# sony/aki

Hardware: AMD Instinct MI355X
Metric: image+text tokens/sec forward, AKI-4B, 336px img + 512 txt (higher is better)
Workload: dtype bf16

## Files before the change

aki_amd/_lib.py:

```python
from __future__ import annotations

import ctypes as C
import os
from typing import Optional

_HERE = os.path.dirname(os.path.abspath(__file__))
LIB_PATH = os.environ.get("AKI_MI355X_LIB") or os.path.join(_HERE, "lib", "libaki_mi355x.so")
LAB_LIB_PATH = os.path.join(_HERE, "lib", "libaki_mi355x_lab.so")

AKI_DT_BF16, AKI_DT_F32, AKI_DT_FP8_E4M3, AKI_DT_W8A16, AKI_DT_W4A16 = 0, 1, 2, 3, 4
AKI_ACT_NONE, AKI_ACT_GELU_ERF, AKI_ACT_GELU_TANH, AKI_ACT_SWIGLU = 0, 1, 2, 3
AKI_DEAD_ROWS_ZERO, AKI_DEAD_ROWS_UNIFORM = 0, 1
AKI_MAX_RECTS = 8
AKI_PLAN_STRIDE = 12
AKI_ABI_VERSION = 17
AKI_LOGITS_PROCESS_MAX_V = 131072
AKI_BEAM_MAX_K, AKI_BEAM_MAX_EOS, AKI_KV_BEAM_REORDER_CHUNK = 16, 8, 16


class AkiError(RuntimeError):
    pass


class MmaRect(C.Structure):
    _fields_ = [("row_lo", C.c_int32), ("row_hi", C.c_int32), ("col_lo", C.c_int32), ("col_hi", C.c_int32)]


class MmaAttnCoreArgs(C.Structure):
    _fields_ = [("q", C.c_void_p), ("k", C.c_void_p), ("v", C.c_void_p), ("o", C.c_void_p), ("lse", C.c_void_p),
                ("rects", C.c_void_p), ("col_valid_bits", C.c_void_p), ("seq_lens", C.c_void_p),
                ("max_rects", C.c_int32), ("B", C.c_int32), ("H", C.c_int32), ("L", C.c_int32), ("Dh", C.c_int32),
                ("scale", C.c_float), ("dtype", C.c_int32), ("dead_rows", C.c_int32), ("kv_capacity", C.c_int32)]


class MmaAttnArgs(C.Structure):
    _fields_ = [("x", C.c_void_p), ("w_qkv", C.c_void_p), ("cos", C.c_void_p), ("sin", C.c_void_p),
                ("position_ids", C.c_void_p), ("o", C.c_void_p), ("lse", C.c_void_p), ("rects", C.c_void_p),
                ("col_valid_bits", C.c_void_p), ("seq_lens", C.c_void_p), ("max_rects", C.c_int32),
                ("B", C.c_int32), ("H", C.c_int32), ("L", C.c_int32), ("Dh", C.c_int32), ("d_model", C.c_int32),
                ("ldx", C.c_int32), ("ldw", C.c_int32), ("pos_rows", C.c_int32), ("scale", C.c_float),
                ("dtype", C.c_int32), ("dead_rows", C.c_int32), ("kv_capacity", C.c_int32),
                ("x_scale", C.c_void_p), ("w_scale", C.c_void_p), ("row_scale", C.c_void_p)]


class AttnArgs(C.Structure):
    _fields_ = [("q", C.c_void_p), ("k", C.c_void_p), ("v", C.c_void_p), ("o", C.c_void_p),
                ("q_stride_b", C.c_int64), ("q_stride_h", C.c_int64), ("q_stride_t", C.c_int64),
                ("k_stride_b", C.c_int64), ("k_stride_h", C.c_int64), ("k_stride_t", C.c_int64),
                ("v_stride_b", C.c_int64), ("v_stride_h", C.c_int64), ("v_stride_t", C.c_int64),
                ("B", C.c_int32), ("H", C.c_int32), ("Lq", C.c_int32), ("Lk", C.c_int32), ("Dh", C.c_int32),
                ("scale", C.c_float), ("dtype", C.c_int32), ("lse", C.c_void_p)]


class AttnBwdArgs(C.Structure):
    _fields_ = [("q", C.c_void_p), ("k", C.c_void_p), ("v", C.c_void_p), ("o", C.c_void_p), ("d_o", C.c_void_p), ("lse", C.c_void_p),
                ("dq", C.c_void_p), ("dk", C.c_void_p), ("dv", C.c_void_p), ("rects", C.c_void_p), ("max_rects", C.c_int32),
                ("col_valid_bits", C.c_void_p), ("seq_lens", C.c_void_p), ("masked", C.c_int32),
                ("B", C.c_int32), ("H", C.c_int32), ("Lq", C.c_int32), ("Lk", C.c_int32), ("Dh", C.c_int32),
                ("scale", C.c_float), ("dtype", C.c_int32)]


class LinearArgs(C.Structure):
    _fields_ = [("x", C.c_void_p), ("w", C.c_void_p), ("bias", C.c_void_p), ("residual", C.c_void_p), ("y", C.c_void_p),
                ("M", C.c_int32), ("N", C.c_int32), ("K", C.c_int32), ("ldx", C.c_int32), ("ldw", C.c_int32),
                ("ldy", C.c_int32), ("ldr", C.c_int32), ("res_row_mod", C.c_int32), ("act", C.c_int32),
                ("dtype", C.c_int32), ("x_scale", C.c_void_p), ("w_scale", C.c_void_p),
                ("w2", C.c_void_p), ("w2_row0", C.c_int32), ("w2_rows", C.c_int32),
                ("row_scale", C.c_void_p), ("row_shift", C.c_void_p), ("col_shift", C.c_void_p), ("stats_rstd", C.c_void_p),
                ("stats_mean", C.c_void_p), ("stats_eps", C.c_float), ("stats_workspace", C.c_void_p),
                ("stats_workspace_bytes", C.c_size_t), ("splitk_workspace", C.c_void_p), ("splitk_workspace_bytes", C.c_size_t),
                ("preact_out", C.c_void_p), ("ld_preact", C.c_int64)]


class DecoderLayer(C.Structure):
    _fields_ = [("w_qkv", C.c_void_p), ("w_o", C.c_void_p), ("w_gate_up", C.c_void_p), ("w_down", C.c_void_p), ("k_cache", C.c_void_p),
                ("v_cache", C.c_void_p)]


class DecoderStackArgs(C.Structure):
    _fields_ = [("layers", C.POINTER(DecoderLayer)), ("n_layers", C.c_int32), ("h_in", C.c_void_p), ("h_out", C.c_void_p), ("rstd_out", C.c_void_p),
                ("cos", C.c_void_p), ("sin", C.c_void_p), ("position_ids", C.c_void_p), ("pos_rows", C.c_int32), ("rects", C.c_void_p),
                ("col_valid_bits", C.c_void_p), ("seq_lens", C.c_void_p), ("max_rects", C.c_int32), ("B", C.c_int32), ("H", C.c_int32),
                ("L", C.c_int32), ("Dh", C.c_int32), ("d", C.c_int32), ("F", C.c_int32), ("kv_capacity", C.c_int32), ("scale", C.c_float),
                ("rms_eps", C.c_float), ("dead_rows", C.c_int32), ("workspace", C.c_void_p), ("workspace_bytes", C.c_size_t),
                ("stats_workspace", C.c_void_p), ("stats_workspace_bytes", C.c_size_t), ("splitk_workspace", C.c_void_p),
                ("splitk_workspace_bytes", C.c_size_t)]


class SiglipLayer(C.Structure):
    _fields_ = [("w_qkv", C.c_void_p), ("b_qkv", C.c_void_p), ("c_qkv", C.c_void_p), ("w_out", C.c_void_p), ("b_out", C.c_void_p),
                ("w_fc1", C.c_void_p), ("b_fc1", C.c_void_p), ("c_fc1", C.c_void_p), ("w_fc2", C.c_void_p), ("b_fc2", C.c_void_p)]


class SiglipStackArgs(C.Structure):
    _fields_ = [("layers", C.POINTER(SiglipLayer)), ("n_layers", C.c_int32), ("h_in", C.c_void_p), ("h_out", C.c_void_p), ("fc1_out", C.c_void_p),
                ("N", C.c_int32), ("L", C.c_int32), ("E", C.c_int32), ("heads", C.c_int32), ("I", C.c_int32), ("Ip", C.c_int32),
                ("act", C.c_int32), ("ln_eps", C.c_float), ("scale", C.c_float), ("workspace", C.c_void_p), ("workspace_bytes", C.c_size_t),
                ("stats_workspace", C.c_void_p), ("stats_workspace_bytes", C.c_size_t), ("splitk_workspace", C.c_void_p),
                ("splitk_workspace_bytes", C.c_size_t)]


class PerceiverLayer(C.Structure):
    _fields_ = [("norm_media_w", C.c_void_p), ("norm_media_b", C.c_void_p), ("norm_latents_w", C.c_void_p), ("norm_latents_b", C.c_void_p),
                ("w_q", C.c_void_p), ("w_kv", C.c_void_p), ("w_out", C.c_void_p), ("ff_ln_w", C.c_void_p), ("ff_ln_b", C.c_void_p),
                ("ff_w1", C.c_void_p), ("ff_w2", C.c_void_p)]


class PerceiverStackArgs(C.Structure):
    _fields_ = [("layers", C.POINTER(PerceiverLayer)), ("n_layers", C.c_int32), ("x", C.c_void_p), ("latents", C.c_void_p), ("norm_w", C.c_void_p),
                ("norm_b", C.c_void_p), ("proj_w", C.c_void_p), ("proj_b", C.c_void_p), ("out", C.c_void_p), ("n1", C.c_int32), ("n2", C.c_int32),
                ("D", C.c_int32), ("heads", C.c_int32), ("dim_head", C.c_int32), ("d_ff", C.c_int32), ("D_out", C.c_int32), ("scale", C.c_float),
                ("eps", C.c_float), ("workspace", C.c_void_p), ("workspace_bytes", C.c_size_t)]


class SpliceArgs(C.Structure):
    _fields_ = [("lang_x", C.c_void_p), ("attention_mask", C.c_void_p), ("labels", C.c_void_p),
                ("embed_weight", C.c_void_p), ("embed_additional", C.c_void_p), ("vision_tokens", C.c_void_p),
                ("plan", C.c_void_p), ("inputs_embeds", C.c_void_p), ("labels_out", C.c_void_p),
                ("mask_1d_out", C.c_void_p), ("rects", C.c_void_p), ("col_valid_bits", C.c_void_p),
                ("seq_lens", C.c_void_p), ("max_original_id", C.c_int64), ("media_token_id", C.c_int64),
                ("pad_token_id", C.c_int64), ("B", C.c_int32), ("T", C.c_int32), ("T_img", C.c_int32),
                ("Nv", C.c_int32), ("d", C.c_int32), ("L_out", C.c_int32), ("max_rects", C.c_int32),
                ("padding_side", C.c_int32), ("dtype", C.c_int32)]


class DecodeChainLayer(C.Structure):
    _fields_ = [("w_qkv", C.c_void_p), ("w_o", C.c_void_p), ("w_gate_up", C.c_void_p), ("w_down", C.c_void_p), ("norm1", C.c_void_p),
                ("norm2", C.c_void_p), ("k_cache", C.c_void_p), ("v_cache", C.c_void_p), ("s_qkv", C.c_void_p), ("s_o", C.c_void_p),
                ("s_gate_up", C.c_void_p), ("s_down", C.c_void_p)]


class DecodeChainArgs(C.Structure):
    _fields_ = [("layers", C.c_void_p), ("h_in", C.c_void_p), ("h_out", C.c_void_p), ("cos", C.c_void_p), ("sin", C.c_void_p),
                ("cache_len", C.c_void_p), ("col_valid_bits", C.c_void_p), ("workspace", C.c_void_p), ("workspace_bytes", C.c_size_t),
                ("n_layers", C.c_int32), ("nwords", C.c_int32), ("d", C.c_int32), ("H", C.c_int32), ("Dh", C.c_int32), ("F", C.c_int32),
                ("capacity", C.c_int32), ("max_keys", C.c_int32), ("scale", C.c_float), ("rms_eps", C.c_float), ("dtype", C.c_int32),
                ("batch", C.c_int32)]


SIGNATURES = {
    "aki_strerror": (C.c_char_p, [C.c_int]),
    "aki_abi_version": (C.c_int, []),
    "aki_mma_attn_core_workspace_bytes": (C.c_size_t, [C.c_int32] * 5),
    "aki_mma_attn_core_fwd": (C.c_int, [C.POINTER(MmaAttnCoreArgs), C.c_void_p, C.c_size_t, C.c_void_p]),
    "aki_mma_attn_workspace_bytes": (C.c_size_t, [C.c_int32] * 5),
    "aki_mma_attn_fwd": (C.c_int, [C.POINTER(MmaAttnArgs), C.c_void_p, C.c_size_t, C.c_void_p]),
    "aki_qkv_rope_fwd": (C.c_int, [C.POINTER(MmaAttnArgs), C.c_void_p, C.c_void_p, C.c_void_p, C.c_void_p, C.c_size_t, C.c_void_p]),
    "aki_attn_fwd": (C.c_int, [C.POINTER(AttnArgs), C.c_void_p, C.c_size_t, C.c_void_p]),
    "aki_linear_fwd": (C.c_int, [C.POINTER(LinearArgs), C.c_void_p]),
    "aki_linear_stats_workspace_bytes": (C.c_size_t, [C.c_int32, C.c_int32]),
    "aki_linear_splitk_workspace_bytes": (C.c_size_t, [C.c_int32, C.c_int32, C.c_int32]),
    "aki_linear_stats_counter_bytes": (C.c_size_t, [C.c_int32]),
    "aki_row_stats": (C.c_int, [C.c_void_p, C.c_int32, C.c_int32, C.c_int32, C.c_float, C.c_void_p, C.c_void_p, C.c_int32, C.c_void_p]),
    "aki_rmsnorm_fwd": (C.c_int, [C.c_void_p, C.c_void_p, C.c_void_p, C.c_int32, C.c_int32, C.c_int32, C.c_int32,
                                  C.c_float, C.c_int32, C.c_void_p]),
    "aki_layernorm_fwd": (C.c_int, [C.c_void_p, C.c_void_p, C.c_void_p, C.c_void_p, C.c_int32, C.c_int32, C.c_int32,
                                    C.c_int32, C.c_float, C.c_int32, C.c_void_p]),
    "aki_patch_embed_workspace_bytes": (C.c_size_t, [C.c_int32] * 4),
    "aki_patch_embed_fwd": (C.c_int, [C.c_void_p] * 5 + [C.c_int32] * 6 + [C.c_void_p, C.c_size_t, C.c_void_p]),
    "aki_connector_mlp_workspace_bytes": (C.c_size_t, [C.c_int32] * 4),
    "aki_connector_mlp_fwd": (C.c_int, [C.c_void_p] * 6 + [C.c_int32] * 3 + [C.c_float, C.c_int32, C.c_void_p, C.c_size_t,
                                                                            C.c_void_p]),
    "aki_connector_proj_fwd": (C.c_int, [C.c_void_p] * 6 + [C.c_int32] * 3 + [C.c_float, C.c_int32, C.c_void_p, C.c_size_t,
                                                                             C.c_void_p]),
    "aki_rope_append_fwd": (C.c_int, [C.c_void_p] * 8 + [C.c_int32] * 5 + [C.c_void_p]),
    "aki_decode_attn_workspace_bytes": (C.c_size_t, [C.c_int32] * 4),
    "aki_decode_attn_fwd": (C.c_int, [C.c_void_p] * 6 + [C.c_int32] * 6 + [C.c_float, C.c_int32, C.c_void_p, C.c_size_t, C.c_void_p]),
    "aki_decode_attn_fused_fwd": (C.c_int, [C.c_void_p] * 8 + [C.c_int32] * 6 + [C.c_float, C.c_int32, C.c_void_p, C.c_size_t,
                                            C.c_void_p]),
    "aki_decode_linear_fwd": (C.c_int, [C.POINTER(LinearArgs), C.c_void_p, C.c_float, C.c_void_p]),
    "aki_kv_cache_quant_fp8": (C.c_int, [C.c_void_p, C.c_int32, C.c_void_p, C.c_void_p] + [C.c_int32] * 5 + [C.c_void_p]),
    "aki_decode_attn_fused_fp8kv_fwd": (C.c_int, [C.c_void_p] * 10 + [C.c_int32] * 6 + [C.c_float, C.c_int32, C.c_void_p, C.c_size_t,
                                                                                  C.c_void_p]),
    "aki_chunk_attn_workspace_bytes": (C.c_size_t, [C.c_int32] * 4),
    "aki_chunk_attn_fwd": (C.c_int, [C.c_void_p] * 9 + [C.c_int32] * 7 + [C.c_float, C.c_int32, C.c_void_p, C.c_size_t, C.c_void_p]),
    "aki_decode_attn_group_workspace_bytes": (C.c_size_t, [C.c_int32] * 6),
    "aki_decode_attn_group_fwd": (C.c_int, [C.c_void_p] * 11 + [C.c_int32] * 9 + [C.c_float, C.c_int32, C.c_void_p, C.c_size_t, C.c_void_p]),
    "aki_decode_chain_workspace_bytes": (C.c_size_t, [C.c_int32] * 5),
    "aki_decode_chain_error_offset": (C.c_size_t, [C.c_int32] * 2),
    "aki_decode_chain_batch_workspace_bytes": (C.c_size_t, [C.c_int32] * 6),
    "aki_decode_chain_batch_error_offset": (C.c_size_t, [C.c_int32] * 3),
    "aki_decode_chain_fwd": (C.c_int, [C.POINTER(DecodeChainArgs), C.c_void_p]),
    "aki_attn_bwd_workspace_bytes": (C.c_size_t, [C.c_int32] * 3),
    "aki_attn_bwd": (C.c_int, [C.POINTER(AttnBwdArgs), C.c_void_p, C.c_size_t, C.c_void_p]),
    "aki_transpose": (C.c_int, [C.c_void_p, C.c_void_p] + [C.c_int32] * 6 + [C.c_void_p]),
    "aki_gemm_tn": (C.c_int, [C.c_void_p, C.c_void_p, C.c_void_p] + [C.c_int32] * 3 + [C.c_int64] * 3 + [C.c_int32, C.c_void_p]),
    "aki_norm_bwd_workspace_bytes": (C.c_size_t, [C.c_int32]),
    "aki_norm_bwd": (C.c_int, [C.c_int32] + [C.c_void_p] * 7 + [C.c_int32] * 6 + [C.c_float, C.c_int32, C.c_int32, C.c_void_p, C.c_size_t,
                                                                                  C.c_void_p]),
    "aki_colsum_workspace_bytes": (C.c_size_t, [C.c_int32]),
    "aki_colsum": (C.c_int, [C.c_void_p, C.c_void_p] + [C.c_int32] * 5 + [C.c_void_p, C.c_size_t, C.c_void_p]),
    "aki_swiglu_fwd": (C.c_int, [C.c_void_p, C.c_void_p] + [C.c_int32] * 5 + [C.c_void_p]),
    "aki_swiglu_bwd": (C.c_int, [C.c_void_p] * 3 + [C.c_int32] * 6 + [C.c_void_p]),
    "aki_gelu_fwd": (C.c_int, [C.c_void_p, C.c_void_p, C.c_size_t, C.c_int32, C.c_void_p]),
    "aki_gelu_bwd": (C.c_int, [C.c_void_p] * 3 + [C.c_size_t, C.c_int32, C.c_void_p]),
    "aki_rope_bwd_merge": (C.c_int, [C.c_void_p] * 7 + [C.c_int32] * 5 + [C.c_void_p]),
    "aki_ce_loss_fwd_bwd": (C.c_int, [C.c_void_p] * 5 + [C.c_int32] * 5 + [C.c_float, C.c_int32, C.c_void_p]),
    "aki_ce_rows_fwd_bwd": (C.c_int, [C.c_void_p] * 5 + [C.c_int32] * 4 + [C.c_float, C.c_int32, C.c_void_p]),
    "aki_grad_sqnorm_workspace_bytes": (C.c_size_t, []),
    "aki_grad_sqnorm": (C.c_int, [C.c_void_p, C.c_size_t, C.c_void_p, C.c_int32, C.c_int32, C.c_void_p, C.c_size_t, C.c_void_p]),
    "aki_adamw_step": (C.c_int, [C.c_void_p] * 5 + [C.c_size_t, C.c_void_p] + [C.c_float] * 7 + [C.c_int32, C.c_void_p]),
    "aki_adamw_step_t": (C.c_int, [C.c_void_p] * 6 + [C.c_int32] * 3 + [C.c_void_p] + [C.c_float] * 7 + [C.c_int32, C.c_int32, C.c_void_p]),
# ... 179 lines not shown
```

aki_amd/csrc/aki_device.h:

```cpp
#pragma once
#include <hip/hip_runtime.h>
#include <stdint.h>

#include "aki_mi355x.h"

namespace aki {

typedef __attribute__((ext_vector_type(8))) __bf16 bf16x8;
typedef __attribute__((ext_vector_type(4))) __bf16 bf16x4;
typedef __attribute__((ext_vector_type(2))) __bf16 bf16x2;
typedef __attribute__((ext_vector_type(4))) short s16x4;
typedef __attribute__((ext_vector_type(16))) float f32x16;
typedef __attribute__((ext_vector_type(4))) float f32x4;
typedef __attribute__((ext_vector_type(4))) unsigned u32x4;
typedef __attribute__((ext_vector_type(2))) unsigned u32x2;

typedef uint16_t bf16_t;

#ifndef AKI_DEC_ITEMS
#define AKI_DEC_ITEMS 2048
#endif
#define AKI_GLOBAL_PTR(p) ((const __attribute__((address_space(1))) void*)(p))
#define AKI_LDS_PTR(p) ((__attribute__((address_space(3))) void*)(p))

// ... 21 lines not shown
}

__device__ __forceinline__ float fast_sigmoid(float x) {
  return __builtin_amdgcn_rcpf(1.0f + __builtin_amdgcn_exp2f(-1.44269504088896340736f * x));
}
__device__ __forceinline__ float silu_fast(float x) { return x * fast_sigmoid(x); }
__device__ __forceinline__ float gelu_tanh_fast(float x) {
  const float u = 0.79788456080286535588f * (x + 0.044715f * x * x * x);
  return x * fast_sigmoid(2.0f * u);
}
__device__ __forceinline__ float gelu_erf_fast(float x) {
  const float z = fabsf(x) * 0.70710678118654752440f;
  const float t = __builtin_amdgcn_rcpf(1.0f + 0.3275911f * z);
  const float poly = t * (0.254829592f + t * (-0.284496736f + t * (1.421413741f + t * (-1.453152027f + t * 1.061405429f))));
  const float erfz = 1.0f - poly * __builtin_amdgcn_exp2f(-1.44269504088896340736f * z * z);
  return 0.5f * x * (1.0f + copysignf(erfz, x));
}

__device__ __forceinline__ void halves_pair(float x, float& lo, float& hi) {
  float a = x, b = x;
  asm volatile("s_nop 1\n\tv_permlane32_swap_b32 %0, %1" : "+v"(a), "+v"(b));
  lo = a;
  hi = b;
}
__device__ __forceinline__ void mfma_results_settle(f32x16& a, f32x16& b) {
  asm volatile("s_nop 15\n\ts_nop 3" : "+v"(a), "+v"(b));
}

__device__ __forceinline__ float halves_max(float x) {
  float lo, hi;
  halves_pair(x, lo, hi);
  return fmaxf(lo, hi);
}
__device__ __forceinline__ float halves_sum(float x) {
  float lo, hi;
  halves_pair(x, lo, hi);
  return lo + hi;
}

__device__ __forceinline__ int xcd_remap(int bid, int nwg) {
  const int q = nwg >> 3, r = nwg & 7, xcd = bid & 7;
  const int base = (xcd < r) ? xcd * (q + 1) : r * (q + 1) + (xcd - r) * q;
  return base + (bid >> 3);
}

__device__ __forceinline__ void lds_reads_landed() { asm volatile("s_waitcnt lgkmcnt(0)" ::: "memory"); }
template <int N>
__device__ __forceinline__ void lds_fold_ready(float (&v)[N]) {
  lds_reads_landed();
#pragma unroll
  for (int i = 0; i < N; ++i) asm volatile("" : "+v"(v[i]));
}

__device__ __forceinline__ float wave_sum(float v) {
#pragma unroll
  for (int o = 32; o > 0; o >>= 1) v += __shfl_xor(v, o);
  return v;
}
__device__ __forceinline__ float wave_max(float v) {
#pragma unroll
  for (int o = 32; o > 0; o >>= 1) v = fmaxf(v, __shfl_xor(v, o));
  return v;
}
template <int NT>
__device__ __forceinline__ void block_sum2(float& a, float& b, float* red) {
  a = wave_sum(a);
  b = wave_sum(b);
  const int w = threadIdx.x >> 6, lane = threadIdx.x & 63;
  if (lane == 0) { red[w] = a; red[w + NT / 64] = b; }
  __syncthreads();
  float sa = 0.f, sb = 0.f;
#pragma unroll
  for (int i = 0; i < NT / 64; ++i) { sa += red[i]; sb += red[i + NT / 64]; }
  a = sa; b = sb;
  __syncthreads();
}

}

#define AKI_CHECK_ARG(cond) \
  do {                      \
    if (!(cond)) return AKI_ERR_INVALID_ARG; \
  } while (0)
#define AKI_CHECK_ALIGN16(p) \
  do {                       \
    if (((uintptr_t)(p)) & 15) return AKI_ERR_ALIGNMENT; \
  } while (0)
#define AKI_CLEAR_ERR() ((void)hipGetLastError())
#define AKI_LAUNCH_CHECK() \
  do {                     \
    if (hipGetLastError() != hipSuccess) return AKI_ERR_LAUNCH; \
  } while (0)

static inline size_t aki_elt_size(int dtype) { return dtype == AKI_DT_BF16 ? 2 : 4; }
static inline size_t aki_align_up(size_t x, size_t a) { return (x + a - 1) / a * a; }
```

aki_amd/csrc/api.hip:

```cpp
#include "aki_device.h"

namespace aki {
int linear_bf16(const aki_linear_args* a, hipStream_t stream);
size_t linear_stats_ws_bytes(int M, int n_out);
size_t linear_stats_cnt_bytes(int M);
int row_stats_launch(const void* x, int rows, int cols, int ldx, float eps, float* rstd, float* mean, hipStream_t s);
int linear_f32(const aki_linear_args* a, hipStream_t stream);
int qkv_rope_bf16(const aki_mma_attn_args* a, void* q, void* k, void* v, hipStream_t stream);
int qkv_rope_fp8(const aki_mma_attn_args* a, void* q, void* k, void* v, hipStream_t stream);
int linear_fp8(const aki_linear_args* a, hipStream_t stream);
int quant_rows_fp8_launch(const void* x, const void* rms_w, float eps, void* q, float* scale, int rows, int cols, int ldx, int ldq,
                          hipStream_t s);
int qkv_rope_f32(const aki_mma_attn_args* a, void* q, void* k, void* v, float* tmp, hipStream_t stream);
int attn_core_bf16(const aki_mma_attn_core_args* a, void* ws, size_t ws_bytes, hipStream_t stream);
int attn_core_f32(const aki_mma_attn_core_args* a, void* ws, size_t ws_bytes, hipStream_t stream, int causal);
int attn_nc_bf16(const aki_attn_args* a, hipStream_t stream);
int gemv_bf16(const aki_linear_args* a, const void* rms_w, float eps, hipStream_t stream);
int skinny_gemm_bf16(const aki_linear_args* a, const void* rms_w, float eps, hipStream_t stream);
int skinny_gemm_w8(const aki_linear_args* a, const void* rms_w, float eps, hipStream_t stream);
int quant_mxfp4_launch(const void* w, int N, int K, int ldw, uint8_t* wq, uint8_t* ws, hipStream_t s);
int gemv_w4(const aki_linear_args* a, const uint8_t* ws, const void* rms_w, float eps, hipStream_t stream);
int skinny_gemm_w4(const aki_linear_args* a, const uint8_t* ws, const void* rms_w, float eps, hipStream_t stream);
size_t decode_attn_ws_bytes(int B, int H, int Dh, int cap);
int decode_attn_split_launch(const void* q_or_qkv, const float* cos, const float* sin, const int* len, void* kc, void* vc, void* o,
                             const uint64_t* vbits, int nwords, int B, int H, int cap, int max_keys, float scale, bool fused,
                             void* ws, size_t ws_bytes, hipStream_t s);
int rope_append_launch(const void* qkv, const float* cos, const float* sin, const int* pos, const int* cache_len, void* q_out,
                       void* k_cache, void* v_cache, int B, int H, int Dh, int cap, int dtype, hipStream_t s);
int kv_cache_quant_fp8_launch(const void* src, int src_cap, void* dst, float* scale, int dst_cap, int slabs, int rows, hipStream_t s);
int decode_attn_split_fp8kv_launch(const void* qkv, const float* cos, const float* sin, const int* len, void* kc, void* vc, float* ks, float* vs,
                                   void* o, const uint64_t* vbits, int nwords, int B, int H, int cap, int max_keys, float scale, void* ws,
                                   size_t ws_bytes, hipStream_t s);
size_t decode_attn_group_ws_bytes(int B0, int N, int H, int pcap, int scap);
int decode_attn_group_launch(const void* qkv, const float* cos, const float* sin, const int* len, const int* plen, const void* kp,
                             const void* vp, void* ks, void* vs, void* o, const uint64_t* vbits, int nwords, int B0, int N, int H, int pcap,
                             int scap, int max_pkeys, int max_skeys, float scale, void* ws, size_t ws_bytes, hipStream_t s);
size_t chunk_attn_ws_bytes(int B, int H, int T);
int chunk_attn_launch(const void* qkv, const float* cos, const float* sin, const int* cache_len, const int* n_new, void* k_cache, void* v_cache,
                      void* o, const uint64_t* vbits, int nwords, int B, int H, int T, int max_new, int cap, float scale, void* ws,
                      size_t ws_bytes, hipStream_t s);
size_t decode_chain_ws_bytes(int n_layers, int d, int H, int F, int cap);
size_t decode_chain_err_offset(int n_layers, int H);
size_t decode_chain_b_ws_bytes(int n_layers, int d, int H, int F, int cap, int B);
size_t decode_chain_b_err_offset(int n_layers, int H, int B);
int decode_chain_launch(const aki_decode_chain_args* a, hipStream_t stream);
int decode_attn_launch(const void* q, const void* kc, const void* vc, void* o, const int* n_keys, const uint64_t* vbits, int nwords,
                       int B, int H, int Dh, int cap, float scale, int dtype, hipStream_t s);
int norm_launch(bool rms, const void* x, const void* w, const void* b, void* y, int rows, int cols, int ldx, int ldy,
                float eps, int dtype, hipStream_t stream);
int splice_plan_launch(const int64_t* lang_x, int B, int T, int64_t media, int64_t assistant, int Nv, int* plan, hipStream_t s);
int splice_launch(const aki_splice_args* a, hipStream_t s);
int mask_dense_launch(const aki_mma_rect* rects, int max_rects, const uint64_t* vbits, const int* seq_lens, int B, int L,
                      int64_t* out, hipStream_t s);
int im2col_launch(const void* pix, void* out, int N, int S, int P, int Kp, int dtype, hipStream_t s);
int greedy_pick_launch(const void* logits, int B, int V, int ld, const int64_t* eos, int n_eos, int64_t pad, unsigned char* done, int64_t* ids,
                       int64_t* tokens, int tokens_ld, int* cache_len, const int* start_len, int advance, int* done_at, const void* emb_main,
                       const void* emb_extra, int64_t max_original_id, int d, void* emb_out, hipStream_t s);
int logits_process_launch(const void* logits, int in_f32, int B, int V, int ld, float* out, int ld_out, const int64_t* tokens, int tokens_ld,
                          const int* cache_len, const int* start_len, int step, const unsigned char* done, float penalty, int ngram,
                          int min_len, const int64_t* eos, int n_eos, const int64_t* suppress, int n_suppress, const int64_t* begin_suppress,
                          int n_begin, const int64_t* bad_ids, const int* bad_off, int n_bad, int n_bad_ids, hipStream_t s);
// ... 119 lines not shown
  AKI_CHECK_ARG(dtype_ok(a->dtype));
  AKI_CHECK_ARG(a->max_rects >= 0 && (a->max_rects == 0 || a->rects));
  if (a->dtype == AKI_DT_BF16) return attn_core_bf16(a, ws, ws_bytes, (hipStream_t)stream);
  return attn_core_f32(a, ws, ws_bytes, (hipStream_t)stream, 1);
}

int aki_attn_fwd(const aki_attn_args* a, void* ws, size_t ws_bytes, void* stream) {
  AKI_CLEAR_ERR();
  AKI_CHECK_ARG(a && a->q && a->k && a->v && a->o);
  AKI_CHECK_ARG(a->B > 0 && a->H > 0 && a->Lq > 0 && a->Lk > 0 && a->Dh > 0 && a->scale > 0.f && dtype_ok(a->dtype));
  if (a->dtype == AKI_DT_BF16) return attn_nc_bf16(a, (hipStream_t)stream);
  const int64_t Dh = a->Dh;
  if (a->q_stride_t != Dh || a->k_stride_t != Dh || a->v_stride_t != Dh || a->q_stride_h != (int64_t)a->Lq * Dh ||
      a->k_stride_h != (int64_t)a->Lk * Dh || a->v_stride_h != (int64_t)a->Lk * Dh || a->Lq != a->Lk)
    return AKI_ERR_UNSUPPORTED;
  aki_mma_attn_core_args c = {};
  c.q = a->q; c.k = a->k; c.v = a->v; c.o = a->o; c.B = a->B; c.H = a->H; c.L = a->Lq; c.Dh = a->Dh; c.scale = a->scale;
  c.dtype = AKI_DT_F32; c.dead_rows = AKI_DEAD_ROWS_ZERO;
  return attn_core_f32(&c, ws, ws_bytes, (hipStream_t)stream, 0);
}

static size_t qkv_bytes(int B, int H, int L, int Dh, int dtype) {
  return aki_align_up((size_t)B * H * L * Dh * aki_elt_size(dtype), 256);
}

size_t aki_mma_attn_workspace_bytes(int32_t B, int32_t H, int32_t L, int32_t Dh, int32_t dtype) {
  size_t n = 3 * qkv_bytes(B, H, L, Dh, dtype) + aki_mma_attn_core_workspace_bytes(B, H, L, Dh, dtype);
  if (dtype == AKI_DT_F32) n += 3 * qkv_bytes(B, H, L, Dh, dtype);
  return n;
}

static int check_fused(const aki_mma_attn_args* a) {
  AKI_CHECK_ARG(a && a->x && a->w_qkv && a->cos && a->sin);
  AKI_CHECK_ARG(a->B > 0 && a->H > 0 && a->L > 0 && a->Dh > 0 && a->d_model > 0);
  AKI_CHECK_ARG(a->ldx >= a->d_model && a->ldw >= a->d_model && a->pos_rows > 0);
  AKI_CHECK_ARG(a->position_ids || a->pos_rows >= a->L);
  AKI_CHECK_ARG(dtype_ok(a->dtype) || (a->dtype == AKI_DT_FP8_E4M3 && a->x_scale && a->w_scale));
  AKI_CHECK_ARG(!a->row_scale || a->dtype == AKI_DT_BF16);
  return AKI_OK;
}

int aki_qkv_rope_fwd(const aki_mma_attn_args* a, void* q, void* k, void* v, void* ws, size_t ws_bytes, void* stream) {
  AKI_CLEAR_ERR();
  int rc = check_fused(a);
  if (rc) return rc;
  AKI_CHECK_ARG(q && k && v);
  AKI_CHECK_ARG(a->kv_capacity == 0 || a->kv_capacity >= a->L);
  if (a->dtype == AKI_DT_BF16) return qkv_rope_bf16(a, q, k, v, (hipStream_t)stream);
  if (a->dtype == AKI_DT_FP8_E4M3) return qkv_rope_fp8(a, q, k, v, (hipStream_t)stream);
  if (!ws || ws_bytes < (size_t)a->B * a->L * 3 * a->H * a->Dh * sizeof(float)) return AKI_ERR_WORKSPACE;
  return qkv_rope_f32(a, q, k, v, (float*)ws, (hipStream_t)stream);
}

int aki_mma_attn_fwd(const aki_mma_attn_args* a, void* ws, size_t ws_bytes, void* stream) {
  AKI_CLEAR_ERR();
  int rc = check_fused(a);
  if (rc) return rc;
  AKI_CHECK_ARG(a->o && a->scale > 0.f);
  AKI_CHECK_ARG(a->max_rects >= 0 && (a->max_rects == 0 || a->rects));
  const int cdt = a->dtype == AKI_DT_FP8_E4M3 ? AKI_DT_BF16 : a->dtype;
  if (!ws || ws_bytes < aki_mma_attn_workspace_bytes(a->B, a->H, a->L, a->Dh, cdt)) return AKI_ERR_WORKSPACE;
  AKI_CHECK_ALIGN16(ws);
  const size_t qb = qkv_bytes(a->B, a->H, a->L, a->Dh, cdt);
  char* w = (char*)ws;
  void* q = w; void* k = w + qb; void* v = w + 2 * qb;
  char* rest = w + 3 * qb;
  if (a->dtype == AKI_DT_BF16) {
    rc = qkv_rope_bf16(a, q, k, v, (hipStream_t)stream);
  } else if (a->dtype == AKI_DT_FP8_E4M3) {
    rc = qkv_rope_fp8(a, q, k, v, (hipStream_t)stream);
  } else {
    rc = qkv_rope_f32(a, q, k, v, (float*)rest, (hipStream_t)stream);
    rest += 3 * qb;
  }
  if (rc) return rc;
  aki_mma_attn_core_args c = {};
  c.q = q; c.k = k; c.v = v; c.o = a->o; c.lse = a->lse; c.rects = a->rects; c.col_valid_bits = a->col_valid_bits;
  c.seq_lens = a->seq_lens; c.max_rects = a->max_rects; c.B = a->B; c.H = a->H; c.L = a->L; c.Dh = a->Dh;
  c.scale = a->scale; c.dtype = cdt; c.dead_rows = a->dead_rows; c.kv_capacity = 0;
  return aki_mma_attn_core_fwd(&c, rest, aki_mma_attn_core_workspace_bytes(a->B, a->H, a->L, a->Dh, cdt), stream);
}

size_t aki_linear_stats_counter_bytes(int32_t M) { return M > 0 ? linear_stats_cnt_bytes(M) : 0; }
size_t aki_linear_stats_workspace_bytes(int32_t M, int32_t N_out) { return (M > 0 && N_out > 0) ? aki_align_up(linear_stats_ws_bytes(M, N_out), 256) : 0; }
size_t aki_linear_splitk_workspace_bytes(int32_t M, int32_t N, int32_t K) { return (M > 0 && N > 0 && K > 0) ? aki_align_up(linear_splitk_plan_ws_bytes(M, N, K), 256) : 0; }

int aki_row_stats(const void* x, int32_t rows, int32_t cols, int32_t ldx, float eps, float* rstd, float* mean, int32_t dtype, void* stream) {
  AKI_CLEAR_ERR();
  AKI_CHECK_ARG(x && rstd && rows > 0 && cols > 0 && ldx >= cols && eps > 0.f);
  if (dtype != AKI_DT_BF16) return AKI_ERR_UNSUPPORTED;
  return row_stats_launch(x, rows, cols, ldx, eps, rstd, mean, (hipStream_t)stream);
}

int aki_linear_fwd(const aki_linear_args* a, void* stream) {
  AKI_CLEAR_ERR();
  AKI_CHECK_ARG(a && a->x && a->w && a->y);
  AKI_CHECK_ARG(a->M > 0 && a->N > 0 && a->K > 0);
  AKI_CHECK_ARG(dtype_ok(a->dtype) || (a->dtype == AKI_DT_FP8_E4M3 && a->x_scale && a->w_scale) || (a->dtype == AKI_DT_W8A16 && a->w_scale));
  AKI_CHECK_ARG(a->act >= AKI_ACT_NONE && a->act <= AKI_ACT_SWIGLU);
  const int n_out = a->act == AKI_ACT_SWIGLU ? a->N / 2 : a->N;
  AKI_CHECK_ARG(a->ldx >= a->K && a->ldw >= a->K && a->ldy >= n_out && (!a->residual || a->ldr >= n_out));
  if (a->row_scale || a->row_shift || a->stats_rstd) {
    if (a->dtype != AKI_DT_BF16) return AKI_ERR_UNSUPPORTED;
    return linear_bf16(a, (hipStream_t)stream);
  }
  if (a->preact_out) {
    if (a->dtype != AKI_DT_BF16 || a->act != AKI_ACT_SWIGLU) return AKI_ERR_UNSUPPORTED;
    return linear_bf16(a, (hipStream_t)stream);
  }
  if (a->w2) {
    AKI_CHECK_ARG(a->w2_row0 > 0 && a->w2_rows > 0 && a->w2_row0 < a->N);
    if (a->dtype != AKI_DT_BF16 || a->act != AKI_ACT_NONE) return AKI_ERR_UNSUPPORTED;
    return linear_bf16(a, (hipStream_t)stream);
  }
  if (a->dtype == AKI_DT_FP8_E4M3) return linear_fp8(a, (hipStream_t)stream);
  if (a->dtype == AKI_DT_W8A16) {
    if (a->M >= 2 && a->M <= 16) {
      const int rc = skinny_gemm_w8(a, nullptr, 0.f, (hipStream_t)stream);
      if (rc != AKI_ERR_UNSUPPORTED) return rc;
    }
    return gemv_bf16(a, nullptr, 0.f, (hipStream_t)stream);
  }
  if (a->dtype == AKI_DT_BF16) {
    if (a->M >= 2 && a->M <= 16) {
      const int rc = skinny_gemm_bf16(a, nullptr, 0.f, (hipStream_t)stream);
      if (rc != AKI_ERR_UNSUPPORTED) return rc;
    }
    if (a->M <= 8) {
      const int rc = gemv_bf16(a, nullptr, 0.f, (hipStream_t)stream);
      if (rc != AKI_ERR_UNSUPPORTED) return rc;
    }
    return linear_bf16(a, (hipStream_t)stream);
  }
  return linear_f32(a, (hipStream_t)stream);
}

int aki_quant_rows_fp8(const void* x, const void* rms_weight, float rms_eps, void* q, float* scale, int32_t rows, int32_t cols,
                       int32_t ldx, int32_t ldq, void* stream) {
  AKI_CLEAR_ERR();
  AKI_CHECK_ARG(x && q && scale && rows > 0 && cols > 0 && ldx >= cols && ldq >= cols && (!rms_weight || rms_eps > 0.f));
  return quant_rows_fp8_launch(x, rms_weight, rms_eps, q, scale, rows, cols, ldx, ldq, (hipStream_t)stream);
}

int aki_rmsnorm_fwd(const void* x, const void* w, void* y, int32_t rows, int32_t cols, int32_t ldx, int32_t ldy, float eps,
// ... 565 lines not shown
```

aki_amd/csrc/aux_kernels.hip:

```cpp
#include "aki_device.h"

namespace aki {

template <bool RMS>
__global__ __launch_bounds__(256) void norm_bf16_kernel(const bf16_t* x, const bf16_t* w, const bf16_t* bias, bf16_t* y,
                                                        int cols, int ldx, int ldy, float eps) {
  __shared__ float red[8];
  const int row = blockIdx.x;
  const bf16_t* xr = x + (size_t)row * ldx;
  bf16_t* yr = y + (size_t)row * ldy;
  constexpr int MAXC = 4;
  u32x4 buf[MAXC];
  float s1 = 0.f, s2 = 0.f;
  const int nchunk = cols / 8;
#pragma unroll
  for (int i = 0; i < MAXC; ++i) {
    const int c = threadIdx.x + i * 256;
    if (c < nchunk) {
      buf[i] = *(const u32x4*)(xr + c * 8);
#pragma unroll
      for (int e = 0; e < 4; ++e) {
        const float a = bf16_lo(buf[i][e]), b = bf16_hi(buf[i][e]);
        s1 += a + b;
        s2 += a * a + b * b;
// ... 46 lines not shown
    }
  }
}

template <bool RMS>
__global__ __launch_bounds__(256) void norm_f32_kernel(const float* x, const float* w, const float* bias, float* y, int cols,
                                                       int ldx, int ldy, float eps) {
  __shared__ float red[8];
  const int row = blockIdx.x;
  const float* xr = x + (size_t)row * ldx;
  float* yr = y + (size_t)row * ldy;
  float s1 = 0.f, s2 = 0.f;
  for (int c = threadIdx.x; c < cols; c += 256) { const float a = xr[c]; s1 += a; s2 += a * a; }
  block_sum2<256>(s1, s2, red);
  const float mean = RMS ? 0.f : s1 / cols;
  float var = s2 / cols;
  if (!RMS) {
    float d2 = 0.f, dummy = 0.f;
    for (int c = threadIdx.x; c < cols; c += 256) { const float a = xr[c] - mean; d2 += a * a; }
    block_sum2<256>(d2, dummy, red);
    var = d2 / cols;
  }
  const float rstd = rsqrtf(var + eps);
  for (int c = threadIdx.x; c < cols; c += 256) {
    const float n = (xr[c] - mean) * rstd;
    yr[c] = RMS ? w[c] * n : n * w[c] + (bias ? bias[c] : 0.f);
  }
}

__global__ __launch_bounds__(256) void row_stats_kernel(const bf16_t* x, int cols, int ldx, float eps, float* rstd, float* mean) {
  __shared__ float red[16];
  const int row = blockIdx.x;
  const bf16_t* xr = x + (size_t)row * ldx;
  float s1 = 0.f, s2 = 0.f;
  for (int c = threadIdx.x * 8; c < cols; c += 256 * 8) {
    const u32x4 v = *(const u32x4*)(xr + c);
#pragma unroll
    for (int e = 0; e < 4; ++e) { const float a = bf16_lo(v[e]), b = bf16_hi(v[e]); s1 += a + b; s2 += a * a + b * b; }
  }
  block_sum2<256>(s1, s2, red);
  if (mean == nullptr) {
    if (threadIdx.x == 0) rstd[row] = rsqrtf(s2 / cols + eps);
    return;
  }
  const float mu = s1 / cols;
  float d2 = 0.f, dummy = 0.f;
  for (int c = threadIdx.x * 8; c < cols; c += 256 * 8) {
    const u32x4 v = *(const u32x4*)(xr + c);
#pragma unroll
    for (int e = 0; e < 4; ++e) { const float a = bf16_lo(v[e]) - mu, b = bf16_hi(v[e]) - mu; d2 += a * a + b * b; }
  }
  block_sum2<256>(d2, dummy, red);
  if (threadIdx.x == 0) { mean[row] = mu; rstd[row] = rsqrtf(d2 / cols + eps); }
}

int row_stats_launch(const void* x, int rows, int cols, int ldx, float eps, float* rstd, float* mean, hipStream_t s) {
  if (cols % 8 || ldx % 8) return AKI_ERR_UNSUPPORTED;
  AKI_CHECK_ALIGN16(x);
  AKI_CLEAR_ERR();
  hipLaunchKernelGGL(row_stats_kernel, dim3(rows), dim3(256), 0, s, (const bf16_t*)x, cols, ldx, eps, rstd, mean);
  AKI_LAUNCH_CHECK();
  return AKI_OK;
}

int norm_launch(bool rms, const void* x, const void* w, const void* b, void* y, int rows, int cols, int ldx, int ldy,
                float eps, int dtype, hipStream_t stream) {
  if (rows <= 0 || cols <= 0) return AKI_ERR_INVALID_ARG;
  if (dtype == AKI_DT_BF16) {
    if (cols % 8 || cols > 8192 || ldx % 8 || ldy % 8) return AKI_ERR_UNSUPPORTED;
    AKI_CHECK_ALIGN16(x); AKI_CHECK_ALIGN16(w); AKI_CHECK_ALIGN16(y); AKI_CHECK_ALIGN16(b);
    if (rms) hipLaunchKernelGGL(norm_bf16_kernel<true>, dim3(rows), dim3(256), 0, stream, (const bf16_t*)x, (const bf16_t*)w, (const bf16_t*)b, (bf16_t*)y, cols, ldx, ldy, eps);
    else hipLaunchKernelGGL(norm_bf16_kernel<false>, dim3(rows), dim3(256), 0, stream, (const bf16_t*)x, (const bf16_t*)w, (const bf16_t*)b, (bf16_t*)y, cols, ldx, ldy, eps);
  } else {
    if (rms) hipLaunchKernelGGL(norm_f32_kernel<true>, dim3(rows), dim3(256), 0, stream, (const float*)x, (const float*)w, (const float*)b, (float*)y, cols, ldx, ldy, eps);
    else hipLaunchKernelGGL(norm_f32_kernel<false>, dim3(rows), dim3(256), 0, stream, (const float*)x, (const float*)w, (const float*)b, (float*)y, cols, ldx, ldy, eps);
  }
  AKI_LAUNCH_CHECK();
  return AKI_OK;
}

__global__ void splice_plan_kernel(const int64_t* lang_x, int T, int64_t media_id, int64_t assistant_id, int Nv, int* plan) {
  const int b = blockIdx.x, lane = threadIdx.x;
  const int64_t* row = lang_x + (size_t)b * T;
  int* pl = plan + b * AKI_PLAN_STRIDE;
  int n_img = 0, q = 0x7fffffff;
  for (int t0 = 0; t0 < T; t0 += 64) {
    const int t = t0 + lane;
    const int64_t id = t < T ? row[t] : (int64_t)-1;
    unsigned long long mm = __ballot(t < T && id == media_id);
    if (t < T && id == assistant_id) q = min(q, t);
    while (mm) {
      const int bit = __builtin_ctzll(mm);
      mm &= mm - 1;
      if (lane == 0 && n_img < AKI_MAX_RECTS) pl[4 + n_img] = t0 + bit;
      n_img++;
    }
  }
#pragma unroll
  for (int o = 32; o > 0; o >>= 1) q = min(q, __shfl_xor(q, o));
  if (lane == 0) {
    pl[0] = n_img;
    pl[1] = q == 0x7fffffff ? 0 : q;
    pl[2] = T - n_img + Nv * n_img;
    pl[3] = 0;
    for (int i = n_img; i < AKI_MAX_RECTS; ++i) pl[4 + i] = -1;
  }
// ... 278 lines not shown
```

aki_amd/csrc/gemm_bf16.hip:

```cpp
#include <type_traits>

#include "aki_device.h"

namespace aki {

enum { EPI_PLAIN = 0, EPI_SWIGLU = 1, EPI_QKV_ROPE8 = 3 };

__device__ __forceinline__ int qkv_unit_row(int u, int s_, int H) {
  const int nqk = 6 * H;
  if (u < nqk) { const int hs = u / 3, j = u - 3 * hs; return hs * 96 + 16 * j + 48 * s_; }
  const int u2 = u - nqk, vh = u2 / 3, j2 = u2 - 3 * vh;
  return 2 * H * 96 + vh * 96 + 32 * j2 + 16 * s_;
}

struct GemmParams {
  const bf16_t* x;
  const bf16_t* w;
  const bf16_t* bias;
  const bf16_t* residual;
  bf16_t* y;
  int M, N, K;
  int ldx, ldw, ldy, ldr;
  int res_row_mod;
  int m_offset;
  int act;
  int tiles_m, tiles_n;
  bf16_t* preact;
  int ld_preact;
  int wide;
  int res_wide;
  bf16_t* q_out;
  bf16_t* k_out;
  bf16_t* v_out;
  const float* cos;
  const float* sin;
  const int* position_ids;
  int H, L;
  int kvcap;
  const float* sx;
  const float* sw;
  const bf16_t* w2;
  int w2_row0, w2_rows;
  const float* row_scale;
  const float* row_shift;
  const float* col_c;
  float* st_rstd;
  float* st_mean;
  float* st_part;
  unsigned* st_cnt;
  int ksplit;
  float* sk_part;
  size_t sk_bytes;
  int sk_slice_major;
  unsigned* sk_cnt;
#ifdef AKI_LAB_HOOKS
  int probe_block;
  long long* clock_probe;
#endif
  float st_eps;
};

__device__ __forceinline__ u32x4 pair_to_wide(unsigned p0, unsigned p1, unsigned q0, unsigned q1) {
  asm volatile("s_nop 1\n\tv_permlane16_swap_b32 %0, %1\n\tv_permlane16_swap_b32 %2, %3" : "+v"(p0), "+v"(q0), "+v"(p1), "+v"(q1));
  u32x4 o = {p0, p1, q0, q1};
  return o;
}

typedef int v8i_t __attribute__((ext_vector_type(8)));

template <int NF, int NT, int WN, int WM, int EPI, int ACT, bool FP8 = false, int NST = 2, int PIPE = 0, int SK = 0>
__global__ __launch_bounds__(WN* WM * 64, (NF * NT > 32 ? 1 : 2)) void gemm_bf16_kernel(const GemmParams p) {
  static_assert(!SK || (!FP8 && PIPE == 0), "split-K: bf16, the plain K loops");
  constexpr int BK = FP8 ? 128 : 64, ES = FP8 ? 1 : 2, NWAVES = WN * WM;
  constexpr int WROWS = NF * 16;
  constexpr int BN = WN * WROWS;
  constexpr int WTOK = NT * 16;
  constexpr int BM = WM * WTOK;
  constexpr int ROWS = BN + BM;
  constexpr int STAGE_BYTES = ROWS * 128;
  constexpr int NLD = ROWS / 8 / NWAVES;
  static_assert(ROWS % (8 * NWAVES) == 0 && NF % 2 == 0, "tile shape");
  extern __shared__ __attribute__((aligned(16))) char smem_all[];

  const int lane = threadIdx.x & 63;
  const int wave = __builtin_amdgcn_readfirstlane(threadIdx.x >> 6);
  const int tid = threadIdx.x;
  char* const smem = smem_all;
  const int wn = wave % WN, wm = wave / WN;
  const int l15 = lane & 15, kg = lane >> 4;
#ifdef AKI_LAB_HOOKS
  long long probe_c0 = 0, probe_w0 = 0;
  if ((int)blockIdx.x == p.probe_block && tid == 0 && p.clock_probe) { probe_c0 = clock64(); probe_w0 = wall_clock64(); }
#define AKI_WG_STAMP(k) do { if (p.probe_block == -2 && tid == 0 && p.clock_probe) p.clock_probe[4 * (size_t)blockIdx.x + (k)] = wall_clock64(); } while (0)
  AKI_WG_STAMP(0);
#else
#define AKI_WG_STAMP(k) do { } while (0)
#endif

  int t = xcd_remap(blockIdx.x, gridDim.x);
  int ksp = 0, kt0 = 0;
  int nk = p.K / (FP8 ? 128 : 64);
  if constexpr (SK) {
// ... 24 lines not shown
      const int w_ = row / WROWS, within = row % WROWS, nb = within >> 4, i = within & 15;
      const int f = min(n0 + w_ * (WROWS / 2) + (nb % (NF / 2)) * 16 + i, n_out - 1);
      return (nb < NF / 2) ? f : n_out + f;
    } else if (EPI == EPI_QKV_ROPE8) {
      const int w_ = row / WROWS, within = row % WROWS, nb = within >> 4, i = within & 15;
      const int u = n0 / 32 + w_ * (NF / 2) + (nb % (NF / 2));
      return min(qkv_unit_row(min(u, 9 * p.H - 1), nb / (NF / 2), p.H) + i, p.N - 1);
    } else {
      return min(n0 + row, p.N - 1);
    }
  };
  auto weight_row = [&](int row) { return weight_row_n(n0, row); };
  const char* src[NLD];
#pragma unroll
  for (int j = 0; j < NLD; ++j) {
    const int row = (j * NWAVES + wave) * 8 + (lane >> 3);
    const int chunk = (lane & 7) ^ ((row >> 1) & 7);
    if (row < BN) {
      const int wr = weight_row(row);
      const char* wp = (const char*)p.w + (size_t)wr * p.ldw * ES;
      if (EPI == EPI_PLAIN && !FP8) {
        if (p.w2 != nullptr && wr >= p.w2_row0) wp = (const char*)p.w2 + (size_t)min(wr - p.w2_row0, p.w2_rows - 1) * p.ldw * ES;
      }
      src[j] = wp + chunk * 16;
    } else {
      const int xrow = min(m0 + row - BN, p.M - 1);
      src[j] = (const char*)p.x + (size_t)xrow * p.ldx * ES + chunk * 16;
    }
    if constexpr (SK) src[j] += (size_t)kt0 * 128;
  }

  auto stage = [&](int s, int kt) {
#pragma unroll
    for (int j = 0; j < NLD; ++j) {
      char* dst = smem + s * STAGE_BYTES + (j * NWAVES + wave) * 1024;
      __builtin_amdgcn_global_load_lds(AKI_GLOBAL_PTR(src[j] + (size_t)kt * 128), AKI_LDS_PTR(dst), 16, 0, 0);
    }
  };

  f32x4 acc[NF][NT];
#pragma unroll
  for (int n = 0; n < NF; ++n)
#pragma unroll
    for (int m = 0; m < NT; ++m)
#pragma unroll
      for (int r = 0; r < 4; ++r) acc[n][m][r] = 0.f;

  const int swz = (l15 >> 1) & 7;
  const int wbase = (wn * WROWS + l15) * 128;
  const int xbase = BN * 128 + (wm * WTOK + l15) * 128;

  constexpr int NOUT = (EPI == EPI_SWIGLU) ? NF / 2 : NF;
  const int fwave = n0 + wn * (EPI == EPI_SWIGLU ? WROWS / 2 : WROWS);
  const bool shifted = (PIPE == 0 || PIPE == 4 || PIPE == 8) && (EPI == EPI_PLAIN) && p.row_shift != nullptr;
  u32x2 biasp[NOUT];
  f32x4 colc4[NOUT];
  float rsv[NT], muv[NT];
  auto fetch_epilogue_operands = [&]() {
    if (EPI == EPI_QKV_ROPE8) return;
#pragma unroll
    for (int n = 0; n < NOUT; ++n) {
      const int f = fwave + n * 16 + 4 * kg;
      biasp[n] = u32x2{0u, 0u};
      colc4[n] = f32x4{0.f, 0.f, 0.f, 0.f};
      if (EPI == EPI_PLAIN && p.bias && f < n_out) biasp[n] = *(const u32x2*)(p.bias + f);
      if (EPI == EPI_PLAIN && shifted && f < n_out) colc4[n] = *(const f32x4*)(p.col_c + f);
    }
#pragma unroll
    for (int m = 0; m < NT; ++m) {
      const int mr = min(m0 + wm * WTOK + m * 16 + l15, p.M - 1);
      rsv[m] = p.row_scale ? p.row_scale[mr] : 1.0f;
      muv[m] = (EPI == EPI_PLAIN && shifted) ? p.row_shift[mr] : 0.0f;
    }
  };
  constexpr bool EARLY_OPERANDS = (!PIPE || PIPE == 8) && !FP8 && NF * NT <= 16;
  constexpr int RCH = BN / 8;
  constexpr int CMASK = RCH >= 16 ? 15 : RCH - 1;
  constexpr int RES_PIECES = (BM * RCH * 16) / (NWAVES * 1024);
  constexpr bool RES_PF_OK = EPI == EPI_PLAIN && ACT == 0 && !FP8 && (!PIPE || PIPE == 8) && NST == 2 && RCH <= 64 && (64 % RCH == 0) && BM * RCH * 16 <= STAGE_BYTES &&
                             (PIPE != 8 || BM * RCH * 16 <= 2 * BM * 128) &&
                             (BM * RCH * 16) % (NWAVES * 1024) == 0;
  const bool res_pf = RES_PF_OK && p.residual != nullptr && p.res_wide && p.res_row_mod <= 0 && n_out >= 8;
  int res_off = 0;
  const bool cs_pf = EPI == EPI_QKV_ROPE8 && PIPE == 4 && BM == 256 && n0 / 32 < 6 * p.H && p.position_ids == nullptr && p.L >= BM;
  if constexpr (EARLY_OPERANDS) fetch_epilogue_operands();
  auto compute = [&](const char* sb) {
    if constexpr (FP8) {
      const int c0 = ((2 * kg) ^ swz) << 4, c1 = ((2 * kg + 1) ^ swz) << 4;
      v8i_t a[NF], b[NT];
#pragma unroll
      for (int n = 0; n < NF; ++n) {
        const u32x4 lo = *(const u32x4*)(sb + wbase + n * 2048 + c0), hi = *(const u32x4*)(sb + wbase + n * 2048 + c1);
        a[n] = v8i_t{(int)lo[0], (int)lo[1], (int)lo[2], (int)lo[3], (int)hi[0], (int)hi[1], (int)hi[2], (int)hi[3]};
      }
#pragma unroll
      for (int m = 0; m < NT; ++m) {
        const u32x4 lo = *(const u32x4*)(sb + xbase + m * 2048 + c0), hi = *(const u32x4*)(sb + xbase + m * 2048 + c1);
        b[m] = v8i_t{(int)lo[0], (int)lo[1], (int)lo[2], (int)lo[3], (int)hi[0], (int)hi[1], (int)hi[2], (int)hi[3]};
      }
#pragma unroll
      for (int n = 0; n < NF; ++n)
#pragma unroll
        for (int m = 0; m < NT; ++m)
          acc[n][m] = __builtin_amdgcn_mfma_scale_f32_16x16x128_f8f6f4(a[n], b[m], acc[n][m], 0, 0, 0, 0x7f7f7f7f, 0, 0x7f7f7f7f);
    } else {
#pragma unroll
      for (int ks = 0; ks < 2; ++ks) {
        const int coff = ((4 * ks + kg) ^ swz) << 4;
        bf16x8 a[NF], b[NT];
#pragma unroll
        for (int n = 0; n < NF; ++n) a[n] = *(const bf16x8*)(sb + wbase + n * 2048 + coff);
#pragma unroll
        for (int m = 0; m < NT; ++m) b[m] = *(const bf16x8*)(sb + xbase + m * 2048 + coff);
#pragma unroll
        for (int n = 0; n < NF; ++n)
#pragma unroll
          for (int m = 0; m < NT; ++m) acc[n][m] = __builtin_amdgcn_mfma_f32_16x16x32_bf16(a[n], b[m], acc[n][m], 0, 0, 0);
      }
    }
  };
#ifdef AKI_LAB_HOOKS
  long long probe_l0 = 0, probe_l1 = 0;
  if ((int)blockIdx.x == p.probe_block && tid == 0 && p.clock_probe) probe_l0 = clock64();
#endif
  AKI_WG_STAMP(1);
  if constexpr (PIPE >= 4 && PIPE <= 6) {
    static_assert(NST == 2 && !FP8, "bf16, two stages");
    auto mma = [&](const bf16x8 (&a)[NF], const bf16x8 (&b)[NT]) {
#pragma unroll
      for (int n = 0; n < NF; ++n)
#pragma unroll
        for (int m = 0; m < NT; ++m) acc[n][m] = __builtin_amdgcn_mfma_f32_16x16x32_bf16(a[n], b[m], acc[n][m], 0, 0, 0);
    };
    auto interleave_reads = [&]() {
#pragma unroll
      for (int i = 0; i < NF + NT; ++i) {
        __builtin_amdgcn_sched_group_barrier(0x008, (NF * NT) / (2 * (NF + NT)) > 0 ? (NF * NT) / (2 * (NF + NT)) : 1, 0);
// ... 18 lines not shown
    };
    bf16x8 a0[NF], b0[NT], a1[NF], b1[NT];
    constexpr bool DX = PIPE == 6, RESPF = PIPE == 5 || PIPE == 6;
    static_assert(BN == BM && (BN / 8) % NWAVES == 0 && NLD % 2 == 0, "weight / token pieces split evenly");
    static_assert(!RESPF || (WTOK == 64 && RCH == 32 && BM == 256 && NWAVES == 8), "one 32 KiB residual block per wave row");
    constexpr int WB = BN * 128, XB = BM * 128, NLH = NLD / 2;
    static_assert(WB == XB, "equal slots");
    char* const sS = smem + 3 * WB;
    constexpr int JD = DX ? NLH : 0, JS = DX ? 0 : NLH;
    auto stage_w = [&](int slot, int kt_) {
#pragma unroll
      for (int j = 0; j < NLH; ++j)
        __builtin_amdgcn_global_load_lds(AKI_GLOBAL_PTR(src[JD + j] + (size_t)kt_ * 128), AKI_LDS_PTR(smem + slot * WB + (j * NWAVES + wave) * 1024), 16, 0, 0);
    };
    auto stage_x = [&](int slot, int kt_) {
#pragma unroll
      for (int j = 0; j < NLH; ++j)
        __builtin_amdgcn_global_load_lds(AKI_GLOBAL_PTR(src[JS + j] + (size_t)kt_ * 128), AKI_LDS_PTR(sS + slot * XB + (j * NWAVES + wave) * 1024), 16, 0, 0);
    };
    const int xb0 = (wm * WTOK + l15) * 128;
    auto load_frags2 = [&](const char* sdeep, const char* sshal, int ks, bf16x8 (&a)[NF], bf16x8 (&b)[NT]) {
      const char* const sw = DX ? sshal : sdeep;
      const char* const sx = DX ? sdeep : sshal;
      const int coff = ((4 * ks + kg) ^ swz) << 4;
#pragma unroll
      for (int n = 0; n < NF; ++n) a[n] = *(const bf16x8*)(sw + wbase + n * 2048 + coff);
#pragma unroll
      for (int m = 0; m < NT; ++m) b[m] = *(const bf16x8*)(sx + xb0 + m * 2048 + coff);
    };
    auto interleave_pieces = [&](int n_) {
      for (int i = 0; i < n_; ++i) {
        __builtin_amdgcn_sched_group_barrier(0x008, 1, 0);
        __builtin_amdgcn_sched_group_barrier(0x010, 1, 0);
      }
    };
    int blkoff[4] = {0, 0, 0, 0};
    auto issue_res_block = [&](int b_, int dst_off) {
      if constexpr (RESPF) {
        blkoff[b_] = dst_off;
#pragma unroll
        for (int j = 0; j < 4; ++j) {
          const int q = j * NWAVES + wave;
          const int tk = b_ * 64 + 2 * q + (lane >> 5);
          const int ch = (lane & (RCH - 1)) ^ (tk & CMASK);
          const int f = min(n0 + 8 * ch, n_out - 8);
          const bf16_t* src_ = p.residual + (size_t)min(m0 + tk, p.M - 1) * p.ldr + f;
          __builtin_amdgcn_global_load_lds(AKI_GLOBAL_PTR(src_), AKI_LDS_PTR(smem + dst_off + q * 1024), 16, 0, 0);
        }
      }
    };
    stage_w(0, 0); stage_x(0, 0);
    if (nk > 1) { stage_w(1, 1); stage_x(1, 1); }
    if (nk > 2) stage_w(2, 2);
    if (nk > 2) asm volatile("s_waitcnt vmcnt(%0)" ::"n"(3 * NLH) : "memory");
    else if (nk > 1) asm volatile("s_waitcnt vmcnt(%0)" ::"n"(NLD) : "memory");
    else asm volatile("s_waitcnt vmcnt(0)" ::: "memory");
    __builtin_amdgcn_s_barrier();
#ifdef AKI_LAB_HOOKS
    if ((int)blockIdx.x == p.probe_block && tid == 0 && p.clock_probe) p.clock_probe[21] = clock64() - probe_l0;
#endif
    load_frags2(smem, sS, 0, a0, b0);
    int ws = 0;
    auto step4 = [&](int kt, auto next1, auto next2, auto next3) {
      constexpr bool NEXT1 = decltype(next1)::value, NEXT2 = decltype(next2)::value, NEXT3 = decltype(next3)::value;
      const int ws1 = ws == 2 ? 0 : ws + 1;
      load_frags2(smem + ws * WB, sS + (kt & 1) * XB, 1, a1, b1);
      mma(a0, b0);
      interleave_reads();
      __builtin_amdgcn_sched_barrier(0);
      if constexpr (NEXT2) asm volatile("s_waitcnt vmcnt(%0) lgkmcnt(0)" ::"n"(NLH) : "memory");
      else if constexpr (NEXT1 || !RESPF) asm volatile("s_waitcnt vmcnt(0) lgkmcnt(0)" ::: "memory");
      else asm volatile("s_waitcnt lgkmcnt(0)" ::: "memory");
      __builtin_amdgcn_s_barrier();
      if constexpr (NEXT1) load_frags2(smem + ws1 * WB, sS + ((kt + 1) & 1) * XB, 0, a0, b0);
      if constexpr (NEXT2) stage_x(kt & 1, kt + 2);
      if constexpr (NEXT3) stage_w(ws, kt + 3);
      if constexpr (RESPF && NEXT2 && !NEXT3) issue_res_block(0, ws * WB);
      if constexpr (RESPF && NEXT1 && !NEXT2) {
        if (nk == 2) issue_res_block(0, 2 * WB);
        issue_res_block(1, ws * WB);
        issue_res_block(2, 3 * WB + (kt & 1) * XB);
      }
      if constexpr (RESPF && !NEXT1) {
        if (nk == 1) { issue_res_block(0, 1 * WB); issue_res_block(1, 2 * WB); issue_res_block(2, 3 * WB + XB); }
        issue_res_block(3, ws * WB);
      }
      if constexpr (EPI == EPI_QKV_ROPE8 && !NEXT1) { if (cs_pf) issue_cos_sin(); }
      mma(a1, b1);
      if constexpr (NEXT1) interleave_reads();
      if constexpr (NEXT2 || NEXT3) interleave_pieces((NEXT2 ? NLH : 0) + (NEXT3 ? NLH : 0));
      if constexpr (RESPF && !NEXT3) interleave_pieces(NEXT2 ? 4 : (NEXT1 ? 8 : 4));
      __builtin_amdgcn_sched_barrier(0);
      ws = ws1;
    };
    int kt = 0;
    for (; kt + 3 < nk; ++kt) step4(kt, std::true_type{}, std::true_type{}, std::true_type{});
    if (kt + 2 < nk) { step4(kt, std::true_type{}, std::true_type{}, std::false_type{}); ++kt; }
    if (kt + 1 < nk) { step4(kt, std::true_type{}, std::false_type{}, std::false_type{}); ++kt; }
    step4(kt, std::false_type{}, std::false_type{}, std::false_type{});
    if constexpr (RESPF) res_off = (wm == 0 ? blkoff[0] : wm == 1 ? blkoff[1] : wm == 2 ? blkoff[2] : blkoff[3]) - wm * (64 * RCH * 16);
  } else if constexpr (PIPE == 8) {
    static_assert(PIPE != 8 || (!FP8 && NST == 2 && (BN / 8) % NWAVES == 0 && (BM / 8) % NWAVES == 0), "whole pieces per operand and wave");
    constexpr int WB = BN * 128, XB = BM * 128, NLW = BN / 8 / NWAVES, NLX = BM / 8 / NWAVES;
    char* const sXr = smem + 2 * WB;
    auto stage_w8 = [&](int slot, int kt_) {
#pragma unroll
      for (int j = 0; j < NLW; ++j)
        __builtin_amdgcn_global_load_lds(AKI_GLOBAL_PTR(src[j] + (size_t)kt_ * 128), AKI_LDS_PTR(smem + slot * WB + (j * NWAVES + wave) * 1024), 16, 0, 0);
    };
    auto stage_x8 = [&](int slot, int kt_) {
#pragma unroll
      for (int j = 0; j < NLX; ++j)
        __builtin_amdgcn_global_load_lds(AKI_GLOBAL_PTR(src[NLW + j] + (size_t)kt_ * 128), AKI_LDS_PTR(sXr + slot * XB + (j * NWAVES + wave) * 1024), 16, 0, 0);
    };
    const int xb8 = (wm * WTOK + l15) * 128;
    auto compute8 = [&](const char* sw, const char* sx) {
#pragma unroll
      for (int ks = 0; ks < 2; ++ks) {
        const int coff = ((4 * ks + kg) ^ swz) << 4;
        bf16x8 a[NF], b[NT];
#pragma unroll
        for (int n = 0; n < NF; ++n) a[n] = *(const bf16x8*)(sw + wbase + n * 2048 + coff);
#pragma unroll
        for (int m = 0; m < NT; ++m) b[m] = *(const bf16x8*)(sx + xb8 + m * 2048 + coff);
#pragma unroll
        for (int n = 0; n < NF; ++n)
#pragma unroll
          for (int m = 0; m < NT; ++m) acc[n][m] = __builtin_amdgcn_mfma_f32_16x16x32_bf16(a[n], b[m], acc[n][m], 0, 0, 0);
      }
    };
    stage_w8(0, 0); stage_x8(0, 0);
    if (nk > 1) stage_x8(1, 1);
    int xs = 0;
    for (int kt = 0; kt < nk; ++kt) {
      if (kt + 1 < nk) asm volatile("s_waitcnt vmcnt(%0)" ::"n"(NLX) : "memory");
      else asm volatile("s_waitcnt vmcnt(0)" ::: "memory");
      __builtin_amdgcn_s_barrier();
      const int xs1 = xs == 2 ? 0 : xs + 1, xs2 = xs1 == 2 ? 0 : xs1 + 1;
      if (kt + 1 < nk) stage_w8((kt + 1) & 1, kt + 1);
      if (kt + 2 < nk) stage_x8(xs2, kt + 2);
      if (kt + 1 == nk && RES_PF_OK && res_pf) {
        res_off = 2 * WB + (xs == 2 ? 0 : 2 * XB);
#pragma unroll
        for (int j = 0; j < RES_PIECES; ++j) {
          const int q = j * NWAVES + wave;
          const int tk = q * (64 / RCH) + lane / RCH;
          const int ch = (lane & (RCH - 1)) ^ (tk & CMASK);
          const int f = min(n0 + 8 * ch, n_out - 8);
          const bf16_t* src_ = p.residual + (size_t)min(m0 + tk, p.M - 1) * p.ldr + f;
          __builtin_amdgcn_global_load_lds(AKI_GLOBAL_PTR(src_), AKI_LDS_PTR(smem + res_off + q * 1024), 16, 0, 0);
        }
      }
      compute8(smem + (kt & 1) * WB, sXr + xs * XB);
      xs = xs1;
    }
  } else if constexpr (NST == 2) {
    stage(0, 0);
    for (int kt = 0; kt < nk; ++kt) {
      __syncthreads();
      if (kt + 1 < nk) stage((kt + 1) & 1, kt + 1);
      else if (RES_PF_OK && res_pf) {
        res_off = ((kt + 1) & 1) * STAGE_BYTES;
#pragma unroll
        for (int j = 0; j < RES_PIECES; ++j) {
          const int q = j * NWAVES + wave;
          const int tk = q * (64 / RCH) + lane / RCH;
          const int ch = (lane & (RCH - 1)) ^ (tk & CMASK);
          const int f = min(n0 + 8 * ch, n_out - 8);
          const bf16_t* src_ = p.residual + (size_t)min(m0 + tk, p.M - 1) * p.ldr + f;
          __builtin_amdgcn_global_load_lds(AKI_GLOBAL_PTR(src_), AKI_LDS_PTR(smem + res_off + q * 1024), 16, 0, 0);
        }
      }
      compute(smem + (kt & 1) * STAGE_BYTES);
    }
  } else {
    static_assert(NST >= 3 && NST <= 6 && (NST - 2) * NLD < 64, "the counted waits below are written for three to six stages");
#pragma unroll
    for (int s_ = 0; s_ < NST - 1; ++s_)
      if (s_ < nk) stage(s_, s_);
    for (int kt = 0; kt < nk; ++kt) {
      const int rem = nk - 1 - kt;
      if (NST >= 6 && rem >= 4) asm volatile("s_waitcnt vmcnt(%0)" ::"n"(4 * NLD) : "memory");
      else if (NST >= 5 && rem >= 3) asm volatile("s_waitcnt vmcnt(%0)" ::"n"(3 * NLD) : "memory");
      else if (NST >= 4 && rem >= 2) asm volatile("s_waitcnt vmcnt(%0)" ::"n"(2 * NLD) : "memory");
      else if (rem >= 1) asm volatile("s_waitcnt vmcnt(%0)" ::"n"(NLD) : "memory");
      else asm volatile("s_waitcnt vmcnt(0)" ::: "memory");
      __builtin_amdgcn_s_barrier();
      if (kt + NST - 1 < nk) stage((kt + NST - 1) % NST, kt + NST - 1);
      compute(smem + (kt % NST) * STAGE_BYTES);
    }
  }

#ifdef AKI_LAB_HOOKS
  if ((int)blockIdx.x == p.probe_block && tid == 0 && p.clock_probe) probe_l1 = clock64();
#endif
  AKI_WG_STAMP(2);
  if constexpr (SK) {
    if (p.ksplit > 1) {
      __shared__ unsigned sk_last;
      constexpr int TILE_BYTES = BN * BM * 4;
      float* const tile_base = p.sk_part + (size_t)t * p.ksplit * (BN * BM);
      const __amdgpu_buffer_rsrc_t rs = __builtin_amdgcn_make_buffer_rsrc((void*)tile_base, (short)0, p.ksplit * TILE_BYTES, 0x00020000);
      const int lane_off = (wave * NF * NT * 64 + lane) * 16;
#pragma unroll
      for (int n = 0; n < NF; ++n)
#pragma unroll
        for (int m = 0; m < NT; ++m)
          __builtin_amdgcn_raw_buffer_store_b128(__builtin_bit_cast(u32x4, acc[n][m]), rs, ksp * TILE_BYTES + lane_off + (n * NT + m) * 1024, 0, 16);
      asm volatile("s_waitcnt vmcnt(0)" ::: "memory");
      __syncthreads();
      if (tid == 0) {
        const unsigned old = __hip_atomic_fetch_add(p.sk_cnt + t, 1u, __ATOMIC_RELAXED, __HIP_MEMORY_SCOPE_AGENT);
        sk_last = (old == (unsigned)p.ksplit - 1u) ? 1u : 0u;
        if (old == (unsigned)p.ksplit - 1u) __hip_atomic_store(p.sk_cnt + t, 0u, __ATOMIC_RELAXED, __HIP_MEMORY_SCOPE_AGENT);
      }
      __syncthreads();
#ifdef AKI_LAB_HOOKS
      if ((int)blockIdx.x == p.probe_block && tid == 0 && p.clock_probe) {
        p.clock_probe[0] = clock64() - probe_c0; p.clock_probe[1] = wall_clock64() - probe_w0;
        p.clock_probe[18] = probe_l0 - probe_c0; p.clock_probe[19] = clock64() - probe_l1; p.clock_probe[22] = sk_last;
      }
#endif
      if (sk_last == 0u) { AKI_WG_STAMP(3); return; }
      auto load_slice = [&](int i, f32x4 (&dst)[NF][NT]) {
#pragma unroll
        for (int n = 0; n < NF; ++n)
#pragma unroll
          for (int m = 0; m < NT; ++m)
            dst[n][m] = __builtin_bit_cast(f32x4, __builtin_amdgcn_raw_buffer_load_b128(rs, i * TILE_BYTES + lane_off + (n * NT + m) * 1024, 0, 16));
      };
      if (p.ksplit == 2) {
        f32x4 other[NF][NT];
// ... 48 lines not shown
        wrow = min(n0 + wn * WROWS + n * 16 + 4 * kg, p.N - 4);
      }
      const f32x4 s4 = *(const f32x4*)(p.sw + wrow);
#pragma unroll
      for (int m = 0; m < NT; ++m)
#pragma unroll
        for (int r = 0; r < 4; ++r) acc[n][m][r] *= s4[r] * sxm[m];
    }
  }

  if (EPI == EPI_QKV_ROPE8) {
    constexpr int UW = NF / 2;
    const int u0 = n0 / 32 + wn * UW, nqk = 6 * p.H;
    constexpr int CSROW = 400;
    static_assert(EPI != EPI_QKV_ROPE8 || BM * CSROW <= NST * STAGE_BYTES, "cos/sin staging fits the K-loop buffers");
    const bool tile_has_rope = n0 / 32 < nqk;
    if (cs_pf) {
      asm volatile("s_waitcnt vmcnt(0)" ::: "memory");
      __syncthreads();
    } else if (tile_has_rope) {
      __syncthreads();
      for (int tk = tid >> 1; tk < BM; tk += (NWAVES * 64) >> 1) {
        const int mr = min(m0 + tk, p.M - 1) + p.m_offset;
        const int pos = p.position_ids ? p.position_ids[mr] : mr % p.L;
        const int half = tid & 1;
        const float* cp = p.cos + (size_t)pos * 96 + half * 24;
        const float* sp = p.sin + (size_t)pos * 96 + half * 24;
        char* dst = smem + tk * CSROW + half * 96;
#pragma unroll
        for (int i = 0; i < 6; ++i) {
          *(f32x4*)(dst + i * 16) = *(const f32x4*)(cp + 4 * i);
          *(f32x4*)(dst + 192 + i * 16) = *(const f32x4*)(sp + 4 * i);
        }
      }
      __syncthreads();
    }
#ifdef AKI_LAB_HOOKS
    long long probe_s = 0;
    if ((int)blockIdx.x == p.probe_block && tid == 0 && p.clock_probe) probe_s = clock64();
#endif
    size_t offq[NT], dkv[NT];
    int csoff[NT];
    float rsq[NT];
    bool okq[NT];
#pragma unroll
    for (int m = 0; m < NT; ++m) {
      const int mrow = m0 + wm * WTOK + m * 16 + l15;
      okq[m] = mrow < p.M;
      const int mr = min(mrow, p.M - 1) + p.m_offset;
      const int b = mr / p.L, tt = mr - b * p.L;
      offq[m] = ((size_t)b * ((size_t)p.H * p.L) + tt) * 96;
      dkv[m] = (size_t)b * ((size_t)p.H * (p.kvcap - p.L)) * 96;
      csoff[m] = (wm * WTOK + m * 16 + l15) * CSROW + 16 * kg;
      rsq[m] = p.row_scale ? p.row_scale[min(mrow, p.M - 1)] : 1.0f;
    }
    const __attribute__((address_space(3))) char* const lcs = (const __attribute__((address_space(3))) char*)AKI_LDS_PTR(smem);
    auto rope_rows = [&](auto fullm_) {
      constexpr bool FULLM = decltype(fullm_)::value;
#pragma unroll
      for (int q = 0; q < UW; ++q) {
        const int u = u0 + q;
        if (u >= 9 * p.H) continue;
        if (u < nqk) {
          const int hs = u / 3, j = u - 3 * hs, which = hs / p.H, head = hs - which * p.H;
          bf16_t* const plane = which == 0 ? p.q_out + (size_t)head * p.L * 96 : p.k_out + (size_t)head * p.kvcap * 96;
          const int d1 = 16 * j + 4 * kg, d2 = d1 + 48;
          const int dw = ((kg & 1) ? d2 : d1) - 4 * kg + 8 * (kg >> 1);
#pragma unroll
          for (int m = 0; m < NT; ++m) {
            const f32x4 c4 = *(const __attribute__((address_space(3))) f32x4*)(lcs + csoff[m] + 64 * j);
            const f32x4 s4 = *(const __attribute__((address_space(3))) f32x4*)(lcs + csoff[m] + 192 + 64 * j);
            float v1[4], v2[4];
#pragma unroll
            for (int r = 0; r < 4; ++r) {
              const float x1 = acc[q][m][r] * rsq[m], x2 = acc[q + UW][m][r] * rsq[m];
              v1[r] = x1 * c4[r] - x2 * s4[r];
              v2[r] = x2 * c4[r] + x1 * s4[r];
            }
            const u32x4 o = pair_to_wide(pack_bf16x2(v1[0], v1[1]), pack_bf16x2(v1[2], v1[3]), pack_bf16x2(v2[0], v2[1]), pack_bf16x2(v2[2], v2[3]));
            bf16_t* dst = plane + offq[m] + (which == 0 ? (size_t)0 : dkv[m]) + dw;
            if (FULLM || okq[m]) *(u32x4*)dst = o;
          }
        } else {
          const int u2 = u - nqk, vh = u2 / 3, j2 = u2 - 3 * vh;
          bf16_t* const plane = p.v_out + (size_t)vh * p.kvcap * 96;
          const int d1 = 32 * j2 + 4 * kg, d2 = d1 + 16;
          const int dw = ((kg & 1) ? d2 : d1) - 4 * kg + 8 * (kg >> 1);
#pragma unroll
          for (int m = 0; m < NT; ++m) {
            float v1[4], v2[4];
#pragma unroll
            for (int r = 0; r < 4; ++r) { v1[r] = acc[q][m][r] * rsq[m]; v2[r] = acc[q + UW][m][r] * rsq[m]; }
            const u32x4 o = pair_to_wide(pack_bf16x2(v1[0], v1[1]), pack_bf16x2(v1[2], v1[3]), pack_bf16x2(v2[0], v2[1]), pack_bf16x2(v2[2], v2[3]));
            bf16_t* dst = plane + offq[m] + dkv[m] + dw;
            if (FULLM || okq[m]) *(u32x4*)dst = o;
          }
        }
      }
    };
    if (m0 + BM <= p.M) rope_rows(std::true_type{});
    else rope_rows(std::false_type{});
#ifdef AKI_LAB_HOOKS
    if ((int)blockIdx.x == p.probe_block && tid == 0 && p.clock_probe) {
      p.clock_probe[0] = clock64() - probe_c0;
      p.clock_probe[1] = wall_clock64() - probe_w0;
      p.clock_probe[18] = probe_l0 - probe_c0;
      p.clock_probe[19] = clock64() - probe_l1;
// ... 98 lines not shown
        }
        if (HR == 2 && has_res && fin) {
          if (in_lds) {
            const int ch = (wn * WROWS + n * 16) / 8 + (kg >> 1);
            rr[n] = *(const __attribute__((address_space(3))) u32x2*)(lres + (tk * RCH + (ch ^ (tk & CMASK))) * 16 + (kg & 1) * 8);
          } else {
            rr[n] = *(const u32x2*)(rrow + f);
          }
        }
        if (has_res && fin) {
          v[n][0] += bf16_lo(rr[n][0]); v[n][1] += bf16_hi(rr[n][0]); v[n][2] += bf16_lo(rr[n][1]); v[n][3] += bf16_hi(rr[n][1]);
        }
      }
      if (EPI == EPI_SWIGLU) {
        if (p.preact) {
          bf16_t* const prow = p.preact + (size_t)mr * p.ld_preact;
          const bool pwide = NOUT % 2 == 0 && n_out % 8 == 0 && p.ld_preact % 8 == 0 && (((uintptr_t)p.preact) & 15) == 0;
          if (pwide) {
#pragma unroll
            for (int n = 0; n + 1 < NOUT; n += 2) {
              const u32x4 og = pair_to_wide(gpk[n][0], gpk[n][1], gpk[n + 1][0], gpk[n + 1][1]);
              const u32x4 ou = pair_to_wide(upk[n][0], upk[n][1], upk[n + 1][0], upk[n + 1][1]);
              const int f = fwave + (n + (kg & 1)) * 16 + 8 * (kg >> 1);
              if (ok && (FULL || f < n_out)) { *(u32x4*)(prow + f) = og; *(u32x4*)(prow + n_out + f) = ou; }
            }
          } else {
#pragma unroll
            for (int n = 0; n < NOUT; ++n) {
              const int f = fwave + n * 16 + 4 * kg;
              if (ok && f < n_out) { *(u32x2*)(prow + f) = u32x2{gpk[n][0], gpk[n][1]}; *(u32x2*)(prow + n_out + f) = u32x2{upk[n][0], upk[n][1]}; }
            }
          }
        }
      }
      unsigned pk[NOUT][2];
#pragma unroll
      for (int n = 0; n < NOUT; ++n) { pk[n][0] = pack_bf16x2(v[n][0], v[n][1]); pk[n][1] = pack_bf16x2(v[n][2], v[n][3]); }
      if (has_stats) {
        float s1 = 0.f, s2 = 0.f;
#pragma unroll
        for (int n = 0; n < NOUT; ++n) {
          const bool fin = FULL || fwave + n * 16 + 4 * kg < n_out;
#pragma unroll
          for (int r = 0; r < 4; ++r) {
            const unsigned w_ = pk[n][r >> 1];
            const float vb = fin ? ((r & 1) ? bf16_hi(w_) : bf16_lo(w_)) : 0.f;
            s1 += vb;
            s2 += vb * vb;
          }
        }
        s1 += __shfl_xor(s1, 16); s2 += __shfl_xor(s2, 16);
        s1 += __shfl_xor(s1, 32); s2 += __shfl_xor(s2, 32);
        if (kg == 0 && ok) {
          unsigned long long* pp = (unsigned long long*)p.st_part + (size_t)(tn * WN + wn) * p.M + mrow;
          const unsigned long long both = (unsigned long long)__float_as_uint(s2) | ((unsigned long long)__float_as_uint(s1) << 32);
          __hip_atomic_store(pp, both, __ATOMIC_RELAXED, __HIP_MEMORY_SCOPE_AGENT);
        }
      }
      if (wide) {
#pragma unroll
        for (int n = 0; n + 1 < NOUT; n += 2) {
          const u32x4 o = pair_to_wide(pk[n][0], pk[n][1], pk[n + 1][0], pk[n + 1][1]);
          const int f = fwave + (n + (kg & 1)) * 16 + 8 * (kg >> 1);
          if (ok && (FULL || f < n_out)) *(u32x4*)(yrow + f) = o;
        }
      } else {
#pragma unroll
        for (int n = 0; n < NOUT; ++n) {
          const int f = fwave + n * 16 + 4 * kg;
          if (ok && f < n_out) {
            u32x2 o = {pk[n][0], pk[n][1]};
            *(u32x2*)(yrow + f) = o;
          }
        }
      }
    }
  };
  {
    using c0 = std::integral_constant<int, 0>;
    using c1 = std::integral_constant<int, 1>;
    using c2 = std::integral_constant<int, 2>;
    const bool inside = m0 + BM <= p.M && n0 + (EPI == EPI_SWIGLU ? BN / 2 : BN) <= n_out;
    const bool fast = inside && NOUT % 2 == 0 && p.wide && (p.residual == nullptr || (EPI == EPI_PLAIN && res_lds));
    const int key = (EPI == EPI_PLAIN && p.bias ? 1 : 0) | (p.residual ? 2 : 0) | (stats ? 4 : 0) | (p.row_scale ? 8 : 0) | (shifted ? 16 : 0);
    bool done = false;
    if (fast) {
      done = true;
      if (key == 0) write_rows(c1{}, c0{}, c0{}, c0{}, c0{}, c0{});
      else if (key == 8) write_rows(c1{}, c0{}, c0{}, c0{}, c1{}, c0{});
      else if constexpr (EPI == EPI_PLAIN) {
        if (key == 1) write_rows(c1{}, c1{}, c0{}, c0{}, c0{}, c0{});
        else if (key == 2) write_rows(c1{}, c0{}, c1{}, c0{}, c0{}, c0{});
        else if (key == 3) write_rows(c1{}, c1{}, c1{}, c0{}, c0{}, c0{});
        else if (key == 6) write_rows(c1{}, c0{}, c1{}, c1{}, c0{}, c0{});
        else if (key == 7) write_rows(c1{}, c1{}, c1{}, c1{}, c0{}, c0{});
        else if constexpr (PIPE == 0 || PIPE == 4 || PIPE == 8) {
          if (key == 25) write_rows(c1{}, c1{}, c0{}, c0{}, c1{}, c1{});
          else done = false;
        } else done = false;
      } else done = false;
    }
    if (!done) write_rows(c0{}, c2{}, c2{}, c2{}, c2{}, c2{});
  }
  if (EPI == EPI_PLAIN && stats) {
    asm volatile("s_waitcnt vmcnt(0)" ::: "memory");
    __syncthreads();
    unsigned* const flag = (unsigned*)smem;
    if (tid == 0) {
      const unsigned old = __hip_atomic_fetch_add(p.st_cnt + tm, 1u, __ATOMIC_RELAXED, __HIP_MEMORY_SCOPE_AGENT);
      *flag = (old == (unsigned)p.tiles_n - 1u) ? 1u : 0u;
    }
    __syncthreads();
    if (*flag != 0u) {
      const int slots = p.tiles_n * WN;
      constexpr int NTHR = NWAVES * 64;
      constexpr int CH = (NST * STAGE_BYTES - 16) / (BM * 8);
      static_assert(CH >= 8, "statistics staging");
      unsigned long long* const park = (unsigned long long*)(smem + 16);
      const unsigned long long* const part = (const unsigned long long*)p.st_part;
      float s1 = 0.f, s2 = 0.f;
      for (int sl0 = 0; sl0 < slots; sl0 += CH) {
        const int total = min(CH, slots - sl0) * BM;
        for (int it0 = tid; it0 < total; it0 += 8 * NTHR) {
          unsigned long long got[8];
#pragma unroll
          for (int u = 0; u < 8; ++u) {
            const int it = it0 + u * NTHR;
            const int sl = it / BM, row = it - sl * BM;
            got[u] = 0ull;
            if (it < total && m0 + row < p.M)
              got[u] = __hip_atomic_load(part + (size_t)(sl0 + sl) * p.M + m0 + row, __ATOMIC_RELAXED, __HIP_MEMORY_SCOPE_AGENT);
          }
#pragma unroll
          for (int u = 0; u < 8; ++u) {
            const int it = it0 + u * NTHR;
            if (it < total) park[it] = got[u];
          }
        }
        __syncthreads();
        if (tid < BM) {
          for (int sl = 0; sl < total / BM; ++sl) {
            unsigned long long both = park[sl * BM + tid];
            asm volatile("s_waitcnt lgkmcnt(0)" : "+v"(both));
            s2 += __uint_as_float((unsigned)both);
            s1 += __uint_as_float((unsigned)(both >> 32));
          }
        }
        __syncthreads();
      }
      if (tid < BM && m0 + tid < p.M) {
        const int mrow = m0 + tid;
        const float inv_n = 1.0f / (float)n_out;
        const float mean = s1 * inv_n;
        if (p.st_mean) {
          p.st_mean[mrow] = mean;
          p.st_rstd[mrow] = rsqrtf(fmaxf(s2 * inv_n - mean * mean, 0.f) + p.st_eps);
        } else {
          p.st_rstd[mrow] = rsqrtf(s2 * inv_n + p.st_eps);
        }
      }
      if (tid == 0) __hip_atomic_store(p.st_cnt + tm, 0u, __ATOMIC_RELAXED, __HIP_MEMORY_SCOPE_AGENT);
    }
  }
#ifdef AKI_LAB_HOOKS
  if ((int)blockIdx.x == p.probe_block && tid == 0 && p.clock_probe) {
    p.clock_probe[0] = clock64() - probe_c0;
    p.clock_probe[1] = wall_clock64() - probe_w0;
    p.clock_probe[18] = probe_l0 - probe_c0;
    p.clock_probe[19] = clock64() - probe_l1;
  }
#endif
  AKI_WG_STAMP(3);
}
#undef AKI_WG_STAMP

#ifdef AKI_LAB_HOOKS
int g_sk_slice_major = 0;
int g_force_tile = 0, g_deep_ring = 1, g_res_prefetch = 1, g_deepx = 0;
long long* g_clock_probe = nullptr;
int g_probe_block = 0;
constexpr int kGemmLogFields = 14, kGemmLogCap = 256;
static int g_gemm_log[kGemmLogCap][kGemmLogFields];
static int g_gemm_log_n = 0;
int g_gemm_dry_run = 0;
void gemm_log_reset() { g_gemm_log_n = 0; }
int gemm_log_copy(int* out, int cap) {
  const int n = g_gemm_log_n < kGemmLogCap ? g_gemm_log_n : kGemmLogCap;
  for (int i = 0; out && i < n && i < cap; ++i)
    for (int j = 0; j < kGemmLogFields; ++j) out[i * kGemmLogFields + j] = g_gemm_log[i][j];
  return g_gemm_log_n;
}
static void gemm_log_push(const int (&r)[kGemmLogFields]) {
  if (g_gemm_log_n < kGemmLogCap)
    for (int j = 0; j < kGemmLogFields; ++j) g_gemm_log[g_gemm_log_n][j] = r[j];
  ++g_gemm_log_n;
}
#else
static constexpr int g_force_tile = 0, g_deep_ring = 1, g_res_prefetch = 1, g_deepx = 0, g_sk_slice_major = 0;
#endif

template <int NF, int NT, int WN, int WM, int EPI, int ACT = 0, bool FP8 = false, int NST = 2, int PIPE = 0, int SK = 0>
static int launch_gemm(GemmParams& p, hipStream_t stream) {
  constexpr int BN = WN * NF * 16, BM = WM * NT * 16;
  constexpr int SMEM = (PIPE >= 4 && PIPE <= 6) ? (BN > BM ? 3 * BN + 2 * BM : 3 * BM + 2 * BN) * 128
                       : (PIPE == 8 ? (2 * BN + 4 * BM) * 128 : NST * (BN + BM) * 128);
  static_assert(SMEM <= 160 * 1024, "LDS");
#ifdef AKI_LAB_HOOKS
  {
    const int n_out_ = (EPI == EPI_SWIGLU) ? p.N / 2 : p.N, bn_out_ = (EPI == EPI_SWIGLU) ? BN / 2 : BN;
    const int slices_ = (SK && p.ksplit > 1) ? p.ksplit : 1;
    const int grid_ = ((p.M + BM - 1) / BM) * ((n_out_ + bn_out_ - 1) / bn_out_) * slices_;
    gemm_log_push({NF, NT, WN, WM, EPI, ACT, FP8 ? 1 : 0, NST, PIPE, SK, slices_, p.M, p.m_offset, grid_});
    if (g_gemm_dry_run) return AKI_OK;
  }
#endif
  static bool attr_set = false;
  if (!attr_set) {
    if (hipFuncSetAttribute((const void*)gemm_bf16_kernel<NF, NT, WN, WM, EPI, ACT, FP8, NST, PIPE, SK>, hipFuncAttributeMaxDynamicSharedMemorySize, SMEM) != hipSuccess)
      return AKI_ERR_LAUNCH;
    attr_set = true;
  }
  const int n_out = (EPI == EPI_SWIGLU) ? p.N / 2 : p.N;
  const int bn_out = (EPI == EPI_SWIGLU) ? BN / 2 : BN;
  p.tiles_m = (p.M + BM - 1) / BM;
  p.tiles_n = (n_out + bn_out - 1) / bn_out;
  AKI_CLEAR_ERR();
#ifdef AKI_LAB_HOOKS
  p.clock_probe = g_clock_probe;
  p.probe_block = g_probe_block;
#endif
  const int slices = SK ? (p.ksplit > 1 ? p.ksplit : (p.ksplit = 1)) : 1;
  p.sk_slice_major = g_sk_slice_major;
  hipLaunchKernelGGL((gemm_bf16_kernel<NF, NT, WN, WM, EPI, ACT, FP8, NST, PIPE, SK>), dim3(p.tiles_m * p.tiles_n * slices), dim3(WN * WM * 64), SMEM, stream, p);
  AKI_LAUNCH_CHECK();
  return AKI_OK;
}


static double cost_big(long tiles, int ksteps = 0) {
  const long full = tiles / 256, rem = tiles % 256;
  if (rem == 0) return (double)full;
  return (double)full + ((ksteps >= 64 && full >= 1 && rem <= 128) ? 0.65 : 1.0);
}
static double cost_small(long tiles, double work) {
  return tiles <= 256 ? (tiles ? work / 0.75 : 0.0) : (double)((tiles + 511) / 512) * (2.0 * work / 0.9);
}

static int plan_tiles(int M, int n_out, int bn_big, int bn_small, double small_work = 0.25, bool mid_ok = false, int ksteps = 0) {
  if (g_force_tile) return g_force_tile == 2 ? 1 : (g_force_tile == 3 ? (mid_ok ? 3 : 1) : (g_force_tile == 5 ? (mid_ok ? 4 : 1) : 0));
  const long nb = (n_out + bn_big - 1) / bn_big, ns = (n_out + bn_small - 1) / bn_small;
  const double all_big = cost_big((long)((M + 255) / 256) * nb, ksteps);
  const double all_small = cost_small((long)((M + 127) / 128) * ns, small_work);
  const int m_main = M / 256 * 256, tail = M - m_main;
  double split = 1e30;
  if (m_main > 0 && tail > 0) split = cost_big((long)(m_main / 256) * nb) + cost_small((long)((tail + 127) / 128) * ns, small_work);
  if (mid_ok) {
    const long nm = (long)((M + 95) / 96) * ns;
    if (M > 128 && nm <= 128 && ksteps >= 32 && (long)((M + 63) / 64) * ((n_out + 63) / 64) <= 512) return 4;
    if (nm <= 512) {
      const double all_mid = cost_small(nm, 0.75 * small_work);
      if (all_mid < all_small && all_mid < all_big && all_mid < split) return 3;
    }
  }
  if (all_small < all_big && all_small <= split) return 1;
  if (split < all_big) return 2;
  return 0;
}


template <int EPI, int ACT, bool FP8>
static int launch_small(GemmParams& p, hipStream_t stream) {
  if constexpr (!FP8) {
    const int n_out = (EPI == EPI_SWIGLU) ? p.N / 2 : p.N, bn_out = (EPI == EPI_SWIGLU) ? 64 : 128;
    const long tiles = (long)((p.M + 127) / 128) * ((n_out + bn_out - 1) / bn_out);
    if (g_deep_ring && p.M <= 128 && p.K / 64 >= 4) {
      if (EPI != EPI_QKV_ROPE8 && tiles <= 128) return launch_gemm<2, 4, 2, 2, EPI, ACT, FP8, 4>(p, stream);
      if (tiles <= 256) return launch_gemm<4, 4, 2, 2, EPI, ACT, FP8, 4>(p, stream);
    }
  }
  return launch_gemm<4, 4, 2, 2, EPI, ACT, FP8>(p, stream);
}

static bool deep_tokens(const GemmParams& p) { return g_deepx == 1 || (g_deepx == 0 && (long)p.M > 3L * p.N / 2 && p.K >= 4096); }

template <int EPI, int ACT, bool FP8>
static int launch_big(GemmParams& p, hipStream_t stream) {
  if constexpr (FP8) {
    return launch_gemm<8, 4, 2, 4, EPI, ACT, FP8>(p, stream);
  } else {
    if constexpr (EPI == EPI_PLAIN && ACT == 0) {
      if (g_res_prefetch && p.row_shift == nullptr && p.residual != nullptr && p.res_wide && p.res_row_mod <= 0 && p.N % 8 == 0 && p.N >= 8)
        return deep_tokens(p) ? launch_gemm<8, 4, 2, 4, EPI, ACT, FP8, 2, 6>(p, stream) : launch_gemm<8, 4, 2, 4, EPI, ACT, FP8, 2, 5>(p, stream);
    }
    return launch_gemm<8, 4, 2, 4, EPI, ACT, FP8, 2, 4>(p, stream);
  }
}

struct SmallMTile { int bn, bm; };
static SmallMTile small_m_tile(int variant) {
  switch (variant) {
    case 1: return {128, 128};
    case 3: case 4: return {128, 96};
    case 5: return {128, 64};
  }
  return {0, 0};
}
size_t linear_splitk_cnt_bytes() { return size_t(64) << 10; }
static size_t linear_splitk_ws_bytes(int variant, int ksplit, int M, int n_out) {
  const SmallMTile tl = small_m_tile(variant);
  if (ksplit <= 1 || tl.bn == 0) return 0;
  const size_t tiles = (size_t)((M + tl.bm - 1) / tl.bm) * ((n_out + tl.bn - 1) / tl.bn);
  return linear_splitk_cnt_bytes() + tiles * ksplit * tl.bn * tl.bm * sizeof(float);
}

static void plan_small_m(int epi, int M, int n_out, int K, bool can_split, int& variant, int& ksplit) {
  variant = -1; ksplit = 1;
  if (M < 17 || M > 1024 || g_force_tile) return;
  const int nk = K / 64;
  if (epi == EPI_QKV_ROPE8) { variant = M > 256 ? 3 : 4; return; }
  if (epi == EPI_SWIGLU) { if (M <= 256 && nk >= 8) variant = 1; return; }
  if (n_out > 4096 || nk < 36 || !can_split) return;
  const int v = M > 256 ? 3 : 5;
  const SmallMTile tl = small_m_tile(v);
  const long tiles = (long)((M + tl.bm - 1) / tl.bm) * ((n_out + tl.bn - 1) / tl.bn);
  const int ks = (int)(512 / tiles) < 3 ? (int)(512 / tiles) : 3;
  if (ks < 2) return;
  variant = v; ksplit = ks;
}
size_t linear_splitk_plan_ws_bytes(int M, int N, int K) {
  int v, ks;
  plan_small_m(EPI_PLAIN, M, N, K, true, v, ks);
  return linear_splitk_ws_bytes(v, ks, M, N);
}

template <int EPI, int ACT>
static int launch_small_m(GemmParams& p, int variant, int ksplit, hipStream_t stream) {
  p.ksplit = ksplit;
  if constexpr (EPI == EPI_QKV_ROPE8) {
    if (variant == 3) return launch_gemm<4, 3, 2, 2, EPI, ACT, false, 2, 0, 0>(p, stream);
    if (variant == 4) return launch_gemm<4, 3, 2, 2, EPI, ACT, false, 3, 0, 0>(p, stream);
  } else if constexpr (EPI == EPI_SWIGLU) {
    if (variant == 1) return launch_gemm<4, 4, 2, 2, EPI, ACT, false, 3, 0, 0>(p, stream);
  } else if constexpr (ACT == 0) {
    if (variant == 3) return launch_gemm<4, 3, 2, 2, EPI, ACT, false, 2, 0, 1>(p, stream);
    if (variant == 5) return launch_gemm<4, 2, 2, 2, EPI, ACT, false, 3, 0, 1>(p, stream);
  }
  return AKI_ERR_UNSUPPORTED;
}

template <int EPI, int ACT, bool FP8 = false>
static int run_planned(GemmParams& p, int plan, hipStream_t stream) {
  if constexpr (!FP8 && (EPI != EPI_PLAIN || ACT == 0)) {
    if (p.w2 == nullptr) {
      int v, ks;
      const int n_out = (EPI == EPI_SWIGLU) ? p.N / 2 : p.N;
      plan_small_m(EPI, p.M, n_out, p.K, p.sk_part != nullptr, v, ks);
      if (v >= 0 && ks > 1 && p.sk_bytes < linear_splitk_ws_bytes(v, ks, p.M, n_out) - linear_splitk_cnt_bytes()) v = -1;
      if (v >= 0 && !(EPI == EPI_PLAIN && p.row_shift != nullptr)) return launch_small_m<EPI, ACT>(p, v, ks, stream);
    }
  }
  if (plan == 1) return launch_small<EPI, ACT, FP8>(p, stream);
  if (plan == 0) return launch_big<EPI, ACT, FP8>(p, stream);
  if constexpr (EPI == EPI_PLAIN && !FP8) {
    if (plan == 3) return launch_gemm<4, 3, 2, 2, EPI, ACT, FP8, 2, 8>(p, stream);
    if (plan == 4) return launch_gemm<2, 2, 2, 2, EPI, ACT, FP8, 4>(p, stream);
  }
  const int m_main = p.M / 256 * 256;
  GemmParams a = p, b = p;
  a.M = m_main;
  int rc = launch_big<EPI, ACT, FP8>(a, stream);
  if (rc) return rc;
  b.M = p.M - m_main;
  b.m_offset = p.m_offset + m_main;
  b.x = (const bf16_t*)((const char*)p.x + (size_t)m_main * p.ldx * (FP8 ? 1 : 2));
  if (FP8) b.sx = p.sx + m_main;
  b.y = p.y + (size_t)m_main * p.ldy;
  if (p.preact) b.preact = p.preact + (size_t)m_main * p.ld_preact;
  if (p.residual && p.res_row_mod <= 0) b.residual = p.residual + (size_t)m_main * p.ldr;
  if (p.row_scale) b.row_scale = p.row_scale + m_main;
  if (p.row_shift) b.row_shift = p.row_shift + m_main;
  if (p.st_rstd) b.st_rstd = p.st_rstd + m_main;
  if (p.st_mean) b.st_mean = p.st_mean + m_main;
  return launch_small<EPI, ACT, FP8>(b, stream);
}

constexpr size_t kStatsCntBytes = size_t(1) << 20;
constexpr int kStatsMaxRows = int(kStatsCntBytes / sizeof(unsigned)) * 64;
size_t linear_stats_cnt_bytes(int M) {
  (void)M;
  return kStatsCntBytes;
}
size_t linear_stats_ws_bytes(int M, int n_out) {
  return linear_stats_cnt_bytes(M) + (size_t)(2 * ((n_out + 63) / 64) + 2) * 2 * (size_t)M * sizeof(float);
}

int linear_bf16(const aki_linear_args* a, hipStream_t stream) {
  if (a->K % 64 != 0) return AKI_ERR_UNSUPPORTED;
  const int n_out = a->act == AKI_ACT_SWIGLU ? a->N / 2 : a->N;
  if (n_out % 4 != 0 || (a->act == AKI_ACT_SWIGLU && (a->N % 8 != 0))) return AKI_ERR_UNSUPPORTED;
  if ((a->ldx % 8) || (a->ldw % 8) || (a->ldy % 4) || (a->residual && (a->ldr % 4))) return AKI_ERR_ALIGNMENT;
  AKI_CHECK_ALIGN16(a->x);
  AKI_CHECK_ALIGN16(a->w);
  if (((uintptr_t)a->y & 7) || ((uintptr_t)a->residual & 7) || ((uintptr_t)a->bias & 7)) return AKI_ERR_ALIGNMENT;
  GemmParams p = {};
  p.x = (const bf16_t*)a->x; p.w = (const bf16_t*)a->w; p.bias = (const bf16_t*)a->bias;
  p.residual = (const bf16_t*)a->residual; p.y = (bf16_t*)a->y;
  p.M = a->M; p.N = a->N; p.K = a->K; p.ldx = a->ldx; p.ldw = a->ldw; p.ldy = a->ldy; p.ldr = a->ldr;
  p.res_row_mod = a->res_row_mod; p.act = a->act;
  p.wide = (n_out % 8 == 0) && (a->ldy % 8 == 0) && (((uintptr_t)a->y & 15) == 0);
  p.res_wide = a->residual && (n_out % 8 == 0) && (a->ldr % 8 == 0) && (((uintptr_t)a->residual & 15) == 0);
  if (a->w2) {
    AKI_CHECK_ALIGN16(a->w2);
    p.w2 = (const bf16_t*)a->w2; p.w2_row0 = a->w2_row0; p.w2_rows = a->w2_rows;
  }
  p.row_scale = a->row_scale; p.row_shift = a->row_shift; p.col_c = a->col_shift;
  if (a->row_shift && (!a->col_shift || !a->row_scale || (((uintptr_t)a->col_shift) & 15) || a->act == AKI_ACT_SWIGLU)) return AKI_ERR_INVALID_ARG;
  if (a->stats_rstd) {
    if (a->act == AKI_ACT_SWIGLU || a->M > kStatsMaxRows) return AKI_ERR_UNSUPPORTED;
    if (!a->stats_workspace || a->stats_workspace_bytes < linear_stats_ws_bytes(a->M, n_out) || (((uintptr_t)a->stats_workspace) & 15)) return AKI_ERR_WORKSPACE;
    p.st_rstd = a->stats_rstd; p.st_mean = a->stats_mean; p.st_eps = a->stats_eps;
    p.st_cnt = (unsigned*)a->stats_workspace;
    p.st_part = (float*)((char*)a->stats_workspace + linear_stats_cnt_bytes(a->M));
  }
  if (a->preact_out) {
    if (a->act != AKI_ACT_SWIGLU || a->row_scale) return AKI_ERR_INVALID_ARG;
    if ((a->ld_preact % 4) || a->ld_preact < a->N || ((uintptr_t)a->preact_out & 7)) return AKI_ERR_ALIGNMENT;
    p.preact = (bf16_t*)a->preact_out; p.ld_preact = (int)a->ld_preact;
  }
  if (a->act == AKI_ACT_SWIGLU) {
    if (a->bias) return AKI_ERR_UNSUPPORTED;
    return run_planned<EPI_SWIGLU, 0>(p, plan_tiles(a->M, n_out, 128, 64), stream);
  }
  if (a->splitk_workspace && a->splitk_workspace_bytes > linear_splitk_cnt_bytes() && !(((uintptr_t)a->splitk_workspace) & 255)) {
    p.sk_cnt = (unsigned*)a->splitk_workspace;
    p.sk_part = (float*)((char*)a->splitk_workspace + linear_splitk_cnt_bytes());
    p.sk_bytes = a->splitk_workspace_bytes - linear_splitk_cnt_bytes();
  }
  const int plan = plan_tiles(a->M, n_out, 256, 128, 0.25, true, a->K / 64);
  switch (a->act) {
    case AKI_ACT_GELU_ERF: return run_planned<EPI_PLAIN, AKI_ACT_GELU_ERF>(p, plan, stream);
    case AKI_ACT_GELU_TANH: return run_planned<EPI_PLAIN, AKI_ACT_GELU_TANH>(p, plan, stream);
    default: return run_planned<EPI_PLAIN, 0>(p, plan, stream);
  }
}

int qkv_rope_bf16(const aki_mma_attn_args* a, void* q, void* k, void* v, hipStream_t stream) {
  if (a->Dh != 96) return AKI_ERR_UNSUPPORTED;
  if (a->d_model % 64 != 0) return AKI_ERR_UNSUPPORTED;
  if ((a->ldx % 8) || (a->ldw % 8)) return AKI_ERR_ALIGNMENT;
  AKI_CHECK_ALIGN16(a->x); AKI_CHECK_ALIGN16(a->w_qkv); AKI_CHECK_ALIGN16(a->cos); AKI_CHECK_ALIGN16(a->sin);
  AKI_CHECK_ALIGN16(q); AKI_CHECK_ALIGN16(k); AKI_CHECK_ALIGN16(v);
  GemmParams p = {};
  p.x = (const bf16_t*)a->x; p.w = (const bf16_t*)a->w_qkv;
  p.M = a->B * a->L; p.N = 3 * a->H * a->Dh; p.K = a->d_model; p.ldx = a->ldx; p.ldw = a->ldw;
  p.q_out = (bf16_t*)q; p.k_out = (bf16_t*)k; p.v_out = (bf16_t*)v;
  p.cos = a->cos; p.sin = a->sin; p.position_ids = a->position_ids; p.H = a->H; p.L = a->L;
  p.kvcap = a->kv_capacity > 0 ? a->kv_capacity : a->L;
  p.row_scale = a->row_scale;
  return run_planned<EPI_QKV_ROPE8, 0>(p, plan_tiles(p.M, p.N, 256, 128), stream);
}

int linear_fp8(const aki_linear_args* a, hipStream_t stream) {
  if (a->K % 128 != 0 || !a->x_scale || !a->w_scale) return AKI_ERR_UNSUPPORTED;
  const int n_out = a->act == AKI_ACT_SWIGLU ? a->N / 2 : a->N;
  if (n_out % 4 != 0 || (a->act == AKI_ACT_SWIGLU && (a->N % 8 != 0))) return AKI_ERR_UNSUPPORTED;
  if ((a->ldx % 16) || (a->ldw % 16) || (a->ldy % 4) || (a->residual && (a->ldr % 4))) return AKI_ERR_ALIGNMENT;
  AKI_CHECK_ALIGN16(a->x);
  AKI_CHECK_ALIGN16(a->w);
  AKI_CHECK_ALIGN16(a->w_scale);
  if (((uintptr_t)a->y & 7) || ((uintptr_t)a->residual & 7) || ((uintptr_t)a->bias & 7)) return AKI_ERR_ALIGNMENT;
  GemmParams p = {};
  p.x = (const bf16_t*)a->x; p.w = (const bf16_t*)a->w; p.bias = (const bf16_t*)a->bias;
  p.residual = (const bf16_t*)a->residual; p.y = (bf16_t*)a->y;
  p.M = a->M; p.N = a->N; p.K = a->K; p.ldx = a->ldx; p.ldw = a->ldw; p.ldy = a->ldy; p.ldr = a->ldr;
  p.res_row_mod = a->res_row_mod; p.act = a->act; p.sx = a->x_scale; p.sw = a->w_scale;
  p.wide = (n_out % 8 == 0) && (a->ldy % 8 == 0) && (((uintptr_t)a->y & 15) == 0);
  p.res_wide = a->residual && (n_out % 8 == 0) && (a->ldr % 8 == 0) && (((uintptr_t)a->residual & 15) == 0);
  if (a->act == AKI_ACT_SWIGLU) {
    if (a->bias) return AKI_ERR_UNSUPPORTED;
    return run_planned<EPI_SWIGLU, 0, true>(p, plan_tiles(a->M, n_out, 128, 64), stream);
  }
  if (a->act != AKI_ACT_NONE) return AKI_ERR_UNSUPPORTED;
  return run_planned<EPI_PLAIN, 0, true>(p, plan_tiles(a->M, n_out, 256, 128), stream);
}

int qkv_rope_fp8(const aki_mma_attn_args* a, void* q, void* k, void* v, hipStream_t stream) {
  if (a->Dh != 96 || a->d_model % 128 != 0 || !a->x_scale || !a->w_scale) return AKI_ERR_UNSUPPORTED;
  if ((a->ldx % 16) || (a->ldw % 16)) return AKI_ERR_ALIGNMENT;
  AKI_CHECK_ALIGN16(a->x); AKI_CHECK_ALIGN16(a->w_qkv); AKI_CHECK_ALIGN16(a->cos); AKI_CHECK_ALIGN16(a->sin);
  AKI_CHECK_ALIGN16(q); AKI_CHECK_ALIGN16(k); AKI_CHECK_ALIGN16(v); AKI_CHECK_ALIGN16(a->w_scale);
  GemmParams p = {};
  p.x = (const bf16_t*)a->x; p.w = (const bf16_t*)a->w_qkv;
  p.M = a->B * a->L; p.N = 3 * a->H * a->Dh; p.K = a->d_model; p.ldx = a->ldx; p.ldw = a->ldw;
  p.q_out = (bf16_t*)q; p.k_out = (bf16_t*)k; p.v_out = (bf16_t*)v;
  p.cos = a->cos; p.sin = a->sin; p.position_ids = a->position_ids; p.H = a->H; p.L = a->L;
  p.kvcap = a->kv_capacity > 0 ? a->kv_capacity : a->L;
  p.sx = a->x_scale; p.sw = a->w_scale;
  return run_planned<EPI_QKV_ROPE8, 0, true>(p, plan_tiles(p.M, p.N, 256, 128), stream);
}

}
```

aki_amd/ops.py:

```python
from __future__ import annotations

import ctypes as C
import threading
from dataclasses import dataclass
from typing import Optional, Tuple

import torch

from . import _lib as L
from ._lib import AkiError

ACT_NONE, ACT_GELU_ERF, ACT_GELU_TANH, ACT_SWIGLU = L.AKI_ACT_NONE, L.AKI_ACT_GELU_ERF, L.AKI_ACT_GELU_TANH, L.AKI_ACT_SWIGLU
DEAD_ROWS_ZERO, DEAD_ROWS_UNIFORM = L.AKI_DEAD_ROWS_ZERO, L.AKI_DEAD_ROWS_UNIFORM


def _dt(t: torch.Tensor) -> int:
    if t.dtype == torch.bfloat16:
        return L.AKI_DT_BF16
    if t.dtype == torch.float32:
        return L.AKI_DT_F32
    raise AkiError(f"unsupported dtype {t.dtype}: the AKI HIP path computes in bf16 or f32")


def _dev(*ts: Optional[torch.Tensor]) -> torch.device:
# ... 29 lines not shown


class EventTap:

    def __init__(self, tags=None, select=None, every=1):
        self.tags = tags
        self.select = select
        self.events = {}
        self.every = every
        self.calls = {}

    def want(self, tag) -> bool:
        if self.tags is not None and tag[0] not in self.tags:
            return False
        return self.select is None or bool(self.select(tag))

    def begin(self, tag):
        n = self.calls[tag] = self.calls.get(tag, 0) + 1
        if (n - 1) % self.every:
            return None
        a = torch.cuda.Event(enable_timing=True)
        b = torch.cuda.Event(enable_timing=True)
        self.events.setdefault(tag, []).append((a, b))
        a.record()
        return b

    def summary(self):
        torch.cuda.synchronize()
        return {tag: (self.calls[tag], sum(a.elapsed_time(b) for a, b in ev) / len(ev)) for tag, ev in self.events.items()}


class Prepared:

    def __init__(self):
        self._c = {}

    def get(self, name, params, fn, epoch=0):
        key = (epoch,) + tuple((p.data_ptr(), p._version, p.dtype, p.device) for p in params)
        hit = self._c.get(name)
        if hit is None or hit[0] != key:
            with torch.no_grad():
                self._c[name] = (key, fn())
        return self._c[name][1]

    def clear(self) -> None:
        self._c.clear()


def fold_gain(w: torch.Tensor, gain: torch.Tensor) -> torch.Tensor:
    ct = torch.float64 if w.dtype == torch.float64 else torch.float32
    return (w.detach().to(ct) * gain.detach().to(ct)[None, :]).to(w.dtype).contiguous()


@dataclass
class RowStats:
    rstd: torch.Tensor
    mean: Optional[torch.Tensor] = None


_STATS_WS = {}


def _stats_ws(M: int, n_out: int, dev) -> torch.Tensor:
    need = int(L.load().aki_linear_stats_workspace_bytes(M, n_out))
    key = (torch.device(dev).index, torch.cuda.current_stream().cuda_stream)
    hit = _STATS_WS.get(key)
    if hit is None or hit.numel() < need:
        hit = _STATS_WS[key] = torch.zeros(max(need, 8 << 20), dtype=torch.uint8, device=dev)
    return hit


_SPLITK_WS = {}
SPLITK_WS_MIN_BYTES = 0
SPLITK_MAX_M = 2048


def _splitk_ws(M: int, N: int, K: int, dev) -> Optional[torch.Tensor]:
    need = max(int(L.load().aki_linear_splitk_workspace_bytes(M, N, K)), SPLITK_WS_MIN_BYTES)
    if need == 0:
        return None
    key = (torch.device(dev).index, torch.cuda.current_stream().cuda_stream)
    hit = _SPLITK_WS.get(key)
    if hit is None or hit.numel() < need:
        hit = _SPLITK_WS[key] = torch.zeros(max(need, 32 << 20), dtype=torch.uint8, device=dev)
    return hit


def new_stats(M: int, dev, ln: bool = False) -> RowStats:
    return RowStats(torch.empty((M,), dtype=torch.float32, device=dev), torch.empty((M,), dtype=torch.float32, device=dev) if ln else None)


def row_stats(x: torch.Tensor, eps: float, ln: bool = False) -> RowStats:
    dev = _dev(x)
    x2 = _rows2d(x)
    st = new_stats(x2.shape[0], dev, ln)
    L.check(L.load().aki_row_stats(_ptr(x2), x2.shape[0], x2.shape[1], x2.stride(0), float(eps), _ptr(st.rstd), _ptr(st.mean), _dt(x),
                                   _stream()), "aki_row_stats")
    return st


_TAP: Optional[EventTap] = None


def set_event_tap(tap: Optional[EventTap]) -> None:
    global _TAP
    _TAP = tap


@dataclass
class MaskTable:
    rects: Optional[torch.Tensor]
    col_valid_bits: Optional[torch.Tensor]
    seq_lens: Optional[torch.Tensor]
    L: int
    mask_1d: Optional[torch.Tensor] = None

    @property
    def max_rects(self) -> int:
        return 0 if self.rects is None else int(self.rects.shape[1])

    def token_counts(self, B: int, device) -> torch.Tensor:
        if self.col_valid_bits is None:
            return torch.full((B,), self.L, dtype=torch.int32, device=device)
        nw = self.col_valid_bits.shape[1]
        shifts = torch.arange(64, device=device, dtype=torch.int64)
        valid = ((self.col_valid_bits[:, :, None] >> shifts) & 1).view(B, nw * 64)[:, : self.L]
        pos = torch.arange(1, self.L + 1, device=device, dtype=torch.int64)
        return (valid * pos).amax(dim=1).to(torch.int32)

    @staticmethod
    def causal(B: int, Lq: int, device) -> "MaskTable":
        return MaskTable(None, None, None, Lq)

    @staticmethod
    def from_host(rects, mask_1d, seq_lens, device) -> "MaskTable":
        import numpy as np
        m = np.asarray(mask_1d).astype(bool)
        B, Lq = m.shape
        k = max(1, max(len(r) for r in rects))
        ra = np.zeros((B, k, 4), dtype=np.int32)
        for b, rs in enumerate(rects):
            for i, r in enumerate(rs):
                ra[b, i] = r
        nw = (Lq + 63) // 64
        pad = np.zeros((B, nw * 64), dtype=bool)
        pad[:, :Lq] = m
        bits = np.packbits(pad.reshape(B, nw, 64), axis=-1, bitorder="little").view(np.uint64).reshape(B, nw)
        t = MaskTable(torch.from_numpy(ra).to(device), torch.from_numpy(bits.view(np.int64).copy()).to(device),
                      None if seq_lens is None else torch.tensor(list(seq_lens), dtype=torch.int32, device=device), Lq,
                      torch.from_numpy(m.astype(np.int64)).to(device))
        return t


def linear(x: torch.Tensor, w: torch.Tensor, bias: Optional[torch.Tensor] = None, residual: Optional[torch.Tensor] = None,
           act: int = ACT_NONE, res_row_mod: int = 0, out: Optional[torch.Tensor] = None, w2: Optional[torch.Tensor] = None,
           w2_row0: int = 0, n_rows: Optional[int] = None, row_scale: Optional[torch.Tensor] = None,
           row_shift: Optional[torch.Tensor] = None, col_shift: Optional[torch.Tensor] = None,
           stats_out: Optional[RowStats] = None, stats_eps: float = 0.0, preact_out: Optional[torch.Tensor] = None) -> torch.Tensor:
    dev = _dev(x, w, bias, residual, out, w2, row_scale, row_shift, col_shift)
    lib = L.load()
    x2 = _rows2d(x)
    M, K = x2.shape
    N = w.shape[0] if w2 is None else int(n_rows if n_rows is not None else w2_row0 + w2.shape[0])
    if w2 is not None and (w2.shape[1] != K or w2.stride(1) != 1 or w2.stride(0) != w.stride(0) or not 0 < w2_row0 <= w.shape[0]):
        raise AkiError("linear: the second weight segment must have the layout of the first")
    if w.shape[1] != K or w.stride(1) != 1:
        raise AkiError(f"linear: weight {tuple(w.shape)} does not match input K={K}")
    n_out = N // 2 if act == ACT_SWIGLU else N
    if out is None:
        out = torch.empty((*x.shape[:-1], n_out), dtype=x.dtype, device=dev)
    o2 = out.view(-1, out.shape[-1])
    if o2.shape != (M, n_out) or o2.stride(1) != 1:
        raise AkiError("linear: bad output buffer")
    r2 = None
    if residual is not None:
        r2 = _rows2d(residual)
    a = L.LinearArgs(_ptr(x2), _ptr(w), _ptr(bias), _ptr(r2), _ptr(o2), M, N, K, x2.stride(0), w.stride(0), o2.stride(0),
                     0 if r2 is None else r2.stride(0), res_row_mod, act, _dt(x), None, None,
                     _ptr(w2), int(w2_row0) if w2 is not None else 0, int(w2.shape[0]) if w2 is not None else 0)
    a.row_scale, a.row_shift, a.col_shift = _ptr(row_scale), _ptr(row_shift), _ptr(col_shift)
    if stats_out is not None:
        sws = _stats_ws(M, n_out, dev)
        a.stats_rstd, a.stats_mean, a.stats_eps = _ptr(stats_out.rstd), _ptr(stats_out.mean), float(stats_eps)
        a.stats_workspace, a.stats_workspace_bytes = sws.data_ptr(), sws.numel()
    if preact_out is not None:
        p2 = preact_out.view(-1, preact_out.shape[-1])
        if act != ACT_SWIGLU or p2.shape != (M, N) or p2.stride(1) != 1 or p2.dtype != torch.bfloat16 or p2.device != x2.device:
            raise AkiError("linear: preact_out must be a bf16 [M, N] buffer of an act=SWIGLU launch")
        a.preact_out, a.ld_preact = p2.data_ptr(), p2.stride(0)
    if act == ACT_NONE and M <= SPLITK_MAX_M and x.dtype == torch.bfloat16:
        sk = _splitk_ws(M, N, K, dev)
        if sk is not None:
            a.splitk_workspace, a.splitk_workspace_bytes = sk.data_ptr(), sk.numel()
    end = _TAP.begin(("linear", M, N, K, act)) if (_TAP is not None and _TAP.want(("linear", M, N, K, act))) else None
    L.check(lib.aki_linear_fwd(C.byref(a), _stream()), "aki_linear_fwd")
    if end is not None:
        end.record()
    return out


def rmsnorm(x: torch.Tensor, w: torch.Tensor, eps: float) -> torch.Tensor:
    dev = _dev(x, w)
    x2 = _rows2d(x)
    y = torch.empty_like(x2)
    L.check(L.load().aki_rmsnorm_fwd(_ptr(x2), _ptr(w), _ptr(y), x2.shape[0], x2.shape[1], x2.stride(0), y.stride(0),
                                     float(eps), _dt(x), _stream()), "aki_rmsnorm_fwd")
    return y.reshape(x.shape)


def layernorm(x: torch.Tensor, w: torch.Tensor, b: Optional[torch.Tensor], eps: float) -> torch.Tensor:
    dev = _dev(x, w, b)
    x2 = _rows2d(x)
    y = torch.empty_like(x2)
    L.check(L.load().aki_layernorm_fwd(_ptr(x2), _ptr(w), _ptr(b), _ptr(y), x2.shape[0], x2.shape[1], x2.stride(0),
                                       y.stride(0), float(eps), _dt(x), _stream()), "aki_layernorm_fwd")
    return y.reshape(x.shape)


def mma_attn_core(q: torch.Tensor, k: torch.Tensor, v: torch.Tensor, table: MaskTable, scale: float,
                  dead_rows: int = DEAD_ROWS_UNIFORM, return_lse: bool = False):
    dev = _dev(q, k, v)
    B, H, Lq, Dh = q.shape
    cap = k.shape[2]
    if v.shape[2] != cap or cap < Lq:
        raise AkiError("mma_attn_core: k/v capacity mismatch")
    q, k, v = q.contiguous(), k.contiguous(), v.contiguous()
    o = torch.empty((B, Lq, H * Dh), dtype=q.dtype, device=dev)
    lse = torch.empty((B, H, Lq), dtype=torch.float32, device=dev) if return_lse else None
    lib = L.load()
    ws = _ws(lib.aki_mma_attn_core_workspace_bytes(B, H, Lq, Dh, _dt(q)), dev)
    a = L.MmaAttnCoreArgs(_ptr(q), _ptr(k), _ptr(v), _ptr(o), _ptr(lse), _ptr(table.rects), _ptr(table.col_valid_bits),
                          _ptr(table.seq_lens), table.max_rects, B, H, Lq, Dh, float(scale), _dt(q), dead_rows,
                          0 if cap == Lq else cap)
    end = _TAP.begin(("mma_attn_core", B, H, Lq, Dh)) if (_TAP is not None and _TAP.want(("mma_attn_core",))) else None
    L.check(lib.aki_mma_attn_core_fwd(C.byref(a), _ptr(ws), ws.numel(), _stream()), "aki_mma_attn_core_fwd")
    if end is not None:
        end.record()
    return (o, lse) if return_lse else o


def attention(q: torch.Tensor, k: torch.Tensor, v: torch.Tensor, scale: float, return_lse: bool = False):
    dev = _dev(q, k, v)
    B, Lq, H, Dh = q.shape
    Lk = k.shape[1]
    o = torch.empty((B, Lq, H * Dh), dtype=q.dtype, device=dev)
    lib = L.load()
    if q.dtype == torch.float32:
        if Lq != Lk:
            qp = torch.zeros((B, Lk, H, Dh), dtype=q.dtype, device=dev)
            qp[:, :Lq] = q
            return attention(qp, k, v, scale)[:, :Lq].contiguous()
        q, k, v = (t_.permute(0, 2, 1, 3).contiguous() for t_ in (q, k, v))
        st = lambda t_: (t_.stride(0), t_.stride(1), t_.stride(2))
    else:
        for t_ in (q, k, v):
            if t_.stride(3) != 1:
                raise AkiError("attention: channel stride must be 1")
        st = lambda t_: (t_.stride(0), t_.stride(2), t_.stride(1))
    ws = _ws(B * H * Dh * 4 + 256, dev)
    lse = torch.empty((B, H, Lq), dtype=torch.float32, device=dev) if return_lse else None
    if return_lse and q.dtype != torch.bfloat16:
        raise AkiError("attention: the log-sum-exp output exists on the bf16 path only")
    a = L.AttnArgs(_ptr(q), _ptr(k), _ptr(v), _ptr(o), *st(q), *st(k), *st(v), B, H, Lq, Lk, Dh, float(scale), _dt(q), _ptr(lse))
    end = _TAP.begin(("attention", B, H, Lq, Lk, Dh)) if (_TAP is not None and _TAP.want(("attention",))) else None
    L.check(lib.aki_attn_fwd(C.byref(a), _ptr(ws), ws.numel(), _stream()), "aki_attn_fwd")
    if end is not None:
        end.record()
    return (o, lse) if return_lse else o


def _fused_args(x2, w_qkv, cos, sin, position_ids, o, lse, table, B, H, Lq, Dh, scale, dead_rows, kv_capacity=0, row_scale=None):
    return L.MmaAttnArgs(_ptr(x2), _ptr(w_qkv), _ptr(cos), _ptr(sin), _ptr(position_ids), _ptr(o), _ptr(lse),
                         _ptr(table.rects), _ptr(table.col_valid_bits), _ptr(table.seq_lens), table.max_rects,
                         B, H, Lq, Dh, x2.shape[1], x2.stride(0), w_qkv.stride(0), cos.shape[0], float(scale),
                         _dt(x2), dead_rows, kv_capacity, None, None, _ptr(row_scale))


def mma_attn(x: torch.Tensor, w_qkv: torch.Tensor, cos: torch.Tensor, sin: torch.Tensor, table: MaskTable, num_heads: int,
             scale: Optional[float] = None, position_ids: Optional[torch.Tensor] = None,
             dead_rows: int = DEAD_ROWS_UNIFORM, row_scale: Optional[torch.Tensor] = None) -> torch.Tensor:
    dev = _dev(x, w_qkv, cos, sin, position_ids, row_scale)
    B, Lq, d = x.shape
    Dh = w_qkv.shape[0] // (3 * num_heads)
    x2 = _rows2d(x)
    cos = cos.to(torch.float32).reshape(-1, Dh).contiguous()
    sin = sin.to(torch.float32).reshape(-1, Dh).contiguous()
    if position_ids is not None:
        position_ids = position_ids.to(torch.int32).expand(B, Lq).contiguous()
    o = torch.empty((B, Lq, num_heads * Dh), dtype=x.dtype, device=dev)
    lib = L.load()
    ws = _ws(lib.aki_mma_attn_workspace_bytes(B, num_heads, Lq, Dh, _dt(x)), dev)
    a = _fused_args(x2, w_qkv, cos, sin, position_ids, o, None, table, B, num_heads, Lq, Dh,
                    scale if scale is not None else Dh ** -0.5, dead_rows, row_scale=row_scale)
    end = _TAP.begin(("mma_attn", B, num_heads, Lq, Dh)) if (_TAP is not None and _TAP.want(("mma_attn",))) else None
    L.check(lib.aki_mma_attn_fwd(C.byref(a), _ptr(ws), ws.numel(), _stream()), "aki_mma_attn_fwd")
    if end is not None:
        end.record()
    return o


def qkv_rope(x: torch.Tensor, w_qkv: torch.Tensor, cos: torch.Tensor, sin: torch.Tensor, num_heads: int,
             position_ids: Optional[torch.Tensor] = None, k_out: Optional[torch.Tensor] = None,
             v_out: Optional[torch.Tensor] = None, row_scale: Optional[torch.Tensor] = None) -> Tuple[torch.Tensor, torch.Tensor, torch.Tensor]:
    dev = _dev(x, w_qkv, cos, sin, k_out, v_out)
    B, Lq, d = x.shape
    Dh = w_qkv.shape[0] // (3 * num_heads)
    x2 = _rows2d(x)
    cos = cos.to(torch.float32).reshape(-1, Dh).contiguous()
    sin = sin.to(torch.float32).reshape(-1, Dh).contiguous()
    if position_ids is not None:
        position_ids = position_ids.to(torch.int32).expand(B, Lq).contiguous()
    q = torch.empty((B, num_heads, Lq, Dh), dtype=x.dtype, device=dev)
    if k_out is None:
        k_out = torch.empty((B, num_heads, Lq, Dh), dtype=x.dtype, device=dev)
        v_out = torch.empty((B, num_heads, Lq, Dh), dtype=x.dtype, device=dev)
    cap = k_out.shape[2]
    if not (k_out.is_contiguous() and v_out.is_contiguous()) or v_out.shape != k_out.shape or cap < Lq:
        raise AkiError("qkv_rope: bad KV output buffers")
    a = _fused_args(x2, w_qkv, cos, sin, position_ids, None, None, MaskTable(None, None, None, Lq), B, num_heads, Lq, Dh,
                    Dh ** -0.5, 0, 0 if cap == Lq else cap, row_scale=row_scale)
    ws = _ws(B * Lq * 3 * num_heads * Dh * 4 if x.dtype == torch.float32 else 256, dev)
    L.check(L.load().aki_qkv_rope_fwd(C.byref(a), _ptr(q), _ptr(k_out), _ptr(v_out), _ptr(ws), ws.numel(), _stream()),
            "aki_qkv_rope_fwd")
    return q, k_out, v_out


def rope_append(qkv: torch.Tensor, cos: torch.Tensor, sin: torch.Tensor, pos: torch.Tensor, cache_len: torch.Tensor,
                k_cache: torch.Tensor, v_cache: torch.Tensor, num_heads: int) -> torch.Tensor:
    dev = _dev(qkv, cos, sin, pos, cache_len, k_cache, v_cache)
    B = qkv.shape[0]
    Dh = qkv.shape[1] // (3 * num_heads)
    q = torch.empty((B, num_heads, Dh), dtype=qkv.dtype, device=dev)
    L.check(L.load().aki_rope_append_fwd(_ptr(qkv.contiguous()), _ptr(cos), _ptr(sin), _ptr(pos), _ptr(cache_len), _ptr(q),
                                         _ptr(k_cache), _ptr(v_cache), B, num_heads, Dh, k_cache.shape[2], _dt(qkv), _stream()),
            "aki_rope_append_fwd")
    return q


def decode_attn_workspace(B: int, H: int, Dh: int, capacity: int, device) -> torch.Tensor:
    nbytes = int(L.load().aki_decode_attn_workspace_bytes(B, H, Dh, capacity))
    return torch.zeros((nbytes + 3) // 4, dtype=torch.int32, device=device)


def kv_cache_quant_fp8(src: torch.Tensor, dst: torch.Tensor, scale: torch.Tensor, rows: int) -> None:
    _dev(src, dst, scale)
    if src.dtype != torch.bfloat16 or dst.dtype != torch.uint8 or scale.dtype != torch.float32:
        raise AkiError("kv_cache_quant_fp8: bf16 source, uint8 destination, f32 scales")
    if not (src.is_contiguous() and dst.is_contiguous() and scale.is_contiguous()) or src.shape[:-2] != dst.shape[:-2] \
# ... 993 lines not shown
```

aki_amd/phi3.py:

```python
from __future__ import annotations

import math
import warnings
from types import SimpleNamespace
from typing import Optional

import torch
import torch.nn.functional as F
from torch import nn

from . import ops
from . import train_ops as T
from .helpers import CausalLMOutputWithPast


def make_phi3_config(**kw):
    defaults = dict(vocab_size=32064, hidden_size=3072, intermediate_size=8192, num_hidden_layers=32,
                    num_attention_heads=32, num_key_value_heads=32, rms_norm_eps=1e-5, rope_theta=10000.0,
                    max_position_embeddings=4096, original_max_position_embeddings=4096, initializer_range=0.02,
                    pad_token_id=32000, bos_token_id=1, eos_token_id=32000, rope_scaling=None)
    defaults.update(kw)
    return SimpleNamespace(**defaults)


# ... 258 lines not shown
                                         cache.grid_keys, cache.attn_ws)
        ks, vs = cache.scales(i)
        return ops.decode_attn_fused(qkv, cos, sin, cache.cache_len, cache.k[i], cache.v[i], self.num_heads, self.scaling, cache.valid_bits,
                                     cache.grid_keys, cache.attn_ws, ks, vs)


class Phi3MLP(nn.Module):
    fuse_train_swiglu = True

    def __init__(self, config):
        super().__init__()
        self.gate_up_proj = nn.Linear(config.hidden_size, 2 * config.intermediate_size, bias=False)
        self.down_proj = nn.Linear(config.intermediate_size, config.hidden_size, bias=False)

    def forward(self, x, residual):
        if _ag(x, self.gate_up_proj.weight, self.down_proj.weight):
            a = T.gate_up_swiglu(x, self.gate_up_proj.weight) if self.fuse_train_swiglu else T.SwigluFn.apply(T.linear(x, self.gate_up_proj.weight))
            return T.linear(a, self.down_proj.weight, None, residual)
        a = ops.linear(x, self.gate_up_proj.weight, act=ops.ACT_SWIGLU)
        return ops.linear(a, self.down_proj.weight, residual=residual)

    def decode(self, h, norm):
        a = ops.decode_linear(h, self.gate_up_proj.weight, norm.weight, norm.variance_epsilon, act=ops.ACT_SWIGLU)
        return ops.linear(a, self.down_proj.weight, residual=h)


class Phi3DecoderLayer(nn.Module):
    def __init__(self, config, layer_idx):
        super().__init__()
        self.self_attn = Phi3Attention(config, layer_idx)
        self.mlp = Phi3MLP(config)
        self.input_layernorm = Phi3RMSNorm(config.hidden_size, eps=config.rms_norm_eps)
        self.post_attention_layernorm = Phi3RMSNorm(config.hidden_size, eps=config.rms_norm_eps)
        self._fp8 = None
        self._w4 = None
        self._prep = ops.Prepared()

    def folds(self, h) -> bool:
        return (h.dtype == torch.bfloat16 and self._fp8 is None and T.CACHE_WT and not T.sharded(self.self_attn.qkv_proj.weight)
                and not _ag(h, *self.parameters()))

    def train(self, mode: bool = True):
        if mode:
            self._prep.clear()
        return super().train(mode)

    def forward_folded(self, h, st, cos, sin, table, position_ids=None, cache=None):
        at, mlp, n1, n2 = self.self_attn, self.mlp, self.input_layernorm, self.post_attention_layernorm
        wq = self._prep.get("qkv", [at.qkv_proj.weight, n1.weight], lambda: ops.fold_gain(at.qkv_proj.weight, n1.weight), T._EPOCH)
        wg = self._prep.get("gate_up", [mlp.gate_up_proj.weight, n2.weight],
                            lambda: ops.fold_gain(mlp.gate_up_proj.weight, n2.weight), T._EPOCH)
        M = h.numel() // h.shape[-1]
        if cache is None:
            o = ops.mma_attn(h, wq, cos, sin, table, at.num_heads, at.scaling, position_ids, row_scale=st.rstd)
        else:
            q, k, v = ops.qkv_rope(h, wq, cos, sin, at.num_heads, position_ids, k_out=cache.k[at.layer_idx],
                                   v_out=cache.v[at.layer_idx], row_scale=st.rstd)
            o = ops.mma_attn_core(q, k, v, table, at.scaling)
        st2 = ops.new_stats(M, h.device)
        h = ops.linear(o, at.o_proj.weight, residual=h, stats_out=st2, stats_eps=n2.variance_epsilon)
        a = ops.linear(h, wg, act=ops.ACT_SWIGLU, row_scale=st2.rstd)
        st3 = ops.new_stats(M, h.device)
        h = ops.linear(a, mlp.down_proj.weight, residual=h, stats_out=st3, stats_eps=n1.variance_epsilon)
        return h, st3

    def forward(self, h, cos, sin, table, position_ids=None, cache=None, stats=None):
        if stats is not None:
            return self.forward_folded(h, stats, cos, sin, table, position_ids, cache)
        if self._fp8 is not None and not torch.is_grad_enabled():
            return self._forward_fp8(h, cos, sin, table, position_ids, cache)
        if cache is None and _ag(h, *self.parameters()):
            n1, n2 = self.input_layernorm, self.post_attention_layernorm
            x, hr = T.rmsnorm_residual(h, n1.weight, n1.variance_epsilon)
            h = self.self_attn(x, cos, sin, table, hr, position_ids, None)
            x, hr = T.rmsnorm_residual(h, n2.weight, n2.variance_epsilon)
            return self.mlp(x, hr)
        h = self.self_attn(self.input_layernorm(h), cos, sin, table, h, position_ids, cache)
        return self.mlp(self.post_attention_layernorm(h), h)

    def _forward_fp8(self, h, cos, sin, table, position_ids, cache=None):
        w = self._fp8
        B, L, d = h.shape
        n1, n2, at = self.input_layernorm, self.post_attention_layernorm, self.self_attn
        xq, xs = ops.quant_rows_fp8(h, n1.weight, n1.variance_epsilon)
        if cache is None:
            o = ops.mma_attn_fp8(xq, xs, *w["qkv"], cos, sin, table, B, at.num_heads, at.scaling, position_ids)
        else:
            q, k, v = ops.qkv_rope_fp8(xq, xs, *w["qkv"], cos, sin, B, at.num_heads, position_ids,
                                       k_out=cache.k[at.layer_idx], v_out=cache.v[at.layer_idx])
            o = ops.mma_attn_core(q, k, v, table, at.scaling)
        if w["o"] is None:
            h = ops.linear(o.view(B, L, d), at.o_proj.weight, residual=h)
        else:
            oq, os_ = ops.quant_rows_fp8(o)
            h = ops.linear_fp8(oq, os_, *w["o"], residual=h, out_shape=(B, L, d))
        xq, xs = ops.quant_rows_fp8(h, n2.weight, n2.variance_epsilon)
        a = ops.linear_fp8(xq, xs, *w["gate_up"], act=ops.ACT_SWIGLU)
        if w["down"] is None:
            return ops.linear(a.view(B, L, -1), self.mlp.down_proj.weight, residual=h)
        aq, as_ = ops.quant_rows_fp8(a)
        return ops.linear_fp8(aq, as_, *w["down"], residual=h, out_shape=(B, L, d))

    def quantize_fp8(self, residual_writers: bool = True):
        at, mlp = self.self_attn, self.mlp
        self._fp8 = {"qkv": ops.quant_rows_fp8(at.qkv_proj.weight.detach()),
                     "o": ops.quant_rows_fp8(at.o_proj.weight.detach()) if residual_writers else None,
                     "gate_up": ops.quant_rows_fp8(mlp.gate_up_proj.weight.detach()),
                     "down": ops.quant_rows_fp8(mlp.down_proj.weight.detach()) if residual_writers else None}

    def quantize_mxfp4(self):
        at, mlp = self.self_attn, self.mlp
        self._w4 = {"qkv": ops.quant_mxfp4(at.qkv_proj.weight.detach()), "o": ops.quant_mxfp4(at.o_proj.weight.detach()),
                    "gate_up": ops.quant_mxfp4(mlp.gate_up_proj.weight.detach()), "down": ops.quant_mxfp4(mlp.down_proj.weight.detach())}

    def decode(self, h, cos, sin, cache):
# ... 252 lines not shown
            self._fp8_head = None
            return self
        if self.model.embed_tokens.weight.dtype != torch.bfloat16:
            raise ops.AkiError("enable_fp8: the model must hold bf16 weights")
        for layer in self.model.layers:
            layer.quantize_fp8(residual_writers)
        self._fp8_head = None
        if head:
            hd = self.lm_head
            if type(hd) is nn.Linear:
                w, b, n = hd.weight.detach(), hd.bias, hd.weight.shape[0]
            else:
                w, b, n = hd._fused_weight()
            self._fp8_head = (*ops.quant_rows_fp8(w), b, n)
        return self

    def enable_mxfp4(self, enable: bool = True, head: bool = True):
        self.model._weights_version += 1
        if not enable:
            for layer in self.model.layers:
                layer._w4 = None
            self._w4_head = None
            return self
        hd = self.lm_head
        if type(hd) is nn.Linear:
            hw, hb, hn = hd.weight.detach(), hd.bias, hd.weight.shape[0]
        else:
            hw, hb, hn = hd._fused_weight()
        mats = [m.weight for ly in self.model.layers for m in (ly.self_attn.qkv_proj, ly.self_attn.o_proj, ly.mlp.gate_up_proj, ly.mlp.down_proj)]
        mats += [hw] if head else []
        if any(m.dtype != torch.bfloat16 or not m.is_cuda for m in mats):
            raise ops.AkiError("enable_mxfp4: the model must hold bf16 weights on the GPU")
        if not all(bool(torch.isfinite(m).all()) for m in mats):
            raise ops.AkiError("enable_mxfp4: a weight matrix holds non-finite values")
        for layer in self.model.layers:
            layer.quantize_mxfp4()
        self._w4_head = (*ops.quant_mxfp4(hw), hb, hn) if head else None
        return self

    def _head(self, h):
        if getattr(self, "_fp8_head", None) is not None and not torch.is_grad_enabled() and getattr(self, "_pre_norm_h", None) is not None:
            wq, ws, b, n = self._fp8_head
            hq, hs = ops.quant_rows_fp8(self._pre_norm_h, self.model.norm.weight, self.model.norm.variance_epsilon)
            self._pre_norm_h = None
            return ops.linear_fp8(hq, hs, wq, ws, bias=b, out_shape=(*h.shape[:-1], wq.shape[0]))[..., :n]
        if type(self.lm_head) is nn.Linear:
            return ops.linear(h, self.lm_head.weight, bias=self.lm_head.bias)
        return self.lm_head(h)

    def _head_folded(self, h, st):
        norm, head = self.model.norm, self.lm_head
        if type(head) is nn.Linear:
            w = self._prep.get("head", [head.weight, norm.weight], lambda: ops.fold_gain(head.weight, norm.weight), T._EPOCH)
            return ops.linear(h, w, bias=head.bias, row_scale=st.rstd)
        w0, b, n = head._fused_weight()
        w = self._prep.get("head", [w0, norm.weight], lambda: ops.fold_gain(w0, norm.weight), (T._EPOCH, head._fused[0]))
        return ops.linear(h, w, bias=b, row_scale=st.rstd)[..., :n]

    kv_cache_dtype = "bf16"
    share_prompt_kv = False

    chunked_continue = False

    device_beam_search = False

    def set_kv_cache_dtype(self, dtype: str = "bf16"):
        if not isinstance(dtype, str) or dtype not in KV_CACHE_DTYPES:
            raise ValueError(f"kv cache dtype must be one of {KV_CACHE_DTYPES}, got {dtype!r}")
        self.kv_cache_dtype = dtype
        return self

    def forward(self, input_ids=None, attention_mask=None, inputs_embeds=None, labels=None, position_ids=None,
                use_cache=False, past_key_values=None, cache_capacity=None, last_token_logits=False, **kwargs):
        if past_key_values is not None:
            return self._continue(input_ids, inputs_embeds, past_key_values, labels)
        if last_token_logits and labels is not None:
            raise ValueError("last_token_logits=True keeps one row of logits per sample; a loss over `labels` needs all of them")
        if last_token_logits and not use_cache:
            raise ValueError("last_token_logits=True is the prefill of a generation: pass use_cache=True (without a cache the flag used to be ignored silently)")
        if inputs_embeds is None:
            inputs_embeds = self.model.embed_tokens(input_ids)
        B, L, _ = inputs_embeds.shape
        table = attention_mask
        if table is None:
            table = ops.MaskTable.causal(B, L, inputs_embeds.device)
        elif isinstance(table, torch.Tensor):
            table = mask_table_from_tensor(table, L)
        cache = stage = None
        if use_cache:
            cfg = self.config
            H = cfg.num_attention_heads
            Dh = getattr(cfg, "head_dim", None) or cfg.hidden_size // H
            cache = stage = AkiKVCache(len(self.model.layers), B, H, Dh, int(cache_capacity or (L + 256)), inputs_embeds.dtype,
                                       inputs_embeds.device, self.kv_cache_dtype)
            if cache.kv_dtype != "bf16":
                stage = AkiKVCache(len(self.model.layers), B, H, Dh, L, inputs_embeds.dtype, inputs_embeds.device)
        fp8_head = getattr(self, "_fp8_head", None) is not None and not torch.is_grad_enabled()
        self.model.skip_final_norm = fp8_head
        self.model.defer_final_norm = True
        h = self.model(inputs_embeds, table, position_ids, stage)
        self.model.skip_final_norm = self.model.defer_final_norm = False
        if stage is not cache:
            cache.quantise_from(stage, L)
            cache.host_len = stage.host_len
            stage = None
        head_stats, self.model.final_stats = self.model.final_stats, None
        self._pre_norm_h = h if fp8_head else None
        if head_stats is not None and _ag(h, *self.lm_head.parameters()):
            h, head_stats = ops.rmsnorm(h, self.model.norm.weight, self.model.norm.variance_epsilon), None
        if labels is not None and cache is None and _ag(h, *self.lm_head.parameters()):
# ... 146 lines not shown
```

aki_amd/siglip.py:

```python
from __future__ import annotations

from types import SimpleNamespace

import torch
import torch.nn.functional as F
from torch import nn

from . import ops


def make_siglip_config(**kw):
    d = dict(hidden_size=1152, intermediate_size=4304, num_hidden_layers=27, num_attention_heads=16, num_channels=3,
             image_size=384, patch_size=14, layer_norm_eps=1e-6, hidden_act="gelu_pytorch_tanh")
    d.update(kw)
    return SimpleNamespace(**d)


_Prepared = ops.Prepared


def _epoch(params) -> int:
    if not any(p.requires_grad for p in params):
        return 0
    from . import train_ops as T
# ... 12 lines not shown
class SiglipVisionEmbeddings(nn.Module):
    def __init__(self, config):
        super().__init__()
        self.config = config
        self.embed_dim = config.hidden_size
        self.image_size = config.image_size
        self.patch_size = config.patch_size
        self.patch_embedding = nn.Conv2d(config.num_channels, self.embed_dim, kernel_size=self.patch_size,
                                         stride=self.patch_size, padding="valid")
        self.num_patches = (self.image_size // self.patch_size) ** 2
        self.num_positions = self.num_patches
        self.position_embedding = nn.Embedding(self.num_positions, self.embed_dim)
        self._prep = _Prepared()

    def _pos_for(self, grid: int):
        w = self.position_embedding.weight
        g0 = int(round(self.num_positions ** 0.5))
        if grid == g0:
            return w
        return self._prep.get(f"pos{grid}", [w], lambda: F.interpolate(
            w.float().reshape(1, g0, g0, -1).permute(0, 3, 1, 2), size=(grid, grid), mode="bicubic", align_corners=False
        ).permute(0, 2, 3, 1).reshape(grid * grid, -1).to(w.dtype).contiguous())

    def forward(self, pixel_values, interpolate_pos_encoding=False):
        w = self.patch_embedding.weight
        wp = self._prep.get("w", [w], lambda: ops.pad_k(w.reshape(w.shape[0], -1)))
        S = pixel_values.shape[-1]
        grid = S // self.patch_size
        if grid * grid != self.num_positions and not interpolate_pos_encoding:
            raise ValueError(f"input size {S} does not match the position table ({self.num_positions} patches); "
                             "pass interpolate_pos_encoding=True")
        return ops.patch_embed(pixel_values.to(w.dtype), wp, self.patch_embedding.bias, self._pos_for(grid), self.patch_size)


class SiglipAttention(nn.Module):
    def __init__(self, config):
        super().__init__()
        self.embed_dim = config.hidden_size
        self.num_heads = config.num_attention_heads
        self.head_dim = self.embed_dim // self.num_heads
        self.scale = self.head_dim ** -0.5
        self.k_proj = nn.Linear(self.embed_dim, self.embed_dim)
        self.v_proj = nn.Linear(self.embed_dim, self.embed_dim)
        self.q_proj = nn.Linear(self.embed_dim, self.embed_dim)
        self.out_proj = nn.Linear(self.embed_dim, self.embed_dim)
        self._prep = _Prepared()

    def forward_folded(self, h, st, ln, stats_out, stats_eps):
        N, L, E = h.shape
        ps = [self.q_proj.weight, self.k_proj.weight, self.v_proj.weight, self.q_proj.bias, self.k_proj.bias, self.v_proj.bias,
              ln.weight, ln.bias]
        wqkv, bqkv, cqkv = self._prep.get("qkv_ln", ps, lambda: fold_layernorm(torch.cat([p.detach() for p in ps[:3]], 0),
                                                                                torch.cat([p.detach() for p in ps[3:6]], 0), ln), _epoch(ps))
        qkv = ops.linear(h, wqkv, bias=bqkv, row_scale=st.rstd, row_shift=st.mean, col_shift=cqkv)
        qkv = qkv.view(N, L, 3, self.num_heads, self.head_dim)
        a = ops.attention(qkv[:, :, 0], qkv[:, :, 1], qkv[:, :, 2], self.scale)
        return ops.linear(a, self.out_proj.weight, bias=self.out_proj.bias, residual=h, stats_out=stats_out, stats_eps=stats_eps)

    def forward(self, x, residual):
        N, L, E = x.shape
        ps = [self.q_proj.weight, self.k_proj.weight, self.v_proj.weight, self.q_proj.bias, self.k_proj.bias, self.v_proj.bias]
        wqkv, bqkv = self._prep.get("qkv", ps, lambda: (torch.cat([p.detach() for p in ps[:3]], 0).contiguous(),
                                                        torch.cat([p.detach() for p in ps[3:]], 0).contiguous()), _epoch(ps))
        qkv = ops.linear(x, wqkv, bias=bqkv).view(N, L, 3, self.num_heads, self.head_dim)
        a = ops.attention(qkv[:, :, 0], qkv[:, :, 1], qkv[:, :, 2], self.scale)
        return ops.linear(a, self.out_proj.weight, bias=self.out_proj.bias, residual=residual)


_HBUF = {}


def _fc1_buffer(lead, Kp, x):
    key = (tuple(lead), Kp, x.dtype, x.device, torch.cuda.current_stream().cuda_stream)
    hbuf = _HBUF.get(key)
    if hbuf is None:
        if len(_HBUF) > 8:
            _HBUF.clear()
        hbuf = _HBUF[key] = torch.zeros((*lead, Kp), dtype=x.dtype, device=x.device)
    return hbuf


class SiglipMLP(nn.Module):
    def __init__(self, config):
        super().__init__()
        self.fc1 = nn.Linear(config.hidden_size, config.intermediate_size)
        self.fc2 = nn.Linear(config.intermediate_size, config.hidden_size)
        self.act = ops.ACT_GELU_TANH if "tanh" in config.hidden_act else ops.ACT_GELU_ERF
        self._prep = _Prepared()

    def forward(self, x, residual, st=None, ln=None, stats_out=None, stats_eps=0.0):
        inter = self.fc1.weight.shape[0]
        Kp = (inter + 63) // 64 * 64
        w2 = self._prep.get("w2", [self.fc2.weight], lambda: ops.pad_k(self.fc2.weight.detach()), _epoch([self.fc2.weight]))
        lead = x.shape[:-1]
        hbuf = _fc1_buffer(lead, Kp, x)
        if st is None:
            ops.linear(x, self.fc1.weight, bias=self.fc1.bias, act=self.act, out=hbuf[..., :inter])
        else:
            w1, b1, c1 = self._prep.get("fc1_ln", [self.fc1.weight, self.fc1.bias, ln.weight, ln.bias],
                                        lambda: fold_layernorm(self.fc1.weight.detach(), self.fc1.bias.detach(), ln),
                                        _epoch([self.fc1.weight, self.fc1.bias, ln.weight, ln.bias]))
            ops.linear(x, w1, bias=b1, act=self.act, out=hbuf[..., :inter], row_scale=st.rstd, row_shift=st.mean, col_shift=c1)
        return ops.linear(hbuf, w2, bias=self.fc2.bias, residual=residual, stats_out=stats_out, stats_eps=stats_eps)


class SiglipEncoderLayer(nn.Module):
    def __init__(self, config):
        super().__init__()
        self.layer_norm1 = nn.LayerNorm(config.hidden_size, eps=config.layer_norm_eps)
        self.self_attn = SiglipAttention(config)
        self.layer_norm2 = nn.LayerNorm(config.hidden_size, eps=config.layer_norm_eps)
        self.mlp = SiglipMLP(config)

    def forward_folded(self, h, st, want_stats=True):
        M = h.numel() // h.shape[-1]
        st2 = ops.new_stats(M, h.device, ln=True)
        h = self.self_attn.forward_folded(h, st, self.layer_norm1, st2, self.layer_norm2.eps)
        st3 = ops.new_stats(M, h.device, ln=True) if want_stats else None
        return self.mlp(h, h, st=st2, ln=self.layer_norm2, stats_out=st3, stats_eps=self.layer_norm1.eps), st3

    def forward(self, h, stats=None, want_stats=True):
        if stats is not None:
            return self.forward_folded(h, stats, want_stats)
        h = self.self_attn(ops.layernorm(h, self.layer_norm1.weight, self.layer_norm1.bias, self.layer_norm1.eps), h)
        return self.mlp(ops.layernorm(h, self.layer_norm2.weight, self.layer_norm2.bias, self.layer_norm2.eps), h)


class SiglipEncoder(nn.Module):
    def __init__(self, config):
        super().__init__()
        self.layers = nn.ModuleList([SiglipEncoderLayer(config) for _ in range(config.num_hidden_layers)])

    fold_norms = True

    def forward(self, h):
        if self.fold_norms and h.dtype == torch.bfloat16 and not (torch.is_grad_enabled() and (
                h.requires_grad or any(p.requires_grad for p in self.parameters()))):
            if self._can_stack(h):
                return self._forward_stack(h)
            st = ops.row_stats(h, self.layers[0].layer_norm1.eps, ln=True)
            for i, layer in enumerate(self.layers):
                h, st = layer(h, stats=st, want_stats=i + 1 < len(self.layers))
            return h
        for layer in self.layers:
            h = layer(h)
        return h


def _siglip_can_stack(self, h) -> bool:
    if not (self.use_layer_stack and ops.stack_enabled() and h.is_cuda and h.dim() == 3 and h.is_contiguous()):
        return False
    l0 = self.layers[0]
    for ly in self.layers:
        if (ly.layer_norm1.eps != l0.layer_norm1.eps or ly.layer_norm2.eps != l0.layer_norm1.eps
                or ly.mlp.act != l0.mlp.act or ly.mlp.fc1.bias is None or ly.self_attn.q_proj.bias is None):
            return False
    return not ops.python_must_run_between(self.layers)


def _siglip_forward_stack(self, h):
    tb = getattr(self, "_stack_table", None)
    if tb is None:
        tb = self._stack_table = ops.LayerTable(ops.L.SiglipLayer)
    live = []
    for ly in self.layers:
        at, mlp = ly.self_attn, ly.mlp
        for m in (at.q_proj, at.k_proj, at.v_proj, at.out_proj, ly.layer_norm1, ly.layer_norm2, mlp.fc1, mlp.fc2):
            pm = m._parameters
            live.append(pm["weight"])
            if pm.get("bias") is not None:
                live.append(pm["bias"])
# ... 47 lines not shown
```

include/aki_mi355x.h:

```cpp
#ifndef AKI_MI355X_H
#define AKI_MI355X_H

#include <stddef.h>
#include <stdint.h>

#ifdef __cplusplus
extern "C" {
#endif

#define AKI_ABI_VERSION 17

typedef enum {
  AKI_OK = 0,
  AKI_ERR_INVALID_ARG = -1,
  AKI_ERR_UNSUPPORTED = -2,
  AKI_ERR_ALIGNMENT = -3,
  AKI_ERR_WORKSPACE = -4,
  AKI_ERR_LAUNCH = -5
} aki_status;

typedef enum {
  AKI_DT_BF16 = 0,
  AKI_DT_F32 = 1,
  AKI_DT_FP8_E4M3 = 2,
// ... 16 lines not shown
} aki_mma_rect;

#define AKI_MAX_RECTS 8
#define AKI_PLAN_STRIDE 12

typedef enum { AKI_DEAD_ROWS_ZERO = 0, AKI_DEAD_ROWS_UNIFORM = 1 } aki_dead_rows;

typedef struct {
  const void* q;
  const void* k;
  const void* v;
  void* o;
  float* lse;
  const aki_mma_rect* rects;
  const uint64_t* col_valid_bits;
  const int32_t* seq_lens;
  int32_t max_rects;
  int32_t B, H, L, Dh;
  float scale;
  int32_t dtype;
  int32_t dead_rows;
  int32_t kv_capacity;
} aki_mma_attn_core_args;

size_t aki_mma_attn_core_workspace_bytes(int32_t B, int32_t H, int32_t L, int32_t Dh, int32_t dtype);
int aki_mma_attn_core_fwd(const aki_mma_attn_core_args* args, void* workspace, size_t workspace_bytes, void* stream);

typedef struct {
  const void* x;
  const void* w_qkv;
  const float* cos;
  const float* sin;
  const int32_t* position_ids;
  void* o;
  float* lse;
  const aki_mma_rect* rects;
  const uint64_t* col_valid_bits;
  const int32_t* seq_lens;
  int32_t max_rects;
  int32_t B, H, L, Dh, d_model;
  int32_t ldx, ldw;
  int32_t pos_rows;
  float scale;
  int32_t dtype;
  int32_t dead_rows;
  int32_t kv_capacity;
  const float* x_scale;
  const float* w_scale;
  const float* row_scale;
} aki_mma_attn_args;

size_t aki_mma_attn_workspace_bytes(int32_t B, int32_t H, int32_t L, int32_t Dh, int32_t dtype);
int aki_mma_attn_fwd(const aki_mma_attn_args* args, void* workspace, size_t workspace_bytes, void* stream);

int aki_qkv_rope_fwd(const aki_mma_attn_args* args, void* q_out, void* k_out, void* v_out, void* workspace,
                     size_t workspace_bytes, void* stream);

typedef struct {
  const void* q;
  const void* k;
  const void* v;
  void* o;
  int64_t q_stride_b, q_stride_h, q_stride_t;
  int64_t k_stride_b, k_stride_h, k_stride_t;
  int64_t v_stride_b, v_stride_h, v_stride_t;
  int32_t B, H, Lq, Lk, Dh;
  float scale;
  int32_t dtype;
  float* lse;
} aki_attn_args;

int aki_attn_fwd(const aki_attn_args* args, void* workspace, size_t workspace_bytes, void* stream);

typedef struct {
  const void* x;
  const void* w;
  const void* bias;
  const void* residual;
  void* y;
  int32_t M, N, K;
  int32_t ldx, ldw, ldy, ldr;
  int32_t res_row_mod;
  int32_t act;
  int32_t dtype;
  const float* x_scale;
  const float* w_scale;
  const void* w2;
  int32_t w2_row0;
  int32_t w2_rows;
  const float* row_scale;
  const float* row_shift;
  const float* col_shift;
  float* stats_rstd;
  float* stats_mean;
  float stats_eps;
  void* stats_workspace;
  size_t stats_workspace_bytes;
  void* splitk_workspace;
  size_t splitk_workspace_bytes;
  void* preact_out;
  int64_t ld_preact;
} aki_linear_args;

int aki_linear_fwd(const aki_linear_args* args, void* stream);
size_t aki_linear_stats_workspace_bytes(int32_t M, int32_t N_out);
size_t aki_linear_splitk_workspace_bytes(int32_t M, int32_t N, int32_t K);
size_t aki_linear_stats_counter_bytes(int32_t M);
int aki_row_stats(const void* x, int32_t rows, int32_t cols, int32_t ldx, float eps, float* rstd, float* mean, int32_t dtype, void* stream);

int aki_rmsnorm_fwd(const void* x, const void* weight, void* y, int32_t rows, int32_t cols, int32_t ldx, int32_t ldy,
                    float eps, int32_t dtype, void* stream);
int aki_layernorm_fwd(const void* x, const void* weight, const void* bias, void* y, int32_t rows, int32_t cols,
                      int32_t ldx, int32_t ldy, float eps, int32_t dtype, void* stream);

size_t aki_patch_embed_workspace_bytes(int32_t N, int32_t S, int32_t P, int32_t dtype);
int aki_patch_embed_fwd(const void* pixels, const void* w, const void* bias, const void* pos, void* out, int32_t N,
                        int32_t S, int32_t P, int32_t E, int32_t Kp, int32_t dtype, void* workspace,
                        size_t workspace_bytes, void* stream);

size_t aki_connector_mlp_workspace_bytes(int32_t rows, int32_t d, int32_t d_inner, int32_t dtype);
int aki_connector_mlp_fwd(const void* x, const void* ln_w, const void* ln_b, const void* w1, const void* w2, void* out,
                          int32_t rows, int32_t d, int32_t d_inner, float eps, int32_t dtype, void* workspace,
                          size_t workspace_bytes, void* stream);
int aki_connector_proj_fwd(const void* x, const void* ln_w, const void* ln_b, const void* w, const void* b, void* out,
                           int32_t rows, int32_t d, int32_t d_out, float eps, int32_t dtype, void* workspace,
                           size_t workspace_bytes, void* stream);

typedef struct {
  const int64_t* lang_x;
  const int64_t* attention_mask;
  const int64_t* labels;
  const void* embed_weight;
  const void* embed_additional;
  const void* vision_tokens;
  const int32_t* plan;
  void* inputs_embeds;
  int64_t* labels_out;
  int64_t* mask_1d_out;
  aki_mma_rect* rects;
  uint64_t* col_valid_bits;
  int32_t* seq_lens;
  int64_t max_original_id;
  int64_t media_token_id;
  int64_t pad_token_id;
  int32_t B, T, T_img, Nv, d, L_out;
  int32_t max_rects;
  int32_t padding_side;
  int32_t dtype;
} aki_splice_args;

int aki_splice_plan(const int64_t* lang_x, int32_t B, int32_t T, int64_t media_token_id, int64_t assistant_token_id,
                    int32_t Nv, int32_t* plan, void* stream);
int aki_splice_fwd(const aki_splice_args* args, void* stream);

int aki_rope_append_fwd(const void* qkv, const float* cos, const float* sin, const int32_t* pos, const int32_t* cache_len,
                        void* q_out, void* k_cache, void* v_cache, int32_t B, int32_t H, int32_t Dh, int32_t capacity,
                        int32_t dtype, void* stream);
// ... 299 lines not shown
```

Measured before the change: 134,300.

## Defer norm row-stats reduction into the consuming GEMM prologue

The producing GEMM no longer runs its cross-tile atomic/flag reduction to finish the RMS/LayerNorm row stats. It writes per-tile partial sums to a slot buffer, and the next GEMM (QKV-rope, gate-up, LM head, SigLIP fc1/qkv) loads them at the start and folds them into rstd/mean while its first weight tiles are in flight. This removes the last-block counter synchronization and the extra stats pass. In exchange it costs 24 extra register pairs per lane, reduces through up to 24 slots redundantly in every consumer tile, and adds a new ABI with inline-asm waitcnt bookkeeping.

```diff
diff --git a/aki_amd/_lib.py b/aki_amd/_lib.py
--- a/aki_amd/_lib.py
+++ b/aki_amd/_lib.py
@@ -72,6 +72,12 @@
                 ("preact_out", C.c_void_p), ("ld_preact", C.c_int64)]
 
 
+class StatsDefer(C.Structure):
+    _fields_ = [("in_partials", C.c_void_p), ("out_partials", C.c_void_p), ("out_partials_bytes", C.c_size_t),
+                ("in_slots", C.c_int32), ("in_n", C.c_int32), ("in_eps", C.c_float), ("in_layernorm", C.c_int32),
+                ("out_slots", C.c_int32), ("reserved", C.c_int32)]
+
+
 class DecoderLayer(C.Structure):
     _fields_ = [("w_qkv", C.c_void_p), ("w_o", C.c_void_p), ("w_gate_up", C.c_void_p), ("w_down", C.c_void_p), ("k_cache", C.c_void_p),
                 ("v_cache", C.c_void_p)]
@@ -148,6 +154,11 @@
     "aki_qkv_rope_fwd": (C.c_int, [C.POINTER(MmaAttnArgs), C.c_void_p, C.c_void_p, C.c_void_p, C.c_void_p, C.c_size_t, C.c_void_p]),
     "aki_attn_fwd": (C.c_int, [C.POINTER(AttnArgs), C.c_void_p, C.c_size_t, C.c_void_p]),
     "aki_linear_fwd": (C.c_int, [C.POINTER(LinearArgs), C.c_void_p]),
+    "aki_linear_fwd_ex": (C.c_int, [C.POINTER(LinearArgs), C.POINTER(StatsDefer), C.c_void_p]),
+    "aki_mma_attn_fwd_ex": (C.c_int, [C.POINTER(MmaAttnArgs), C.POINTER(StatsDefer), C.c_void_p, C.c_size_t, C.c_void_p]),
+    "aki_linear_stats_slots": (C.c_int32, [C.c_int32, C.c_int32, C.c_int32]),
+    "aki_linear_stats_partials_bytes": (C.c_size_t, [C.c_int32, C.c_int32, C.c_int32]),
+    "aki_row_stats_fold": (C.c_int, [C.c_void_p, C.c_int32, C.c_int32, C.c_int32, C.c_float, C.c_void_p, C.c_void_p, C.c_void_p]),
     "aki_linear_stats_workspace_bytes": (C.c_size_t, [C.c_int32, C.c_int32]),
     "aki_linear_splitk_workspace_bytes": (C.c_size_t, [C.c_int32, C.c_int32, C.c_int32]),
     "aki_linear_stats_counter_bytes": (C.c_size_t, [C.c_int32]),
diff --git a/aki_amd/csrc/aki_device.h b/aki_amd/csrc/aki_device.h
--- a/aki_amd/csrc/aki_device.h
+++ b/aki_amd/csrc/aki_device.h
@@ -97,6 +97,19 @@
   for (int i = 0; i < N; ++i) asm volatile("" : "+v"(v[i]));
 }
 
+__device__ __forceinline__ void row_stats_finish(float s1, float s2, int n_out, float eps, bool layernorm, float& rstd, float& mean_out) {
+  const float inv_n = 1.0f / (float)n_out;
+  const float mean = s1 * inv_n;
+  mean_out = mean;
+  if (layernorm) rstd = rsqrtf(fmaxf(s2 * inv_n - mean * mean, 0.f) + eps);
+  else rstd = rsqrtf(s2 * inv_n + eps);
+}
+#define AKI_STATS_DEFER_MAX_SLOTS 24
+__device__ __forceinline__ void row_stats_add(float& s1, float& s2, unsigned lo, unsigned hi) {
+  s2 += __uint_as_float(lo);
+  s1 += __uint_as_float(hi);
+}
+
 __device__ __forceinline__ float wave_sum(float v) {
 #pragma unroll
   for (int o = 32; o > 0; o >>= 1) v += __shfl_xor(v, o);
diff --git a/aki_amd/csrc/api.hip b/aki_amd/csrc/api.hip
--- a/aki_amd/csrc/api.hip
+++ b/aki_amd/csrc/api.hip
@@ -1,12 +1,14 @@
 #include "aki_device.h"
 
 namespace aki {
-int linear_bf16(const aki_linear_args* a, hipStream_t stream);
+int linear_bf16(const aki_linear_args* a, hipStream_t stream, const aki_stats_defer* d = nullptr);
+int linear_stats_slots(int M, int n_out, int K);
+int row_stats_fold_launch(const void* part, int rows, int slots, int n_out, float eps, float* rstd, float* mean, hipStream_t s);
 size_t linear_stats_ws_bytes(int M, int n_out);
 size_t linear_stats_cnt_bytes(int M);
 int row_stats_launch(const void* x, int rows, int cols, int ldx, float eps, float* rstd, float* mean, hipStream_t s);
 int linear_f32(const aki_linear_args* a, hipStream_t stream);
-int qkv_rope_bf16(const aki_mma_attn_args* a, void* q, void* k, void* v, hipStream_t stream);
+int qkv_rope_bf16(const aki_mma_attn_args* a, void* q, void* k, void* v, hipStream_t stream, const aki_stats_defer* d = nullptr);
 int qkv_rope_fp8(const aki_mma_attn_args* a, void* q, void* k, void* v, hipStream_t stream);
 int linear_fp8(const aki_linear_args* a, hipStream_t stream);
 int quant_rows_fp8_launch(const void* x, const void* rms_w, float eps, void* q, float* scale, int rows, int cols, int ldx, int ldq,
@@ -232,10 +234,13 @@
   return qkv_rope_f32(a, q, k, v, (float*)ws, (hipStream_t)stream);
 }
 
-int aki_mma_attn_fwd(const aki_mma_attn_args* a, void* ws, size_t ws_bytes, void* stream) {
+int aki_mma_attn_fwd(const aki_mma_attn_args* a, void* ws, size_t ws_bytes, void* stream) { return aki_mma_attn_fwd_ex(a, nullptr, ws, ws_bytes, stream); }
+
+int aki_mma_attn_fwd_ex(const aki_mma_attn_args* a, const aki_stats_defer* d, void* ws, size_t ws_bytes, void* stream) {
   AKI_CLEAR_ERR();
   int rc = check_fused(a);
   if (rc) return rc;
+  if (d && (d->in_partials || d->out_partials) && a->dtype != AKI_DT_BF16) return AKI_ERR_UNSUPPORTED;
   AKI_CHECK_ARG(a->o && a->scale > 0.f);
   AKI_CHECK_ARG(a->max_rects >= 0 && (a->max_rects == 0 || a->rects));
   const int cdt = a->dtype == AKI_DT_FP8_E4M3 ? AKI_DT_BF16 : a->dtype;
@@ -246,7 +251,7 @@
   void* q = w; void* k = w + qb; void* v = w + 2 * qb;
   char* rest = w + 3 * qb;
   if (a->dtype == AKI_DT_BF16) {
-    rc = qkv_rope_bf16(a, q, k, v, (hipStream_t)stream);
+    rc = qkv_rope_bf16(a, q, k, v, (hipStream_t)stream, d);
   } else if (a->dtype == AKI_DT_FP8_E4M3) {
     rc = qkv_rope_fp8(a, q, k, v, (hipStream_t)stream);
   } else {
@@ -270,6 +275,33 @@
   AKI_CHECK_ARG(x && rstd && rows > 0 && cols > 0 && ldx >= cols && eps > 0.f);
   if (dtype != AKI_DT_BF16) return AKI_ERR_UNSUPPORTED;
   return row_stats_launch(x, rows, cols, ldx, eps, rstd, mean, (hipStream_t)stream);
+}
+
+int32_t aki_linear_stats_slots(int32_t M, int32_t N_out, int32_t K) { return linear_stats_slots(M, N_out, K); }
+size_t aki_linear_stats_partials_bytes(int32_t M, int32_t N_out, int32_t K) {
+  const int slots = linear_stats_slots(M, N_out, K);
+  return slots ? aki_align_up((size_t)M * slots * 8, 256) : 0;
+}
+int aki_row_stats_fold(const void* partials, int32_t rows, int32_t slots, int32_t n_out, float eps, float* rstd, float* mean, void* stream) {
+  AKI_CHECK_ARG(partials && rstd && rows > 0 && n_out > 0 && eps > 0.f);
+  return row_stats_fold_launch(partials, rows, slots, n_out, eps, rstd, mean, (hipStream_t)stream);
+}
+
+int aki_linear_fwd_ex(const aki_linear_args* a, const aki_stats_defer* d, void* stream) {
+  if (!d || (!d->in_partials && !d->out_partials)) return aki_linear_fwd(a, stream);
+  AKI_CLEAR_ERR();
+  AKI_CHECK_ARG(a && a->x && a->w && a->y);
+  AKI_CHECK_ARG(a->M > 0 && a->N > 0 && a->K > 0);
+  AKI_CHECK_ARG(a->act >= AKI_ACT_NONE && a->act <= AKI_ACT_SWIGLU);
+  const int n_out = a->act == AKI_ACT_SWIGLU ? a->N / 2 : a->N;
+  AKI_CHECK_ARG(a->ldx >= a->K && a->ldw >= a->K && a->ldy >= n_out && (!a->residual || a->ldr >= n_out));
+  if (a->dtype != AKI_DT_BF16) return AKI_ERR_UNSUPPORTED;
+  if (a->w2) {
+    AKI_CHECK_ARG(a->w2_row0 > 0 && a->w2_rows > 0 && a->w2_row0 < a->N);
+    if (a->act != AKI_ACT_NONE) return AKI_ERR_UNSUPPORTED;
+  }
+  if (a->preact_out && a->act != AKI_ACT_SWIGLU) return AKI_ERR_UNSUPPORTED;
+  return linear_bf16(a, (hipStream_t)stream, d);
 }
 
 int aki_linear_fwd(const aki_linear_args* a, void* stream) {
diff --git a/aki_amd/csrc/aux_kernels.hip b/aki_amd/csrc/aux_kernels.hip
--- a/aki_amd/csrc/aux_kernels.hip
+++ b/aki_amd/csrc/aux_kernels.hip
@@ -122,6 +122,28 @@
   }
   block_sum2<256>(d2, dummy, red);
   if (threadIdx.x == 0) { mean[row] = mu; rstd[row] = rsqrtf(d2 / cols + eps); }
+}
+
+__global__ __launch_bounds__(256) void row_stats_fold_kernel(const unsigned long long* part, int rows, int slots, int n_out, float eps, float* rstd, float* mean) {
+  const int row = blockIdx.x * 256 + threadIdx.x;
+  if (row >= rows) return;
+  float s1 = 0.f, s2 = 0.f;
+  for (int i = 0; i < slots; ++i) {
+    const unsigned long long g = part[(size_t)i * rows + row];
+    row_stats_add(s1, s2, (unsigned)g, (unsigned)(g >> 32));
+  }
+  float r, mu;
+  row_stats_finish(s1, s2, n_out, eps, mean != nullptr, r, mu);
+  rstd[row] = r;
+  if (mean) mean[row] = mu;
+}
+int row_stats_fold_launch(const void* part, int rows, int slots, int n_out, float eps, float* rstd, float* mean, hipStream_t s) {
+  if (slots < 2 || (slots & 1)) return AKI_ERR_INVALID_ARG;
+  AKI_CHECK_ALIGN16(part);
+  AKI_CLEAR_ERR();
+  hipLaunchKernelGGL(row_stats_fold_kernel, dim3((rows + 255) / 256), dim3(256), 0, s, (const unsigned long long*)part, rows, slots, n_out, eps, rstd, mean);
+  AKI_LAUNCH_CHECK();
+  return AKI_OK;
 }
 
 int row_stats_launch(const void* x, int rows, int cols, int ldx, float eps, float* rstd, float* mean, hipStream_t s) {
diff --git a/aki_amd/csrc/gemm_bf16.hip b/aki_amd/csrc/gemm_bf16.hip
--- a/aki_amd/csrc/gemm_bf16.hip
+++ b/aki_amd/csrc/gemm_bf16.hip
@@ -48,6 +48,10 @@
   float* st_mean;
   float* st_part;
   unsigned* st_cnt;
+  int st_defer, st_slots;
+  const unsigned long long* fold_part;
+  int fold_slots, fold_ld, fold_n, fold_ln;
+  float fold_eps;
   int ksplit;
   float* sk_part;
   size_t sk_bytes;
@@ -178,10 +182,53 @@
 
   constexpr int NOUT = (EPI == EPI_SWIGLU) ? NF / 2 : NF;
   const int fwave = n0 + wn * (EPI == EPI_SWIGLU ? WROWS / 2 : WROWS);
-  const bool shifted = (PIPE == 0 || PIPE == 4 || PIPE == 8) && (EPI == EPI_PLAIN) && p.row_shift != nullptr;
+  const bool shifted = (PIPE == 0 || PIPE == 4 || PIPE == 8) && (EPI == EPI_PLAIN) && (p.row_shift != nullptr || (p.fold_part != nullptr && p.fold_ln));
   u32x2 biasp[NOUT];
   f32x4 colc4[NOUT];
   float rsv[NT], muv[NT];
+  constexpr bool EARLY_OPERANDS = (!PIPE || PIPE == 8) && !FP8 && NF * NT <= 16;
+  const bool folding = !FP8 && p.fold_part != nullptr;
+  constexpr int FOLD_SLOTS = AKI_STATS_DEFER_MAX_SLOTS;
+  u32x2 fold_g[FOLD_SLOTS];
+  float fold_rs = 1.0f, fold_mu = 0.0f;
+  auto fold_issue = [&]() {
+    if constexpr (!FP8) {
+      if (!folding) return;
+      const int row = min(m0 + wm * WTOK + min(lane, WTOK - 1), p.M - 1);
+      const unsigned long long* const src_ = p.fold_part + row;
+#pragma unroll
+      for (int i = 0; i < FOLD_SLOTS; ++i)
+        asm volatile("global_load_dwordx2 %0, %1, off" : "=&v"(fold_g[i]) : "v"(src_ + (size_t)min(i, p.fold_slots - 1) * p.fold_ld) : "memory");
+    }
+  };
+  auto fold_hand_out = [&](float& rs_, float& mu_, int m) {
+    rs_ = __shfl(fold_rs, m * 16 + l15);
+    mu_ = (EPI == EPI_PLAIN && shifted) ? __shfl(fold_mu, m * 16 + l15) : 0.0f;
+  };
+  auto fold_finish = [&](auto dma_after_) {
+    if constexpr (!FP8) {
+      if (!folding) return;
+      static_assert(FOLD_SLOTS == 24, "the wait below names every load");
+      asm volatile("s_waitcnt vmcnt(%24)"
+                   : "+v"(fold_g[0]), "+v"(fold_g[1]), "+v"(fold_g[2]), "+v"(fold_g[3]), "+v"(fold_g[4]), "+v"(fold_g[5]), "+v"(fold_g[6]), "+v"(fold_g[7]),
+                     "+v"(fold_g[8]), "+v"(fold_g[9]), "+v"(fold_g[10]), "+v"(fold_g[11]), "+v"(fold_g[12]), "+v"(fold_g[13]), "+v"(fold_g[14]),
+                     "+v"(fold_g[15]), "+v"(fold_g[16]), "+v"(fold_g[17]), "+v"(fold_g[18]), "+v"(fold_g[19]), "+v"(fold_g[20]), "+v"(fold_g[21]),
+                     "+v"(fold_g[22]), "+v"(fold_g[23])
+                   : "n"(decltype(dma_after_)::value)
+                   : "memory");
+      float s1 = 0.f, s2 = 0.f;
+#pragma unroll
+      for (int i = 0; i < FOLD_SLOTS; ++i)
+        if (i < p.fold_slots) row_stats_add(s1, s2, fold_g[i][0], fold_g[i][1]);
+      row_stats_finish(s1, s2, p.fold_n, p.fold_eps, p.fold_ln != 0, fold_rs, fold_mu);
+      asm volatile("" : "+v"(fold_rs), "+v"(fold_mu));
+      if constexpr (EARLY_OPERANDS) {
+#pragma unroll
+        for (int m = 0; m < NT; ++m) fold_hand_out(rsv[m], muv[m], m);
+      }
+    }
+  };
+  using std::integral_constant;
   auto fetch_epilogue_operands = [&]() {
     if (EPI == EPI_QKV_ROPE8) return;
 #pragma unroll
@@ -195,11 +242,14 @@
 #pragma unroll
     for (int m = 0; m < NT; ++m) {
       const int mr = min(m0 + wm * WTOK + m * 16 + l15, p.M - 1);
-      rsv[m] = p.row_scale ? p.row_scale[mr] : 1.0f;
-      muv[m] = (EPI == EPI_PLAIN && shifted) ? p.row_shift[mr] : 0.0f;
+      if (!FP8 && folding) {
+        if constexpr (!EARLY_OPERANDS) fold_hand_out(rsv[m], muv[m], m);
+      } else {
+        rsv[m] = p.row_scale ? p.row_scale[mr] : 1.0f;
+        muv[m] = (EPI == EPI_PLAIN && shifted) ? p.row_shift[mr] : 0.0f;
+      }
     }
   };
-  constexpr bool EARLY_OPERANDS = (!PIPE || PIPE == 8) && !FP8 && NF * NT <= 16;
   constexpr int RCH = BN / 8;
   constexpr int CMASK = RCH >= 16 ? 15 : RCH - 1;
   constexpr int RES_PIECES = (BM * RCH * 16) / (NWAVES * 1024);
@@ -209,6 +259,7 @@
   const bool res_pf = RES_PF_OK && p.residual != nullptr && p.res_wide && p.res_row_mod <= 0 && n_out >= 8;
   int res_off = 0;
   const bool cs_pf = EPI == EPI_QKV_ROPE8 && PIPE == 4 && BM == 256 && n0 / 32 < 6 * p.H && p.position_ids == nullptr && p.L >= BM;
+  fold_issue();
   if constexpr (EARLY_OPERANDS) fetch_epilogue_operands();
   auto compute = [&](const char* sb) {
     if constexpr (FP8) {
@@ -333,6 +384,9 @@
     stage_w(0, 0); stage_x(0, 0);
     if (nk > 1) { stage_w(1, 1); stage_x(1, 1); }
     if (nk > 2) stage_w(2, 2);
+    if (nk > 2) fold_finish(integral_constant<int, 2 * NLD + NLH>{});
+    else if (nk > 1) fold_finish(integral_constant<int, 2 * NLD>{});
+    else fold_finish(integral_constant<int, NLD>{});
     if (nk > 2) asm volatile("s_waitcnt vmcnt(%0)" ::"n"(3 * NLH) : "memory");
     else if (nk > 1) asm volatile("s_waitcnt vmcnt(%0)" ::"n"(NLD) : "memory");
     else asm volatile("s_waitcnt vmcnt(0)" ::: "memory");
@@ -412,6 +466,8 @@
     };
     stage_w8(0, 0); stage_x8(0, 0);
     if (nk > 1) stage_x8(1, 1);
+    if (nk > 1) fold_finish(integral_constant<int, NLW + 2 * NLX>{});
+    else fold_finish(integral_constant<int, NLW + NLX>{});
     int xs = 0;
     for (int kt = 0; kt < nk; ++kt) {
       if (kt + 1 < nk) asm volatile("s_waitcnt vmcnt(%0)" ::"n"(NLX) : "memory");
@@ -437,6 +493,7 @@
     }
   } else if constexpr (NST == 2) {
     stage(0, 0);
+    fold_finish(integral_constant<int, NLD>{});
     for (int kt = 0; kt < nk; ++kt) {
       __syncthreads();
       if (kt + 1 < nk) stage((kt + 1) & 1, kt + 1);
@@ -459,6 +516,7 @@
 #pragma unroll
     for (int s_ = 0; s_ < NST - 1; ++s_)
       if (s_ < nk) stage(s_, s_);
+    fold_finish(integral_constant<int, NLD>{});
     for (int kt = 0; kt < nk; ++kt) {
       const int rem = nk - 1 - kt;
       if (NST >= 6 && rem >= 4) asm volatile("s_waitcnt vmcnt(%0)" ::"n"(4 * NLD) : "memory");
@@ -613,7 +671,8 @@
       offq[m] = ((size_t)b * ((size_t)p.H * p.L) + tt) * 96;
       dkv[m] = (size_t)b * ((size_t)p.H * (p.kvcap - p.L)) * 96;
       csoff[m] = (wm * WTOK + m * 16 + l15) * CSROW + 16 * kg;
-      rsq[m] = p.row_scale ? p.row_scale[min(mrow, p.M - 1)] : 1.0f;
+      if (!FP8 && folding) rsq[m] = __shfl(fold_rs, m * 16 + l15);
+      else rsq[m] = p.row_scale ? p.row_scale[min(mrow, p.M - 1)] : 1.0f;
     }
     const __attribute__((address_space(3))) char* const lcs = (const __attribute__((address_space(3))) char*)AKI_LDS_PTR(smem);
     auto rope_rows = [&](auto fullm_) {
@@ -818,9 +877,10 @@
         s1 += __shfl_xor(s1, 16); s2 += __shfl_xor(s2, 16);
         s1 += __shfl_xor(s1, 32); s2 += __shfl_xor(s2, 32);
         if (kg == 0 && ok) {
+          const unsigned long long both = (unsigned long long)__float_as_uint(s2) | ((unsigned long long)__float_as_uint(s1) << 32);
           unsigned long long* pp = (unsigned long long*)p.st_part + (size_t)(tn * WN + wn) * p.M + mrow;
-          const unsigned long long both = (unsigned long long)__float_as_uint(s2) | ((unsigned long long)__float_as_uint(s1) << 32);
-          __hip_atomic_store(pp, both, __ATOMIC_RELAXED, __HIP_MEMORY_SCOPE_AGENT);
+          if (!SK && !FP8 && p.st_defer) *pp = both;
+          else __hip_atomic_store(pp, both, __ATOMIC_RELAXED, __HIP_MEMORY_SCOPE_AGENT);
         }
       }
       if (wide) {
@@ -848,7 +908,7 @@
     using c2 = std::integral_constant<int, 2>;
     const bool inside = m0 + BM <= p.M && n0 + (EPI == EPI_SWIGLU ? BN / 2 : BN) <= n_out;
     const bool fast = inside && NOUT % 2 == 0 && p.wide && (p.residual == nullptr || (EPI == EPI_PLAIN && res_lds));
-    const int key = (EPI == EPI_PLAIN && p.bias ? 1 : 0) | (p.residual ? 2 : 0) | (stats ? 4 : 0) | (p.row_scale ? 8 : 0) | (shifted ? 16 : 0);
+    const int key = (EPI == EPI_PLAIN && p.bias ? 1 : 0) | (p.residual ? 2 : 0) | (stats ? 4 : 0) | ((p.row_scale || folding) ? 8 : 0) | (shifted ? 16 : 0);
     bool done = false;
     if (fast) {
       done = true;
@@ -868,7 +928,7 @@
     }
     if (!done) write_rows(c0{}, c2{}, c2{}, c2{}, c2{}, c2{});
   }
-  if (EPI == EPI_PLAIN && stats) {
+  if (EPI == EPI_PLAIN && stats && (SK || FP8 || !p.st_defer)) {
     asm volatile("s_waitcnt vmcnt(0)" ::: "memory");
     __syncthreads();
     unsigned* const flag = (unsigned*)smem;
@@ -908,22 +968,17 @@
           for (int sl = 0; sl < total / BM; ++sl) {
             unsigned long long both = park[sl * BM + tid];
             asm volatile("s_waitcnt lgkmcnt(0)" : "+v"(both));
-            s2 += __uint_as_float((unsigned)both);
-            s1 += __uint_as_float((unsigned)(both >> 32));
+            row_stats_add(s1, s2, (unsigned)both, (unsigned)(both >> 32));
           }
         }
         __syncthreads();
       }
       if (tid < BM && m0 + tid < p.M) {
         const int mrow = m0 + tid;
-        const float inv_n = 1.0f / (float)n_out;
-        const float mean = s1 * inv_n;
-        if (p.st_mean) {
-          p.st_mean[mrow] = mean;
-          p.st_rstd[mrow] = rsqrtf(fmaxf(s2 * inv_n - mean * mean, 0.f) + p.st_eps);
-        } else {
-          p.st_rstd[mrow] = rsqrtf(s2 * inv_n + p.st_eps);
-        }
+        float rstd, mean;
+        row_stats_finish(s1, s2, n_out, p.st_eps, p.st_mean != nullptr, rstd, mean);
+        if (p.st_mean) p.st_mean[mrow] = mean;
+        p.st_rstd[mrow] = rstd;
       }
       if (tid == 0) __hip_atomic_store(p.st_cnt + tm, 0u, __ATOMIC_RELAXED, __HIP_MEMORY_SCOPE_AGENT);
     }
@@ -990,6 +1045,8 @@
   const int bn_out = (EPI == EPI_SWIGLU) ? BN / 2 : BN;
   p.tiles_m = (p.M + BM - 1) / BM;
   p.tiles_n = (n_out + bn_out - 1) / bn_out;
+  if (p.st_defer && (SK || FP8 || EPI != EPI_PLAIN || p.st_slots != p.tiles_n * WN)) return AKI_ERR_INVALID_ARG;
+  if (p.fold_part && FP8) return AKI_ERR_UNSUPPORTED;
   AKI_CLEAR_ERR();
 #ifdef AKI_LAB_HOOKS
   p.clock_probe = g_clock_probe;
@@ -1055,7 +1112,7 @@
     return launch_gemm<8, 4, 2, 4, EPI, ACT, FP8>(p, stream);
   } else {
     if constexpr (EPI == EPI_PLAIN && ACT == 0) {
-      if (g_res_prefetch && p.row_shift == nullptr && p.residual != nullptr && p.res_wide && p.res_row_mod <= 0 && p.N % 8 == 0 && p.N >= 8)
+      if (g_res_prefetch && p.row_shift == nullptr && !p.fold_ln && p.residual != nullptr && p.res_wide && p.res_row_mod <= 0 && p.N % 8 == 0 && p.N >= 8)
         return deep_tokens(p) ? launch_gemm<8, 4, 2, 4, EPI, ACT, FP8, 2, 6>(p, stream) : launch_gemm<8, 4, 2, 4, EPI, ACT, FP8, 2, 5>(p, stream);
     }
     return launch_gemm<8, 4, 2, 4, EPI, ACT, FP8, 2, 4>(p, stream);
@@ -1122,7 +1179,8 @@
       const int n_out = (EPI == EPI_SWIGLU) ? p.N / 2 : p.N;
       plan_small_m(EPI, p.M, n_out, p.K, p.sk_part != nullptr, v, ks);
       if (v >= 0 && ks > 1 && p.sk_bytes < linear_splitk_ws_bytes(v, ks, p.M, n_out) - linear_splitk_cnt_bytes()) v = -1;
-      if (v >= 0 && !(EPI == EPI_PLAIN && p.row_shift != nullptr)) return launch_small_m<EPI, ACT>(p, v, ks, stream);
+      if (p.st_defer && ks > 1) return AKI_ERR_INVALID_ARG;
+      if (v >= 0 && !(EPI == EPI_PLAIN && (p.row_shift != nullptr || p.fold_ln))) return launch_small_m<EPI, ACT>(p, v, ks, stream);
     }
   }
   if (plan == 1) return launch_small<EPI, ACT, FP8>(p, stream);
@@ -1131,6 +1189,7 @@
     if (plan == 3) return launch_gemm<4, 3, 2, 2, EPI, ACT, FP8, 2, 8>(p, stream);
     if (plan == 4) return launch_gemm<2, 2, 2, 2, EPI, ACT, FP8, 4>(p, stream);
   }
+  if (p.st_defer) return AKI_ERR_INVALID_ARG;
   const int m_main = p.M / 256 * 256;
   GemmParams a = p, b = p;
   a.M = m_main;
@@ -1145,6 +1204,7 @@
   if (p.residual && p.res_row_mod <= 0) b.residual = p.residual + (size_t)m_main * p.ldr;
   if (p.row_scale) b.row_scale = p.row_scale + m_main;
   if (p.row_shift) b.row_shift = p.row_shift + m_main;
+  if (p.fold_part) b.fold_part = p.fold_part + m_main;
   if (p.st_rstd) b.st_rstd = p.st_rstd + m_main;
   if (p.st_mean) b.st_mean = p.st_mean + m_main;
   return launch_small<EPI, ACT, FP8>(b, stream);
@@ -1160,7 +1220,35 @@
   return linear_stats_cnt_bytes(M) + (size_t)(2 * ((n_out + 63) / 64) + 2) * 2 * (size_t)M * sizeof(float);
 }
 
-int linear_bf16(const aki_linear_args* a, hipStream_t stream) {
+int linear_stats_slots(int M, int n_out, int K) {
+  if (M < 1 || n_out < 4 || K < 64 || K % 64 != 0 || M > kStatsMaxRows) return 0;
+  int v, ks;
+  plan_small_m(EPI_PLAIN, M, n_out, K, true, v, ks);
+  if (v >= 0) return 0;
+  const int plan = plan_tiles(M, n_out, 256, 128, 0.25, true, K / 64);
+  int bn = 0;
+  if (plan == 0) bn = 256;
+  else if (plan == 3) bn = 128;
+  else if (plan == 4) bn = 64;
+  else if (plan == 1) {
+    const long tiles = (long)((M + 127) / 128) * ((n_out + 127) / 128);
+    bn = (g_deep_ring && M <= 128 && K / 64 >= 4 && tiles <= 128) ? 64 : 128;
+  }
+  const int slots = bn ? 2 * ((n_out + bn - 1) / bn) : 0;
+  return slots <= AKI_STATS_DEFER_MAX_SLOTS ? slots : 0;
+}
+
+static int set_fold_source(GemmParams& p, const aki_stats_defer* d, bool has_row_scale, int rows) {
+  if (!d || !d->in_partials) return AKI_OK;
+  if (has_row_scale || d->in_slots < 2 || (d->in_slots & 1) || d->in_n < 1 || !(d->in_eps > 0.f)) return AKI_ERR_INVALID_ARG;
+  if (d->in_slots > AKI_STATS_DEFER_MAX_SLOTS) return AKI_ERR_UNSUPPORTED;
+  if (((uintptr_t)d->in_partials) & 15) return AKI_ERR_ALIGNMENT;
+  p.fold_part = (const unsigned long long*)d->in_partials;
+  p.fold_slots = d->in_slots; p.fold_ld = rows; p.fold_n = d->in_n; p.fold_eps = d->in_eps; p.fold_ln = d->in_layernorm ? 1 : 0;
+  return AKI_OK;
+}
+
+int linear_bf16(const aki_linear_args* a, hipStream_t stream, const aki_stats_defer* d) {
   if (a->K % 64 != 0) return AKI_ERR_UNSUPPORTED;
   const int n_out = a->act == AKI_ACT_SWIGLU ? a->N / 2 : a->N;
   if (n_out % 4 != 0 || (a->act == AKI_ACT_SWIGLU && (a->N % 8 != 0))) return AKI_ERR_UNSUPPORTED;
@@ -1188,6 +1276,18 @@
     p.st_cnt = (unsigned*)a->stats_workspace;
     p.st_part = (float*)((char*)a->stats_workspace + linear_stats_cnt_bytes(a->M));
   }
+  if (d) {
+    const int rc = set_fold_source(p, d, a->row_scale || a->row_shift, a->M);
+    if (rc) return rc;
+    if (p.fold_ln && (!a->col_shift || (((uintptr_t)a->col_shift) & 15) || a->act == AKI_ACT_SWIGLU)) return AKI_ERR_INVALID_ARG;
+    if (d->out_partials) {
+      if (a->stats_rstd || a->act != AKI_ACT_NONE || a->w2 || a->M > kStatsMaxRows) return AKI_ERR_INVALID_ARG;
+      if (d->out_slots < 2 || d->out_slots != linear_stats_slots(a->M, n_out, a->K)) return AKI_ERR_INVALID_ARG;
+      if (d->out_partials_bytes < (size_t)a->M * d->out_slots * 8) return AKI_ERR_WORKSPACE;
+      if (((uintptr_t)d->out_partials) & 15) return AKI_ERR_ALIGNMENT;
+      p.st_part = (float*)d->out_partials; p.st_defer = 1; p.st_slots = d->out_slots;
+    }
+  }
   if (a->preact_out) {
     if (a->act != AKI_ACT_SWIGLU || a->row_scale) return AKI_ERR_INVALID_ARG;
     if ((a->ld_preact % 4) || a->ld_preact < a->N || ((uintptr_t)a->preact_out & 7)) return AKI_ERR_ALIGNMENT;
@@ -1210,7 +1310,7 @@
   }
 }
 
-int qkv_rope_bf16(const aki_mma_attn_args* a, void* q, void* k, void* v, hipStream_t stream) {
+int qkv_rope_bf16(const aki_mma_attn_args* a, void* q, void* k, void* v, hipStream_t stream, const aki_stats_defer* d) {
   if (a->Dh != 96) return AKI_ERR_UNSUPPORTED;
   if (a->d_model % 64 != 0) return AKI_ERR_UNSUPPORTED;
   if ((a->ldx % 8) || (a->ldw % 8)) return AKI_ERR_ALIGNMENT;
@@ -1223,6 +1323,11 @@
   p.cos = a->cos; p.sin = a->sin; p.position_ids = a->position_ids; p.H = a->H; p.L = a->L;
   p.kvcap = a->kv_capacity > 0 ? a->kv_capacity : a->L;
   p.row_scale = a->row_scale;
+  if (d) {
+    if (d->out_partials || d->in_layernorm) return AKI_ERR_INVALID_ARG;
+    const int rc = set_fold_source(p, d, a->row_scale != nullptr, p.M);
+    if (rc) return rc;
+  }
   return run_planned<EPI_QKV_ROPE8, 0>(p, plan_tiles(p.M, p.N, 256, 128), stream);
 }
 
diff --git a/aki_amd/ops.py b/aki_amd/ops.py
--- a/aki_amd/ops.py
+++ b/aki_amd/ops.py
@@ -105,10 +105,40 @@
     return (w.detach().to(ct) * gain.detach().to(ct)[None, :]).to(w.dtype).contiguous()
 
 
-@dataclass
 class RowStats:
-    rstd: torch.Tensor
-    mean: Optional[torch.Tensor] = None
+
+    def __init__(self, rstd: Optional[torch.Tensor] = None, mean: Optional[torch.Tensor] = None, *, partials: Optional[torch.Tensor] = None,
+                 slots: int = 0, ln: bool = False):
+        self._rstd, self._mean = rstd, mean
+        self.partials, self.slots, self.ln = partials, int(slots), bool(ln or mean is not None)
+        self.n_out, self.eps = 0, 0.0
+
+    @property
+    def deferred(self) -> bool:
+        return self.partials is not None
+
+    def _fold(self) -> None:
+        if self.n_out <= 0:
+            raise AkiError("RowStats: deferred statistics read before a producer GEMM wrote them")
+        M = self.partials.shape[1]
+        dev = self.partials.device
+        self._rstd = torch.empty((M,), dtype=torch.float32, device=dev)
+        self._mean = torch.empty((M,), dtype=torch.float32, device=dev) if self.ln else None
+        with torch.cuda.device(dev):
+            L.check(L.load().aki_row_stats_fold(_ptr(self.partials), M, self.slots, self.n_out, float(self.eps), _ptr(self._rstd),
+                                                _ptr(self._mean), _stream()), "aki_row_stats_fold")
+
+    @property
+    def rstd(self) -> torch.Tensor:
+        if self._rstd is None and self.partials is not None:
+            self._fold()
+        return self._rstd
+
+    @property
+    def mean(self) -> Optional[torch.Tensor]:
+        if self._rstd is None and self.partials is not None:
+            self._fold()
+        return self._mean
 
 
 _STATS_WS = {}
@@ -139,8 +169,23 @@
     return hit
 
 
-def new_stats(M: int, dev, ln: bool = False) -> RowStats:
+DEFER_STATS = True
+
+
+def new_stats(M: int, dev, ln: bool = False, producer: Optional[Tuple[int, int]] = None) -> RowStats:
+    if producer is not None and DEFER_STATS:
+        slots = int(L.load().aki_linear_stats_slots(M, int(producer[0]), int(producer[1])))
+        if slots > 0:
+            return RowStats(partials=torch.empty((slots, M, 2), dtype=torch.float32, device=dev), slots=slots, ln=ln)
     return RowStats(torch.empty((M,), dtype=torch.float32, device=dev), torch.empty((M,), dtype=torch.float32, device=dev) if ln else None)
+
+
+def _stats_source(st: RowStats) -> "L.StatsDefer":
+    if st.n_out <= 0:
+        raise AkiError("deferred statistics consumed before a producer GEMM wrote them")
+    d = L.StatsDefer()
+    d.in_partials, d.in_slots, d.in_n, d.in_eps, d.in_layernorm = st.partials.data_ptr(), st.slots, st.n_out, float(st.eps), int(st.ln)
+    return d
 
 
 def row_stats(x: torch.Tensor, eps: float, ln: bool = False) -> RowStats:
@@ -210,6 +255,14 @@
            w2_row0: int = 0, n_rows: Optional[int] = None, row_scale: Optional[torch.Tensor] = None,
            row_shift: Optional[torch.Tensor] = None, col_shift: Optional[torch.Tensor] = None,
            stats_out: Optional[RowStats] = None, stats_eps: float = 0.0, preact_out: Optional[torch.Tensor] = None) -> torch.Tensor:
+    defer = None
+    if isinstance(row_scale, RowStats):
+        if row_shift is not None:
+            raise AkiError("linear: a RowStats row_scale carries its own row_shift")
+        if row_scale.deferred and row_scale._rstd is None:
+            defer, row_scale = _stats_source(row_scale), None
+        else:
+            row_scale, row_shift = row_scale.rstd, row_scale.mean
     dev = _dev(x, w, bias, residual, out, w2, row_scale, row_shift, col_shift)
     lib = L.load()
     x2 = _rows2d(x)
@@ -232,7 +285,13 @@
                      0 if r2 is None else r2.stride(0), res_row_mod, act, _dt(x), None, None,
                      _ptr(w2), int(w2_row0) if w2 is not None else 0, int(w2.shape[0]) if w2 is not None else 0)
     a.row_scale, a.row_shift, a.col_shift = _ptr(row_scale), _ptr(row_shift), _ptr(col_shift)
-    if stats_out is not None:
+    if stats_out is not None and stats_out.deferred:
+        if stats_out.partials.shape != (stats_out.slots, M, 2):
+            raise AkiError("linear: deferred statistics sized for another launch")
+        defer = defer if defer is not None else L.StatsDefer()
+        defer.out_partials, defer.out_partials_bytes, defer.out_slots = stats_out.partials.data_ptr(), stats_out.partials.numel() * 4, stats_out.slots
+        stats_out.n_out, stats_out.eps, stats_out._rstd, stats_out._mean = n_out, float(stats_eps), None, None
+    elif stats_out is not None:
         sws = _stats_ws(M, n_out, dev)
         a.stats_rstd, a.stats_mean, a.stats_eps = _ptr(stats_out.rstd), _ptr(stats_out.mean), float(stats_eps)
         a.stats_workspace, a.stats_workspace_bytes = sws.data_ptr(), sws.numel()
@@ -246,7 +305,10 @@
         if sk is not None:
             a.splitk_workspace, a.splitk_workspace_bytes = sk.data_ptr(), sk.numel()
     end = _TAP.begin(("linear", M, N, K, act)) if (_TAP is not None and _TAP.want(("linear", M, N, K, act))) else None
-    L.check(lib.aki_linear_fwd(C.byref(a), _stream()), "aki_linear_fwd")
+    if defer is not None:
+        L.check(lib.aki_linear_fwd_ex(C.byref(a), C.byref(defer), _stream()), "aki_linear_fwd_ex")
+    else:
+        L.check(lib.aki_linear_fwd(C.byref(a), _stream()), "aki_linear_fwd")
     if end is not None:
         end.record()
     return out
@@ -332,6 +394,12 @@
 def mma_attn(x: torch.Tensor, w_qkv: torch.Tensor, cos: torch.Tensor, sin: torch.Tensor, table: MaskTable, num_heads: int,
              scale: Optional[float] = None, position_ids: Optional[torch.Tensor] = None,
              dead_rows: int = DEAD_ROWS_UNIFORM, row_scale: Optional[torch.Tensor] = None) -> torch.Tensor:
+    defer = None
+    if isinstance(row_scale, RowStats):
+        if row_scale.deferred and row_scale._rstd is None and not row_scale.ln and x.dtype == torch.bfloat16:
+            defer, row_scale = _stats_source(row_scale), None
+        else:
+            row_scale = row_scale.rstd
     dev = _dev(x, w_qkv, cos, sin, position_ids, row_scale)
     B, Lq, d = x.shape
     Dh = w_qkv.shape[0] // (3 * num_heads)
@@ -346,7 +414,10 @@
     a = _fused_args(x2, w_qkv, cos, sin, position_ids, o, None, table, B, num_heads, Lq, Dh,
                     scale if scale is not None else Dh ** -0.5, dead_rows, row_scale=row_scale)
     end = _TAP.begin(("mma_attn", B, num_heads, Lq, Dh)) if (_TAP is not None and _TAP.want(("mma_attn",))) else None
-    L.check(lib.aki_mma_attn_fwd(C.byref(a), _ptr(ws), ws.numel(), _stream()), "aki_mma_attn_fwd")
+    if defer is not None:
+        L.check(lib.aki_mma_attn_fwd_ex(C.byref(a), C.byref(defer), _ptr(ws), ws.numel(), _stream()), "aki_mma_attn_fwd_ex")
+    else:
+        L.check(lib.aki_mma_attn_fwd(C.byref(a), _ptr(ws), ws.numel(), _stream()), "aki_mma_attn_fwd")
     if end is not None:
         end.record()
     return o
diff --git a/aki_amd/phi3.py b/aki_amd/phi3.py
--- a/aki_amd/phi3.py
+++ b/aki_amd/phi3.py
@@ -334,15 +334,15 @@
                             lambda: ops.fold_gain(mlp.gate_up_proj.weight, n2.weight), T._EPOCH)
         M = h.numel() // h.shape[-1]
         if cache is None:
-            o = ops.mma_attn(h, wq, cos, sin, table, at.num_heads, at.scaling, position_ids, row_scale=st.rstd)
+            o = ops.mma_attn(h, wq, cos, sin, table, at.num_heads, at.scaling, position_ids, row_scale=st)
         else:
             q, k, v = ops.qkv_rope(h, wq, cos, sin, at.num_heads, position_ids, k_out=cache.k[at.layer_idx],
                                    v_out=cache.v[at.layer_idx], row_scale=st.rstd)
             o = ops.mma_attn_core(q, k, v, table, at.scaling)
-        st2 = ops.new_stats(M, h.device)
+        st2 = ops.new_stats(M, h.device, producer=tuple(at.o_proj.weight.shape))
         h = ops.linear(o, at.o_proj.weight, residual=h, stats_out=st2, stats_eps=n2.variance_epsilon)
-        a = ops.linear(h, wg, act=ops.ACT_SWIGLU, row_scale=st2.rstd)
-        st3 = ops.new_stats(M, h.device)
+        a = ops.linear(h, wg, act=ops.ACT_SWIGLU, row_scale=st2)
+        st3 = ops.new_stats(M, h.device, producer=tuple(mlp.down_proj.weight.shape) if cache is None else None)
         h = ops.linear(a, mlp.down_proj.weight, residual=h, stats_out=st3, stats_eps=n1.variance_epsilon)
         return h, st3
 
@@ -701,10 +701,10 @@
         norm, head = self.model.norm, self.lm_head
         if type(head) is nn.Linear:
             w = self._prep.get("head", [head.weight, norm.weight], lambda: ops.fold_gain(head.weight, norm.weight), T._EPOCH)
-            return ops.linear(h, w, bias=head.bias, row_scale=st.rstd)
+            return ops.linear(h, w, bias=head.bias, row_scale=st)
         w0, b, n = head._fused_weight()
         w = self._prep.get("head", [w0, norm.weight], lambda: ops.fold_gain(w0, norm.weight), (T._EPOCH, head._fused[0]))
-        return ops.linear(h, w, bias=b, row_scale=st.rstd)[..., :n]
+        return ops.linear(h, w, bias=b, row_scale=st)[..., :n]
 
     kv_cache_dtype = "bf16"
     share_prompt_kv = False
diff --git a/aki_amd/siglip.py b/aki_amd/siglip.py
--- a/aki_amd/siglip.py
+++ b/aki_amd/siglip.py
@@ -88,7 +88,7 @@
               ln.weight, ln.bias]
         wqkv, bqkv, cqkv = self._prep.get("qkv_ln", ps, lambda: fold_layernorm(torch.cat([p.detach() for p in ps[:3]], 0),
                                                                                 torch.cat([p.detach() for p in ps[3:6]], 0), ln), _epoch(ps))
-        qkv = ops.linear(h, wqkv, bias=bqkv, row_scale=st.rstd, row_shift=st.mean, col_shift=cqkv)
+        qkv = ops.linear(h, wqkv, bias=bqkv, row_scale=st, col_shift=cqkv)
         qkv = qkv.view(N, L, 3, self.num_heads, self.head_dim)
         a = ops.attention(qkv[:, :, 0], qkv[:, :, 1], qkv[:, :, 2], self.scale)
         return ops.linear(a, self.out_proj.weight, bias=self.out_proj.bias, residual=h, stats_out=stats_out, stats_eps=stats_eps)
@@ -136,7 +136,7 @@
             w1, b1, c1 = self._prep.get("fc1_ln", [self.fc1.weight, self.fc1.bias, ln.weight, ln.bias],
                                         lambda: fold_layernorm(self.fc1.weight.detach(), self.fc1.bias.detach(), ln),
                                         _epoch([self.fc1.weight, self.fc1.bias, ln.weight, ln.bias]))
-            ops.linear(x, w1, bias=b1, act=self.act, out=hbuf[..., :inter], row_scale=st.rstd, row_shift=st.mean, col_shift=c1)
+            ops.linear(x, w1, bias=b1, act=self.act, out=hbuf[..., :inter], row_scale=st, col_shift=c1)
         return ops.linear(hbuf, w2, bias=self.fc2.bias, residual=residual, stats_out=stats_out, stats_eps=stats_eps)
 
 
@@ -150,9 +150,10 @@
 
     def forward_folded(self, h, st, want_stats=True):
         M = h.numel() // h.shape[-1]
-        st2 = ops.new_stats(M, h.device, ln=True)
+        E, Kp = h.shape[-1], (self.mlp.fc1.weight.shape[0] + 63) // 64 * 64
+        st2 = ops.new_stats(M, h.device, ln=True, producer=(E, E))
         h = self.self_attn.forward_folded(h, st, self.layer_norm1, st2, self.layer_norm2.eps)
-        st3 = ops.new_stats(M, h.device, ln=True) if want_stats else None
+        st3 = ops.new_stats(M, h.device, ln=True, producer=(E, Kp)) if want_stats else None
         return self.mlp(h, h, st=st2, ln=self.layer_norm2, stats_out=st3, stats_eps=self.layer_norm1.eps), st3
 
     def forward(self, h, stats=None, want_stats=True):
diff --git a/include/aki_mi355x.h b/include/aki_mi355x.h
--- a/include/aki_mi355x.h
+++ b/include/aki_mi355x.h
@@ -92,6 +92,8 @@
 
 size_t aki_mma_attn_workspace_bytes(int32_t B, int32_t H, int32_t L, int32_t Dh, int32_t dtype);
 int aki_mma_attn_fwd(const aki_mma_attn_args* args, void* workspace, size_t workspace_bytes, void* stream);
+struct aki_stats_defer;
+int aki_mma_attn_fwd_ex(const aki_mma_attn_args* args, const struct aki_stats_defer* stats, void* workspace, size_t workspace_bytes, void* stream);
 
 int aki_qkv_rope_fwd(const aki_mma_attn_args* args, void* q_out, void* k_out, void* v_out, void* workspace,
                      size_t workspace_bytes, void* stream);
@@ -143,6 +145,21 @@
 } aki_linear_args;
 
 int aki_linear_fwd(const aki_linear_args* args, void* stream);
+typedef struct aki_stats_defer {
+  const void* in_partials;
+  void* out_partials;
+  size_t out_partials_bytes;
+  int32_t in_slots;
+  int32_t in_n;
+  float in_eps;
+  int32_t in_layernorm;
+  int32_t out_slots;
+  int32_t reserved;
+} aki_stats_defer;
+int aki_linear_fwd_ex(const aki_linear_args* args, const aki_stats_defer* stats, void* stream);
+int32_t aki_linear_stats_slots(int32_t M, int32_t N_out, int32_t K);
+size_t aki_linear_stats_partials_bytes(int32_t M, int32_t N_out, int32_t K);
+int aki_row_stats_fold(const void* partials, int32_t rows, int32_t slots, int32_t n_out, float eps, float* rstd, float* mean, void* stream);
 size_t aki_linear_stats_workspace_bytes(int32_t M, int32_t N_out);
 size_t aki_linear_splitk_workspace_bytes(int32_t M, int32_t N, int32_t K);
 size_t aki_linear_stats_counter_bytes(int32_t M);
```

After: 133,500. Within noise of the previous version (-0.6%).
